# ssteinberg/wave_tracer

Hardware: AMD Instinct MI355X
Metric: Msamples/sec (whole node), cornell-box 1440^2 wave-mode (higher is better)
Workload: dtype f32

## Files before the change

### include/wtgpu.h

```cpp
#ifndef WTGPU_H
#define WTGPU_H

#include <stddef.h>
#include <stdint.h>

#include "wtgpu_scene.h"

#ifdef __cplusplus
extern "C" {
#endif

typedef struct wtgpu_scene wtgpu_scene;
typedef struct wtgpu_comm wtgpu_comm;

enum { WTGPU_OK = 0, WTGPU_ERR_INVALID = 1, WTGPU_ERR_NO_DEVICE = 2, WTGPU_ERR_HIP = 3, WTGPU_ERR_OOM = 4, WTGPU_ERR_OVERFLOW = 5, WTGPU_CANCELLED = 6,
       WTGPU_ERR_COMM = 7 };

typedef struct wtgpu_scene_params {
    uint32_t res;
    int32_t max_depth;
    int32_t fsd;
    int32_t mis;
    int32_t rr;
    int32_t force_ray_tracing;
// ... 34 lines not shown

int wtgpu_scene_upload(wtgpu_scene* scene, int device, uint64_t max_batch_samples);

int wtgpu_render(wtgpu_scene* scene, void* stream, double* d_value, double* d_weight, double* d_light, uint64_t sample_begin, uint64_t sample_end,
                 uint64_t seed);

int wtgpu_render_async(wtgpu_scene* scene, void* stream, double* d_value, double* d_weight, double* d_light, uint64_t sample_begin,
                       uint64_t sample_end, uint64_t seed);
int wtgpu_join(wtgpu_scene* scene, void* stream);

typedef int (*wtgpu_progress_cb)(uint64_t samples_done, uint64_t samples_total, void* user);
int wtgpu_render_progressive(wtgpu_scene* scene, void* stream, double* d_value, double* d_weight, double* d_light, uint64_t sample_begin,
                             uint64_t sample_end, uint64_t seed, uint32_t chunk_spp, wtgpu_progress_cb progress, void* user, uint64_t* spe_done);
int wtgpu_cancel(wtgpu_scene* scene);
int wtgpu_pause(wtgpu_scene* scene);
int wtgpu_resume(wtgpu_scene* scene);
typedef void (*wtgpu_capture_cb)(uint64_t samples_per_element_done, void* user);
int wtgpu_capture_intermediate(wtgpu_scene* scene, wtgpu_capture_cb capture, void* user);

#define WTGPU_COMM_ID_BYTES 128
int wtgpu_comm_unique_id(void* id_out);
int wtgpu_comm_create(int world_size, int rank, int device, const void* id, wtgpu_comm** out);
int wtgpu_film_reduce(wtgpu_comm* comm, void* stream, double* d_value, double* d_weight, double* d_light, uint64_t n_value, uint64_t n_weight,
                      int root);
void wtgpu_comm_destroy(wtgpu_comm* comm);

int wtgpu_trace_rays(wtgpu_scene* scene, void* stream, const float* d_rays, uint32_t n, float* d_dist, uint32_t* d_tuid, float* d_bary,
                     uint32_t* d_front);
int wtgpu_traverse_cones(wtgpu_scene* scene, void* stream, const float* d_cones, uint32_t n, uint32_t cap, float* d_dist, uint32_t* d_flags,
                         uint32_t* d_ntris, uint32_t* d_tris);

int wtgpu_query_regions(wtgpu_scene* scene, void* stream, const float* d_cones, uint32_t n, uint32_t edge_cap, float* d_dist, uint32_t* d_flags,
                        uint32_t* d_primary, uint32_t* d_ntris, uint32_t* d_nedges, uint32_t* d_edges, float* d_flux);

int wtgpu_scene_shape_id(const wtgpu_scene* scene, uint32_t shape, const char** id);
typedef struct wtgpu_sensor_mask_spec {
    int32_t present;
    uint32_t samples;
    const char* regex;
    const uint8_t* shape_flags;
    uint32_t n_shapes;
} wtgpu_sensor_mask_spec;
int wtgpu_scene_sensor_mask_spec(const wtgpu_scene* scene, wtgpu_sensor_mask_spec* out);
int wtgpu_sensor_mask(wtgpu_scene* scene, void* stream, const uint8_t* shape_flags, uint32_t samples, uint64_t seed, float* d_out);
int wtgpu_sensor_mask_host(const wtgpu_scene* scene, const uint8_t* shape_flags, uint32_t samples, uint64_t seed, uint32_t n_threads, float* out);

int wtgpu_calibrate_copy(uint64_t n_dwords, int repeats);

int wtgpu_get_counters(wtgpu_scene* scene, wtgpu_counters* out);
int wtgpu_reset_counters(wtgpu_scene* scene);

int wtgpu_last_render_timings(wtgpu_scene* scene, float out[12]);

int wtgpu_develop(const wtgpu_scene* scene, const double* value, const double* weight, const double* light, uint64_t spe, float* out);

int wtgpu_develop_device(wtgpu_scene* scene, void* stream, const double* d_value, const double* d_weight, const double* d_light, uint64_t spe, float* d_out);

typedef struct wtgpu_tonemap_spec {
    int32_t present, op, mode;
    float gamma, db_min, db_max;
    const char* colourmap;
    const char* function;
} wtgpu_tonemap_spec;
int wtgpu_scene_tonemap_spec(const wtgpu_scene* scene, wtgpu_tonemap_spec* out);
typedef struct wtgpu_tonemap {
    int32_t op, mode;
    float gamma, db_min, db_max;
    const float* table;
    uint32_t table_n;
} wtgpu_tonemap;
int wtgpu_tonemap_device(wtgpu_scene* scene, void* stream, const double* d_value, const double* d_weight, const double* d_light, uint64_t spe,
                         const wtgpu_tonemap* tm, uint32_t stokes_component, const float* d_mask, uint32_t format, void* d_out);
int wtgpu_tonemap_host(const wtgpu_scene* scene, const double* value, const double* weight, const double* light, uint64_t spe,
                       const wtgpu_tonemap* tm, uint32_t stokes_component, const float* mask, uint32_t format, uint32_t n_threads, void* out);

typedef struct wtgpu_film_stats_spec {
    uint32_t stokes_component, scale , bins , flags ;
    float lo, hi;
} wtgpu_film_stats_spec;
typedef struct wtgpu_film_stats {
    uint64_t n, n_nan, n_negative, n_zero, n_below, n_above;
    float min, max, min_positive, pad;
    double sum;
} wtgpu_film_stats;
int wtgpu_film_stats_edges(const wtgpu_film_stats_spec* spec, float* edges);
int wtgpu_film_stats_device(wtgpu_scene* scene, void* stream, const double* d_value, const double* d_weight, const double* d_light, uint64_t spe,
                            const wtgpu_film_stats_spec* spec, const float* d_mask, wtgpu_film_stats* out, uint64_t* hist);
int wtgpu_film_stats_host(const wtgpu_scene* scene, const double* value, const double* weight, const double* light, uint64_t spe,
                          const wtgpu_film_stats_spec* spec, const float* mask, uint32_t n_threads, wtgpu_film_stats* out, uint64_t* hist);

typedef struct wtgpu_film_compare_spec {
    uint32_t stokes_component, flags ;
    double eps;
} wtgpu_film_compare_spec;
typedef struct wtgpu_film_compare {
    uint64_t n, n_nonfinite, n_nonfinite_mismatch, n_differ, argmax;
    double max_abs, sum_abs, sum_sq, sum_a_sq, sum_b_sq, sum_rel;
} wtgpu_film_compare;
int wtgpu_film_compare_device(wtgpu_scene* scene, void* stream, const double* a_value, const double* a_weight, const double* a_light, uint64_t spe_a,
                              const double* b_value, const double* b_weight, const double* b_light, uint64_t spe_b, const wtgpu_film_compare_spec* spec,
                              const float* d_mask, wtgpu_film_compare* out, float* d_diff);
int wtgpu_film_compare_host(const wtgpu_scene* scene, const double* a_value, const double* a_weight, const double* a_light, uint64_t spe_a,
                            const double* b_value, const double* b_weight, const double* b_light, uint64_t spe_b, const wtgpu_film_compare_spec* spec,
                            const float* mask, uint32_t n_threads, wtgpu_film_compare* out, float* diff);

void wtgpu_scene_destroy(wtgpu_scene* scene);
// ... 8 lines not shown
```

### wave_tracer_amd/api.py

```python
import ctypes as C
import json
import math
import os

_HERE = os.path.dirname(os.path.abspath(__file__))

os.environ.setdefault("HSA_KERNARG_POOL_SIZE", str(16 << 20))


def lib_path():
    return os.environ.get("WTGPU_LIB") or os.path.join(_HERE, "libwtgpu.so")


class WtgpuError(RuntimeError):
    pass


class SceneParams(C.Structure):
    _fields_ = [("res", C.c_uint32), ("max_depth", C.c_int32), ("fsd", C.c_int32), ("mis", C.c_int32), ("rr", C.c_int32),
                ("force_ray_tracing", C.c_int32), ("mesh_detail", C.c_int32), ("lut_n_theta", C.c_uint32), ("lut_m", C.c_uint32),
                ("polarimetric", C.c_int32)]


class TestHooks(C.Structure):
# ... 22 lines not shown
class FilmStats(C.Structure):
    _fields_ = [("n", C.c_uint64), ("n_nan", C.c_uint64), ("n_negative", C.c_uint64), ("n_zero", C.c_uint64), ("n_below", C.c_uint64), ("n_above", C.c_uint64),
                ("min", C.c_float), ("max", C.c_float), ("min_positive", C.c_float), ("pad", C.c_float), ("sum", C.c_double)]


class FilmCompareSpec(C.Structure):
    _fields_ = [("stokes_component", C.c_uint32), ("flags", C.c_uint32), ("eps", C.c_double)]


FILM_COMPARE_FIELDS = [("n", C.c_uint64), ("n_nonfinite", C.c_uint64), ("n_nonfinite_mismatch", C.c_uint64), ("n_differ", C.c_uint64), ("argmax", C.c_uint64),
                       ("max_abs", C.c_double), ("sum_abs", C.c_double), ("sum_sq", C.c_double), ("sum_a_sq", C.c_double), ("sum_b_sq", C.c_double),
                       ("sum_rel", C.c_double)]


class FilmCompare(C.Structure):
    _fields_ = FILM_COMPARE_FIELDS


FILM_STATS_SCALES = ["linear", "dB"]
FILM_STATS_ABS, FILM_STATS_LUMINANCE = 1, 2
FILM_STATS_MAX_BINS = 4096
TONEMAP_OPS = ["linear", "gamma", "sRGB", "dB", "function"]
TONEMAP_MODES = ["select", "normal", "colourmap"]
TONEMAP_FORMATS = {"f32": 0, "u8": 1, "u16": 2}


class SceneInfo(C.Structure):
    _fields_ = [("width", C.c_uint32), ("height", C.c_uint32), ("channels", C.c_uint32), ("n_tris", C.c_uint32), ("n_edges", C.c_uint32),
                ("n_nodes", C.c_uint32), ("n_leaves", C.c_uint32), ("n_shapes", C.c_uint32), ("n_emitters", C.c_uint32),
                ("n_materials", C.c_uint32), ("max_depth", C.c_int32), ("sensor_type", C.c_uint32), ("fsd_lut_power", C.c_double * 2),
                ("bytes_per_sample_state", C.c_uint64), ("stokes", C.c_uint32), ("integrator", C.c_uint32)]


COUNTER_FIELDS = ["samples", "segments", "ray_queries", "cone_queries", "vertices", "connections", "shadow_rays", "cone_tri_overflow",
                  "edge_overflow", "fsd_edge_overflow", "fsd_pool_overflow", "fsd_interactions", "null_interactions",
                  "surface_interactions", "light_splats", "walk_iteration_cap_hits", "traversal_stack_dropped"]


class Counters(C.Structure):
    _fields_ = [(n, C.c_uint64) for n in COUNTER_FIELDS]

    def as_dict(self):
        return {n: int(getattr(self, n)) for n in COUNTER_FIELDS}


SYMBOLS = ["wtgpu_scene_create_named", "wtgpu_scene_create_from_desc", "wtgpu_scene_get_info", "wtgpu_scene_host_desc",
           "wtgpu_scene_upload", "wtgpu_render", "wtgpu_trace_rays", "wtgpu_traverse_cones", "wtgpu_get_counters",
           "wtgpu_reset_counters", "wtgpu_last_render_timings", "wtgpu_develop", "wtgpu_scene_destroy", "wtgpu_last_error",
           "wtgpu_scene_stats_json", "wtgpu_calibrate_copy", "wtgpu_render_async", "wtgpu_join", "wtgpu_query_regions", "wtgpu_render_progressive",
           "wtgpu_cancel", "wtgpu_pause", "wtgpu_resume", "wtgpu_capture_intermediate", "wtgpu_comm_unique_id", "wtgpu_comm_create", "wtgpu_film_reduce", "wtgpu_comm_destroy", "wtgpu_scene_create_from_xml",
           "wtgpu_scene_shape_id", "wtgpu_scene_sensor_mask_spec", "wtgpu_sensor_mask", "wtgpu_sensor_mask_host",
           "wtgpu_scene_tonemap_spec", "wtgpu_develop_device", "wtgpu_tonemap_device", "wtgpu_tonemap_host",
           "wtgpu_film_stats_edges", "wtgpu_film_stats_device", "wtgpu_film_stats_host",
           "wtgpu_film_compare_device", "wtgpu_film_compare_host"]
PROGRESS_CB = C.CFUNCTYPE(C.c_int, C.c_uint64, C.c_uint64, C.c_void_p)
CAPTURE_CB = C.CFUNCTYPE(None, C.c_uint64, C.c_void_p)

_lib = None


def connect_class_order():
    import numpy as np
    lib = load_library()
    lib.wtgpu_test_connect_class_order.argtypes = [C.c_void_p, C.c_uint32, C.c_void_p, C.c_void_p]
    n, dim = C.c_uint32(0), C.c_uint32(0)
    _check(lib.wtgpu_test_connect_class_order(None, 0, C.byref(n), C.byref(dim)))
    keys = np.zeros(n.value, np.uint32)
    _check(lib.wtgpu_test_connect_class_order(keys.ctypes.data, keys.size, C.byref(n), C.byref(dim)))
    return keys, int(dim.value)


def load_library():
    global _lib
    if _lib is not None:
        return _lib
    p = lib_path()
    if not os.path.exists(p):
        raise WtgpuError(f"{p} is missing: build it with `python -c 'import __graft_entry__ as g; g.build()'` "
                         f"(hipcc --offload-arch=gfx950); wave_tracer_amd has no CPU fallback")
    os.environ.setdefault("HSA_KERNARG_POOL_SIZE", str(16 << 20))
    try:
        import torch
    except ImportError:
        pass
    lib = C.CDLL(p)
    vp, u64, u32, i32 = C.c_void_p, C.c_uint64, C.c_uint32, C.c_int
    lib.wtgpu_scene_create_named.argtypes = [C.c_char_p, C.POINTER(SceneParams), C.POINTER(vp)]
    lib.wtgpu_scene_create_named_hooks.argtypes = [C.c_char_p, C.POINTER(SceneParams), C.POINTER(TestHooks), C.POINTER(vp)]
    lib.wtgpu_scene_create_from_desc.argtypes = [vp, C.POINTER(vp)]
    lib.wtgpu_scene_create_from_xml.argtypes = [C.c_char_p, C.POINTER(C.c_char_p), u32, C.POINTER(SceneParams), C.POINTER(vp)]
    lib.wtgpu_scene_compare.argtypes = [vp, vp, C.c_char_p, C.c_size_t]
    lib.wtgpu_scene_compare_part.argtypes = [vp, vp, C.c_char_p, C.c_char_p, C.c_size_t]
    lib.wtgpu_trace_ab_stats.argtypes = [vp, C.POINTER(C.c_double), C.POINTER(C.c_double), C.POINTER(u64), C.POINTER(u64), C.POINTER(u64)]
    lib.wtgpu_render_progressive.argtypes = [vp, vp, vp, vp, vp, u64, u64, u64, u32, PROGRESS_CB, vp, C.POINTER(u64)]
    lib.wtgpu_cancel.argtypes = [vp]
    lib.wtgpu_pause.argtypes = [vp]
    lib.wtgpu_resume.argtypes = [vp]
    lib.wtgpu_capture_intermediate.argtypes = [vp, CAPTURE_CB, vp]
    lib.wtgpu_comm_unique_id.argtypes = [vp]
    lib.wtgpu_comm_create.argtypes = [i32, i32, i32, vp, C.POINTER(vp)]
    lib.wtgpu_film_reduce.argtypes = [vp, vp, vp, vp, vp, u64, u64, i32]
    lib.wtgpu_comm_destroy.argtypes = [vp]
    lib.wtgpu_comm_destroy.restype = None
    lib.wtgpu_scene_get_info.argtypes = [vp, C.POINTER(SceneInfo)]
    lib.wtgpu_scene_host_desc.argtypes = [vp]
    lib.wtgpu_scene_host_desc.restype = vp
    lib.wtgpu_scene_upload.argtypes = [vp, i32, u64]
    lib.wtgpu_render.argtypes = [vp, vp, vp, vp, vp, u64, u64, u64]
    lib.wtgpu_render_async.argtypes = [vp, vp, vp, vp, vp, u64, u64, u64]
    lib.wtgpu_join.argtypes = [vp, vp]
    lib.wtgpu_trace_rays.argtypes = [vp, vp, vp, u32, vp, vp, vp, vp]
    lib.wtgpu_traverse_cones.argtypes = [vp, vp, vp, u32, u32, vp, vp, vp, vp]
    lib.wtgpu_query_regions.argtypes = [vp, vp, vp, u32, u32, vp, vp, vp, vp, vp, vp, vp]
    lib.wtgpu_test_fsd_apertures.argtypes = [vp, vp, vp, vp, vp, vp, u32, u32, u32, u32, vp, vp]
    lib.wtgpu_test_utd_sums.argtypes = [vp, vp, vp, vp, vp, u32, u32, u32, vp, vp, vp]
    lib.wtgpu_test_profile_counters.argtypes = [vp, vp, u32]
    lib.wtgpu_test_bsdf_queries.argtypes = [vp, vp, vp, u32, i32, vp]
    lib.wtgpu_test_source_queries.argtypes = [vp, vp, vp, u32, vp]
    lib.wtgpu_scene_shape_id.argtypes = [vp, u32, C.POINTER(C.c_char_p)]
    lib.wtgpu_scene_sensor_mask_spec.argtypes = [vp, C.POINTER(SensorMaskSpec)]
    lib.wtgpu_sensor_mask.argtypes = [vp, vp, vp, u32, u64, vp]
    lib.wtgpu_sensor_mask_host.argtypes = [vp, vp, u32, u64, u32, vp]
    lib.wtgpu_scene_tonemap_spec.argtypes = [vp, C.POINTER(TonemapSpec)]
    lib.wtgpu_develop_device.argtypes = [vp, vp, vp, vp, vp, u64, vp]
    lib.wtgpu_tonemap_device.argtypes = [vp, vp, vp, vp, vp, u64, C.POINTER(Tonemap), u32, vp, u32, vp]
    lib.wtgpu_tonemap_host.argtypes = [vp, vp, vp, vp, u64, C.POINTER(Tonemap), u32, vp, u32, u32, vp]
    lib.wtgpu_film_stats_edges.argtypes = [C.POINTER(FilmStatsSpec), vp]
    lib.wtgpu_film_stats_device.argtypes = [vp, vp, vp, vp, vp, u64, C.POINTER(FilmStatsSpec), vp, vp, vp]
    lib.wtgpu_film_stats_host.argtypes = [vp, vp, vp, vp, u64, C.POINTER(FilmStatsSpec), vp, u32, vp, vp]
    lib.wtgpu_film_compare_device.argtypes = [vp, vp, vp, vp, vp, u64, vp, vp, vp, u64, C.POINTER(FilmCompareSpec), vp, vp, vp]
    lib.wtgpu_film_compare_host.argtypes = [vp, vp, vp, vp, u64, vp, vp, vp, u64, C.POINTER(FilmCompareSpec), vp, u32, vp, vp]
    lib.wtgpu_calibrate_copy.argtypes = [u64, i32]
    lib.wtgpu_get_counters.argtypes = [vp, C.POINTER(Counters)]
    lib.wtgpu_reset_counters.argtypes = [vp]
    lib.wtgpu_last_render_timings.argtypes = [vp, C.POINTER(C.c_float * 12)]
    lib.wtgpu_develop.argtypes = [vp, vp, vp, vp, u64, vp]
    lib.wtgpu_scene_destroy.argtypes = [vp]
    lib.wtgpu_scene_destroy.restype = None
    lib.wtgpu_last_error.restype = C.c_char_p
    lib.wtgpu_scene_stats_json.argtypes = [vp]
    lib.wtgpu_scene_stats_json.restype = C.c_char_p
    _lib = lib
    return lib


def _check(rc):
    if rc != 0:
        raise WtgpuError(f"wtgpu error {rc}: {load_library().wtgpu_last_error().decode(errors='replace')}")


class Scene:

    def __init__(self, name, res=256, max_depth=-1, fsd=-1, mis=-1, rr=-1, force_ray_tracing=0, mesh_detail=1, lut=(0, 0), only_s=None, only_t=None, crop_of=0,
                 polarimetric=0):
        lib = load_library()
        p = SceneParams(res, max_depth, fsd, mis, rr, force_ray_tracing, mesh_detail, lut[0], lut[1], polarimetric)
        h = C.c_void_p()
        if only_s is None and only_t is None and not crop_of:
            _check(lib.wtgpu_scene_create_named(name.encode(), C.byref(p), C.byref(h)))
        else:
            hooks = TestHooks(0 if only_s is None else only_s + 1, 0 if only_t is None else only_t + 1, crop_of)
            _check(lib.wtgpu_scene_create_named_hooks(name.encode(), C.byref(p), C.byref(hooks), C.byref(h)))
        self._h = h
        self.name = name
        info = SceneInfo()
        _check(lib.wtgpu_scene_get_info(h, C.byref(info)))
        self.info = info
        self.spectral_channels, self.stokes = info.channels, info.stokes
        self.width, self.height, self.channels = info.width, info.height, info.channels * info.stokes
        self.device = None

    @classmethod
    def from_desc(cls, desc_ptr, keepalive=None, name="<desc>"):
        lib = load_library()
        self = cls.__new__(cls)
        h = C.c_void_p()
        _check(lib.wtgpu_scene_create_from_desc(C.c_void_p(desc_ptr), C.byref(h)))
        self._h = h
        self._keepalive = keepalive
        self.name = name
        info = SceneInfo()
        _check(lib.wtgpu_scene_get_info(h, C.byref(info)))
        self.info = info
        self.spectral_channels, self.stokes = info.channels, info.stokes
        self.width, self.height, self.channels = info.width, info.height, info.channels * info.stokes
        self.device = None
        return self

# ... 430 lines not shown
        import numpy as np
        sets = [self._host_films("film_compare_host", *films)[:3] for films in (films_a, films_b)]
        m = None if mask is None else np.ascontiguousarray(mask, dtype=np.float32)
        if m is not None and m.size != self.width * self.height:
            raise ValueError("film_compare_host: a mask of the scene's size expected")
        d = {}

        def call(spec, rec, planes):
            if diff:
                d["diff"] = np.zeros((self.height, self.width, planes), dtype=np.float32)
            _check(load_library().wtgpu_film_compare_host(self._h, *(t.ctypes.data for t in sets[0]), int(spe_a), *(t.ctypes.data for t in sets[1]), int(spe_b),
                                                          C.byref(spec), None if m is None else m.ctypes.data, int(threads), C.cast(rec, C.c_void_p),
                                                          d["diff"].ctypes.data if diff else None))
        out = self._film_compare(call, stokes_component, abs, luminance, eps)
        out.update(d)
        return out

    def profile_counters(self, n=8):
        out = (C.c_uint64 * n)()
        _check(load_library().wtgpu_test_profile_counters(self._h, out, n))
        return [int(v) for v in out]

    def connect_class_items(self, slice=0, max_items=1 << 22):
        import numpy as np
        lib = load_library()
        lib.wtgpu_test_connect_class_items.argtypes = [C.c_void_p, C.c_uint32, C.c_void_p, C.c_void_p, C.c_uint32, C.c_void_p]
        n_keys = connect_class_order()[0].size
        table = np.zeros(3 * n_keys + 1, np.uint32)
        items = np.zeros(max_items, np.uint32)
        n = C.c_uint32(0)
        _check(lib.wtgpu_test_connect_class_items(self._h, slice, table.ctypes.data, items.ctypes.data, items.size, C.byref(n)))
        return table[:n_keys + 1].copy(), table[n_keys + 1:2 * n_keys + 1].copy(), table[2 * n_keys + 1:].copy(), items[:n.value].copy()

    def counters(self):
        c = Counters()
        _check(load_library().wtgpu_get_counters(self._h, C.byref(c)))
        return c.as_dict()

    def reset_counters(self):
        _check(load_library().wtgpu_reset_counters(self._h))

    def trace_ab_stats(self):
        a, b, d, w, r = C.c_double(0), C.c_double(0), C.c_uint64(0), C.c_uint64(0), C.c_uint64(0)
        _check(load_library().wtgpu_trace_ab_stats(self._h, C.byref(a), C.byref(b), C.byref(d), C.byref(w), C.byref(r)))
        return {"ms_refill": a.value, "ms_sm": b.value, "differing_words": int(d.value), "walks": int(w.value), "rounds": int(r.value)}

    def timings(self):
        t = (C.c_float * 12)()
        _check(load_library().wtgpu_last_render_timings(self._h, C.byref(t)))
        return {"generate_ms": t[0], "trace_ms": t[1], "interact_ms": t[2], "connect_ms": t[3], "rounds": int(t[4]),
                "trace_launches": int(t[5]), "batches": int(t[6]), "trace_heavy_ms": t[7], "interact_b_ms": t[8], "flux_ms": t[9],
                "interact_c_ms": t[10], "rounds_per_batch": float(t[11])}

    def close(self):
        if self._h:
            load_library().wtgpu_scene_destroy(self._h)
            self._h = None

    def __del__(self):
        try:
            self.close()
        except Exception:
            pass


class Comm:

    def __init__(self, world, rank, device, unique_id):
        h = C.c_void_p()
        self._id = C.create_string_buffer(bytes(unique_id), 128)
        _check(load_library().wtgpu_comm_create(int(world), int(rank), int(device), self._id, C.byref(h)))
        self._h = h

    @staticmethod
    def unique_id():
        buf = C.create_string_buffer(128)
        _check(load_library().wtgpu_comm_unique_id(buf))
        return buf.raw

    def film_reduce(self, value, weight, light, root=0, stream=None):
        sp = C.c_void_p(stream) if stream else None
        _check(load_library().wtgpu_film_reduce(self._h, sp, value.data_ptr(), weight.data_ptr(), light.data_ptr(), value.numel(), weight.numel(), int(root)))

    def close(self):
        if self._h:
            load_library().wtgpu_comm_destroy(self._h)
            self._h = None

    def __del__(self):
        try:
            self.close()
        except Exception:
            pass
```

### wave_tracer_amd/csrc/kernels_fsd.hip

```cpp
#include "wtgpu_kernels.h"

namespace wtk {

__global__ void __launch_bounds__(64, 3) k_flux_split(launch_args_t a) {
    __shared__ coop_gather_shared_t sh;
    coop_set_dropped_counter(sh, a.st.counters + kDroppedSlot);
    uint32_t* ctl = a.st.ctl;
    const uint32_t n = ctl[CTL_INTC_COUNT];
    const int lane = threadIdx.x & 63;
    for (;;) {
        const uint32_t base = wave_grab(ctl + CTL_FSPLIT_HEAD);
        if (base >= n) break;
        uint32_t w_mine = 0;
        bool need = false;
        if (base + (uint32_t)lane < n) {
            w_mine = a.st.intc_queue[base + lane];
            need = is_region_marker(a.st.trav[(size_t)w_mine * kTravWords + WT_TRAV_WORD(tuid)]);
        }
        unsigned long long m = __ballot(need);
        while (m) {
            const int src = __ffsll((long long)m) - 1;
            m &= m - 1;
            const uint32_t w = (uint32_t)__shfl((int)w_mine, src, 64);
            const walk_trace_in_t wk = walk_load_trace_in(a.st.walks, a.st.walk_words, w);
            const cone_t tcone = walk_trace_envelope(a.sc, wk);
            const float beam_dist = __uint_as_float(a.st.trav[(size_t)w * kTravWords + WT_TRAV_WORD(dist)]);
            const float region_depth = __uint_as_float(a.st.trav[(size_t)w * kTravWords + WT_TRAV_WORD(region_depth)]);
            if (threadIdx.x == 0) a.st.facc[w] = 0.0;
            coop_split(a.sc, tcone, range_t{beam_dist, beam_dist + region_depth}, sh, a.flux_task_tris, [&](int32_t ptr) {
                const uint32_t idx = atomicAdd(ctl + CTL_FTASK_COUNT, 1u);
                if (idx < a.st.ftask_cap)
                    a.st.ftasks[idx] = make_uint2(w, (uint32_t)ptr);
                else
                    atomicAdd(a.st.counters + offsetof(bdpt_counters_t, fsd_pool_overflow) / sizeof(unsigned long long), 1ull);
            });
            __syncthreads();
        }
    }
}
__global__ void __launch_bounds__(64, WTGPU_LB_FLUX) k_flux_tasks(launch_args_t a) {
    __shared__ coop_gather_shared_t sh;
    coop_set_dropped_counter(sh, a.st.counters + kDroppedSlot);
    uint32_t* ctl = a.st.ctl;
    const uint32_t n = min(ctl[CTL_FTASK_COUNT], a.st.ftask_cap);
    const size_t W2 = 2 * (size_t)a.st.cap;
    for (;;) {
        const uint32_t item = wave_grab_item(ctl + CTL_FTASK_HEAD);
        if (item >= n) break;
        const uint2 task = a.st.ftasks[item];
        const uint32_t w = task.x;
        walk_t wk;
        soa_load(a.st.walks, a.st.walk_words, w, wk);
        const float beam_dist = __uint_as_float(a.st.trav[(size_t)w * kTravWords + WT_TRAV_WORD(dist)]);
        const float region_depth = __uint_as_float(a.st.trav[(size_t)w * kTravWords + WT_TRAV_WORD(region_depth)]);
        const bool want_front = a.st.trav[(size_t)w * kTravWords + WT_TRAV_WORD(front_face)] != 0;
        const range_t izr{beam_dist, beam_dist + region_depth};
        const vec3 sd3 = beam_footprint(wk.beam, beam_dist) / kBeamEnvelope;
        const cone_t tcone = walk_trace_envelope(a.sc, wk);
        unsigned long long gst[2] = {0, 0};
        const double flux = coop_gather(a.sc, tcone, izr, wk.beam.env, cone_frame(wk.beam.env), izr, vec2{sd3.x, sd3.y}, want_front, sh, true, false,
                                        a.profile ? gst : nullptr, (int32_t)task.y).flux;
        if (threadIdx.x == 0) {
            if (flux != 0.0) unsafeAtomicAdd(&a.st.facc[w], flux);
            if (a.profile) {
                atomicAdd(a.st.counters + kNumCounters + 0, 1ull);
                atomicAdd(a.st.counters + kNumCounters + 1, gst[0]);
                atomicAdd(a.st.counters + kNumCounters + 2, gst[1]);
                atomicMax(a.st.counters + kNumCounters + 4, gst[0]);
            }
        }
        __syncthreads();
    }
}

constexpr uint32_t kEasyTries = 512;
constexpr uint32_t kStageSegs = 256;
template <int BLOCK>
WT_D void interact_c_body(const launch_args_t& a, int in) {
    constexpr bool HARD = BLOCK > 64;
    __shared__ uint32_t s_item;
    __shared__ uint32_t s_tmin;
    __shared__ float s_res[3];
    __shared__ stack_entry_t lds[8];
    __shared__ fsd_edge_t s_seg[kStageSegs];
    uint32_t* ctl = a.st.ctl;
    const uint32_t n = ctl[HARD ? CTL_INTD_COUNT : CTL_INTC_COUNT];
    const uint32_t* queue_in = HARD ? a.st.intd_queue : a.st.intc_queue;
    const int tid = threadIdx.x, lane = threadIdx.x & 63;
    bdpt_counters_t ctr;
    memset(&ctr, 0, sizeof(ctr));
    const size_t W2 = 2 * (size_t)a.st.cap;
    const fsd_pool_t pool{a.st.fsd_hdr, a.st.fsd_edges, ctl + CTL_FSD_COUNTER, a.st.fsd_cap, ctl + CTL_FSD_ECOUNTER, a.st.fsd_ecap};
    for (;;) {
        const long long pl0 = a.profile == 3 ? clock64() : 0;
        uint32_t item = 0;
        if (HARD) {
            __syncthreads();
            if (tid == 0) s_item = atomicAdd(ctl + CTL_INTD_HEAD, 1u);
            __syncthreads();
            item = s_item;
        } else
            item = wave_grab_item(ctl + CTL_INTC_HEAD);
        if (item >= n) break;
        const uint32_t w = queue_in[item];
        uint32_t i, stream;
        walk_ident(a, w, i, stream);
        const uint64_t j = a.j0 + i;
        const uint32_t pix = (uint32_t)(j % a.npix);
        const uint64_t sample_id = ((uint64_t)pix << 32) | ((a.sample_begin + j / a.npix) & 0xFFFFFFFFull);
        const uint32_t rng_draws = a.st.walks[(size_t)w * a.st.walk_words + WT_WALK_WORD(rng_draws)];
        const uint32_t slot = a.st.trav[(size_t)w * kTravWords + WT_TRAV_WORD(by)];
        fsd_aperture_t ap = pool.hdr[slot];
        const fsd_edges_ref_t ed = fsd_pool_edges(pool, slot);
        const long long pc0 = a.profile == 3 ? clock64() : 0;
        if (!HARD) {
            const walk_trace_in_t wk = walk_load_trace_in(a.st.walks, a.st.walk_words, w);
            cone_t benv = wk.env;
            const float tr_dist = __uint_as_float(a.st.trav[(size_t)w * kTravWords + WT_TRAV_WORD(dist)]);
            const float tr_depth = __uint_as_float(a.st.trav[(size_t)w * kTravWords + WT_TRAV_WORD(region_depth)]);
            const uint32_t tr_tuid = a.st.trav[(size_t)w * kTravWords + WT_TRAV_WORD(tuid)], tr_ntris = a.st.trav[(size_t)w * kTravWords + WT_TRAV_WORD(ntris)];
            const bool tr_front = a.st.trav[(size_t)w * kTravWords + WT_TRAV_WORD(front_face)] != 0;
            const range_t izr{tr_dist, tr_dist + tr_depth};
            const vec2 axes = cone_axes(benv, tr_dist);
            const vec2 sigma{axes.x / kBeamEnvelope, axes.y / kBeamEnvelope};
            double flux;
            if (is_region_marker(tr_tuid)) {
                flux = a.st.facc[w];
            } else {
                const uint32_t* tl = a.st.tris + (size_t)w * kTriListWords;
                flux = (uint32_t)lane < tr_ntris ? (double)region_triangle_flux(a.sc, cone_frame(benv), benv, izr, sigma, tl[lane], tr_front) : 0.0;
#pragma unroll
                for (int off = 32; off > 0; off >>= 1) flux += __shfl_xor(flux, off, 64);
            }
            const float I = (float)(1.0 - flux);
            ap.recp_I = I > 0.f ? 1.f / I : 0.f;
            if (lane == 0) pool.hdr[slot] = ap;
        }
        const sampler_t ss = make_sampler(a.seed, sample_id, stream, 0);
        const uint32_t base = fsd_tries_base(make_sampler(a.seed, sample_id, stream, rng_draws));
        const uint32_t max_tries = fsd_max_tries(ap);
        const uint32_t t_begin = HARD ? kEasyTries : 0u, t_end = HARD ? max_tries : (max_tries < kEasyTries ? max_tries : kEasyTries);
        bool acc = false;
        uint32_t t_acc = 0;
        float rx = 0.f, ry = 0.f, rf = 0.f;
        auto run_tries = [&](const fsd_edges_ref_t& edr) {
            for (uint32_t t0 = t_begin; t0 < t_end && !acc; t0 += BLOCK) {
                const uint32_t t = t0 + (uint32_t)tid;
                fsd_try_t r{{0.f, 0.f}, 0.f, 0u};
                if (t < t_end) r = fsd_try(a.sc, ap, edr, sampler_at(ss, base + t * kFsdDrawsPerTry));
                if (!HARD) {
                    const unsigned long long am = __ballot(r.accept != 0);
                    if (am) {
                        const int wl = __ffsll((long long)am) - 1;
                        rx = __shfl(r.x.x, wl, 64);
                        ry = __shfl(r.x.y, wl, 64);
                        rf = __shfl(r.f, wl, 64);
                        t_acc = t0 + (uint32_t)wl;
                        acc = true;
                    }
                } else {
                    if (tid == 0) s_tmin = 0xFFFFFFFFu;
                    __syncthreads();
                    if (r.accept) atomicMin(&s_tmin, t);
                    __syncthreads();
                    const uint32_t tm = s_tmin;
                    if (tm != 0xFFFFFFFFu) {
                        if (t == tm) {
                            s_res[0] = r.x.x;
                            s_res[1] = r.x.y;
                            s_res[2] = r.f;
                        }
                        __syncthreads();
                        rx = s_res[0];
                        ry = s_res[1];
                        rf = s_res[2];
                        t_acc = tm;
                        acc = true;
                    }
                    __syncthreads();
                }
            }
        };
        if (ap.n_edges <= kStageSegs) {
            __syncthreads();
            for (uint32_t k = (uint32_t)tid; k < ap.n_edges; k += BLOCK) s_seg[k] = ed.p[k];
            __syncthreads();
            run_tries(fsd_edges_ref_t{s_seg, 1});
        } else
            run_tries(ed);
        if (a.profile == 3 && tid == 0) {
            const int bin = 31 - __clz((int)max(ap.n_edges, 1u));
            atomicAdd(a.st.counters + kNumCounters + 8 + bin, 1ull);
            atomicAdd(a.st.counters + kNumCounters + 24 + bin, (unsigned long long)(acc ? t_acc + 1u - t_begin : t_end - t_begin));
            atomicAdd(a.st.counters + kNumCounters + 40 + bin, (unsigned long long)(clock64() - pc0));
            atomicAdd(a.st.counters + kNumCounters + 112 + bin, (unsigned long long)(pc0 - pl0));
        }
        const long long pm0 = a.profile == 3 ? clock64() : 0;
        if (!HARD && !acc && t_end < max_tries) {
            if (lane == 0) a.st.intd_queue[atomicAdd(ctl + CTL_INTD_COUNT, 1u)] = w;
            continue;
        }
        bool cont = false;
        if (tid == 0) {
            walk_t wk;
            soa_load(a.st.walks, a.st.walk_words, w, wk);
            trav_result_t tr;
            soa_load(a.st.trav, kTravWords, w, tr);
            fsd_defer_t defer;
            defer.defer_sampling = defer.to_sampling_pass = 0;
            defer.have_aperture = 1;
            defer.split_no_primary = 0;
            defer.known_no_primary = 1;
            defer.no_primary = 0;
            defer.has_gather = defer.gather_n_edges = defer.gather_edge_overflow = 0;
            defer.gather_flux = 0.f;
            defer.gather_edges = nullptr;
            defer.pending = 0;
            defer.resolved = 1;
            defer.slot = slot;
            defer.base = base;
            defer.next_try = 0;
            defer.fs = fsd_finalize(ap, acc, vec2{rx, ry}, rf);
            defer.end_draws = fsd_draws_after(base, acc ? t_acc : max_tries - 1u);
            const uint_list_t tris{a.st.tris + (size_t)w * kTriListWords, 1u, kMaxConeTris};
            const vertex_store_t vs{a.st.verts, a.st.vert_words, w};
            stack_ref_t stack = make_stack_ref(lds, 1, 8, 8, nullptr);
            cont = bdpt_walk_step<2>(a.sc, wk, tr, tris, vs, pool, a.seed, sample_id, stream, &ctr, &stack, &defer);
            wk.active = cont ? 1u : 0u;
            soa_store(a.st.walks, a.st.walk_words, w, wk);
            if (a.profile == 3) atomicAdd(a.st.counters + kNumCounters + 96 + (31 - __clz((int)max(ap.n_edges, 1u))), (unsigned long long)(clock64() - pm0));
        }
        if (tid < 64) queue_append(a, ctl, 1 - in, cont, w);
    }
    if (a.count_stats && tid < 64) flush_counters(a.st.counters, ctr);
}
__global__ void __launch_bounds__(64, WTGPU_LB_INTERACT_C) k_interact_c(launch_args_t a, int in) { interact_c_body<64>(a, in); }
__global__ void __launch_bounds__(WTGPU_HARD_BLOCK) k_interact_c_hard(launch_args_t a, int in) { interact_c_body<WTGPU_HARD_BLOCK>(a, in); }

}
```

### wave_tracer_amd/csrc/kernels_trace.hip

```cpp
#include "wtgpu_kernels.h"

namespace wtk {

}
#include "kernels_trace_refill.h"
namespace wtk {

__global__ void __launch_bounds__(kBlock, WTGPU_LB_TRACE) k_trace_refill(launch_args_t a, int in, int first_round, uint32_t round) { trace_refill_body(a, in, first_round, round); }

#ifndef WTGPU_SM_EXACT_MIN
#define WTGPU_SM_EXACT_MIN 24
#endif
#ifndef WTGPU_SM_SPLIT_NODE
#define WTGPU_SM_SPLIT_NODE 0
#endif
#ifndef WTGPU_SM_BOTH
#define WTGPU_SM_BOTH 0
#endif
enum : int { PH_IDLE = 0, PH_NODE = 1, PH_TRI = 2, PH_EXACT = 3, PH_SERVE = 4, PH_POLICY = 5, PH_RAYDONE = 6 };
#ifdef WTGPU_SM_PROF
#define SP_DECL() unsigned long long sp_t[8] = {0, 0, 0, 0, 0, 0, 0, 0}, sp_l[8] = {0, 0, 0, 0, 0, 0, 0, 0}, sp_n[8] = {0, 0, 0, 0, 0, 0, 0, 0}; long long sp_c = 0
#define SP_BEGIN() sp_c = clock64()
#define SP_END(i, mask) do { const long long d_ = clock64() - sp_c; sp_t[i] += (unsigned long long)d_; sp_l[i] += (unsigned long long)d_ * (unsigned long long)__popcll(mask); sp_n[i] += 1; } while (0)
#else
#define SP_DECL()
#define SP_BEGIN()
#define SP_END(i, mask)
#endif
__global__ void __launch_bounds__(kBlock, WTGPU_LB_TRACE) k_trace_sm(launch_args_t a, int in, int first_round, uint32_t round) {
    __shared__ stack_entry_t lds[kLdsStack * kBlock];
    __shared__ float lds_tri[12 * kBlock];
    uint32_t* ctl = a.st.ctl;
    const uint32_t n = queue_count(ctl, in);
    if (blockIdx.x == 0 && threadIdx.x == 0) trace_round_begin(ctl, in, round, n);
    bdpt_counters_t ctr;
    memset(&ctr, 0, sizeof(ctr));
    stack_entry_t spill[kSpillStack];
    stack_ref_t stack;
    lds_stack(lds, spill, stack);
    const lane_nodes_t ns = lane_nodes(a.sc);
    const bool rt = a.sc.sensor.ray_trace_only || a.sc.opts.force_ray_tracing;
    const int lane = threadIdx.x & 63;
    const unsigned long long below = (1ull << lane) - 1ull;
    float* my_tri = lds_tri + threadIdx.x;
    int ph = PH_IDLE;
    uint32_t w = 0;
    uint32_t t_next = 0, t_left = 0;
    bool ray = false;
    bool pol = false, pol_hit = false;
    cone_t env;
    axis_walk_t aw;
    cone_query_t q;
    memset(&env, 0, sizeof(env));
    memset(&aw, 0, sizeof(aw));
    memset(&q, 0, sizeof(q));
    bool exhausted = false;
    SP_DECL();
    for (;;) {
// ... 544 lines not shown
        tr_finish(a, ctl, ctr, fin, w, r);
    }
    if (a.count_stats) flush_counters(a.st.counters, ctr);
}
__global__ void __launch_bounds__(kBlock, WTGPU_LB_TRACE) k_tr_tail(launch_args_t a, uint32_t it) {
    __shared__ stack_entry_t lds[kLdsStack * kBlock];
    uint32_t* ctl = a.st.ctl;
    const uint32_t n = ctl[CTL_TPOL_COUNT0 + (it & 1u)];
    if (blockIdx.x == 0 && threadIdx.x == 0) ctl[CTL_TCONE_COUNT0] = ctl[CTL_TCONE_COUNT1] = 0;
    bdpt_counters_t ctr;
    memset(&ctr, 0, sizeof(ctr));
    stack_entry_t spill[kSpillStack];
    stack_ref_t stack;
    lds_stack(lds, spill, stack);
    const lane_nodes_t ns = lane_nodes(a.sc);
    const bool rt = a.sc.sensor.ray_trace_only || a.sc.opts.force_ray_tracing;
    const int lane = threadIdx.x & 63;
    uint32_t* stage = trace_stage_words(a);
    const uint32_t* polq = trace_pol_queue(a);
    for (;;) {
        const uint32_t base = wave_grab(ctl + CTL_TPOL_HEAD);
        if (base >= n) break;
        const uint32_t qi = base + (uint32_t)lane;
        const bool have = qi < n;
        uint32_t w = 0;
        trav_result_t r;
        if (have) {
            w = polq[qi];
            trace_stage_t ts;
            soa_load(stage, kStageWords, w, ts);
            uint32_t* slot = a.st.tris + (size_t)w * kTriListWords;
            const uint_list_t tris{slot, 1u, (a.collect_list & 1u) ? kMaxConeTris : 0u, reinterpret_cast<float*>(slot + kMaxConeTris)};
            cone_query_t q;
            for (;;) {
                const int need = aw_next(a.sc, ts.env, rt, stack, ts.aw, q, r);
                if (need == AW_FINAL) break;
                if (need == AW_TEST) {
                    aw_test_done(ts.aw, cone_attempt_too_short_by(a.sc, ts.env, ts.aw.cand, ts.aw.sr, ts.aw.min_df_prog));
                    continue;
                }
                while (cq_running(q)) {
                    while (q.s > 0 && q.leaf == 0) cq_node_step(ns, ts.env, stack, q);
                    if (q.leaf != 0) cq_leaf_step(a.sc, ts.env, stack, tris, q);
                }
                cq_end(ts.env, tris, q);
                if (aw_query_done(a.sc, ts.env, ts.aw, q.rec, r)) break;
            }
        }
        tr_finish(a, ctl, ctr, have, w, r);
    }
    if (a.count_stats) flush_counters(a.st.counters, ctr);
}

template <bool PROF>
WT_D void trace_heavy_body(const launch_args_t& a, coop_shared_t& sh) {
    coop_set_dropped_counter(sh, a.st.counters + kDroppedSlot);
    uint32_t* ctl = a.st.ctl;
    const uint32_t n = ctl[CTL_HEAVY_COUNT];
    const uint32_t* hq = a.st.heavy_queue;
    uint32_t* head = ctl + CTL_HEAVY_HEAD;
    unsigned long long n_segments = 0, n_ray_queries = 0, n_cone_queries = 0, n_overflow = 0;
    const bool rt = a.sc.sensor.ray_trace_only || a.sc.opts.force_ray_tracing;
    for (;;) {
        const uint32_t item = wave_grab_item(head);
        if (item >= n) break;
        const uint32_t w = uniform(hq[item]);
        const walk_trace_in_t wk = walk_load_trace_in(a.st.walks, a.st.walk_words, w);
        const uint_list_t tris{a.st.tris + (size_t)w * kTriListWords, 1u, (a.collect_list & 1u) ? kMaxConeTris : 0u};
        const cone_t env = uniform(walk_trace_envelope(a.sc, wk));
        unsigned long long prof[12] = {0, 0, 0, 0, 0, 0, 0, 0, 0, 0, 0, 0};
        const long long tt0 = PROF ? clock64() : 0;
        const uint32_t* tv = a.st.trav + (size_t)w * kTravWords;
        const float dist0 = uniform(__uint_as_float(tv[WT_TRAV_WORD(dist)]));
        const uint32_t seg0 = uniform(tv[WT_TRAV_WORD(ntris)]);
        const uint32_t nray0 = uniform(tv[WT_TRAV_WORD(n_ray_queries)]), ncone0 = uniform(tv[WT_TRAV_WORD(n_cone_queries)]);
        ray_hit_t axis;
        axis.tuid = uniform(tv[WT_TRAV_WORD(tuid)]);
        axis.bx = uniform(__uint_as_float(tv[WT_TRAV_WORD(bx)]));
        axis.by = uniform(__uint_as_float(tv[WT_TRAV_WORD(by)]));
        axis.dist = uniform(__uint_as_float(tv[WT_TRAV_WORD(pdist)]));
        axis.front_face = uniform(tv[WT_TRAV_WORD(front_face)]);
        const uint32_t short0 = uniform(tv[WT_TRAV_WORD(overflow)]);
        const uint32_t origin0 = uniform(wk.prev_offset_tuid);
        const trav_result_t tr2 = coop_traverse(a.sc, env, uniform(wavenum_to_wavelen_m(wk.k)), WT_INF, rt, sh, tris, PROF ? prof : nullptr, true, seg0, dist0, nray0, ncone0,
                                                &axis, !(a.collect_list & 1u) || (a.collect_list & 2u), a.heavy_probe != 0, a.heavy_cache ? short0 : kInvalid, a.heavy_cache ? origin0 : kInvalid, a.heavy_cache != 0);
        if (PROF && threadIdx.x == 0) {
            prof[3] = (unsigned long long)(clock64() - tt0);
            for (int q = 0; q < 4; ++q) atomicAdd(a.st.counters + kNumCounters + q, prof[q]);
            atomicAdd(a.st.counters + kNumCounters + 5, prof[5]);
            atomicAdd(a.st.counters + kNumCounters + 6, prof[6]);
            atomicAdd(a.st.counters + kNumCounters + 7, prof[7]);
            for (int q = 8; q < 12; ++q) atomicAdd(a.st.counters + kNumCounters + q, prof[q]);
            atomicAdd(a.st.counters + kNumCounters + 4, 1ull);
        }
        n_segments += 1;
        n_ray_queries += tr2.n_ray_queries;
        n_cone_queries += tr2.n_cone_queries;
        if (a.collect_list & 1u) n_overflow += tr2.overflow;
        if (threadIdx.x == 0) soa_store(a.st.trav, kTravWords, w, tr2);
    }
    if (a.count_stats && threadIdx.x == 0) {
        unsigned long long* g = a.st.counters;
        if (n_segments) atomicAdd(g + offsetof(bdpt_counters_t, segments) / 8, n_segments);
        if (n_ray_queries) atomicAdd(g + offsetof(bdpt_counters_t, ray_queries) / 8, n_ray_queries);
        if (n_cone_queries) atomicAdd(g + offsetof(bdpt_counters_t, cone_queries) / 8, n_cone_queries);
        if (n_overflow) atomicAdd(g + offsetof(bdpt_counters_t, cone_tri_overflow) / 8, n_overflow);
    }
}
__global__ void __launch_bounds__(64, WTGPU_LB_HEAVY) k_trace_heavy(launch_args_t a) {
    __shared__ coop_shared_t sh;
    trace_heavy_body<false>(a, sh);
}
__global__ void __launch_bounds__(64, 2) k_trace_heavy_prof(launch_args_t a) {
    __shared__ coop_shared_t sh;
    trace_heavy_body<true>(a, sh);
}

__global__ void __launch_bounds__(256) k_calib_copy(const uint32_t* in, uint32_t* out, size_t n) {
    for (size_t i = blockIdx.x * (size_t)blockDim.x + threadIdx.x; i < n; i += (size_t)gridDim.x * blockDim.x) out[i] = in[i] + 1u;
}

__global__ void __launch_bounds__(kBlock) k_trace_rays(scene_t sc, const float* rays, uint32_t n, float* dist, uint32_t* tuid, float* bary, uint32_t* front) {
    __shared__ stack_entry_t lds[kLdsStack * kBlock];
    const uint32_t i = blockIdx.x * kBlock + threadIdx.x;
    if (i >= n) return;
    stack_entry_t spill[kSpillStack];
    stack_ref_t stack;
    lds_stack(lds, spill, stack);
    const float* r = rays + 8 * (size_t)i;
    ray_hit_t h;
    ads_intersect_ray(sc, vec3{r[0], r[1], r[2]}, vec3{r[3], r[4], r[5]}, range_t{r[6], r[7]}, stack, h);
    dist[i] = h.dist;
    tuid[i] = h.tuid;
    bary[2 * i] = h.bx;
    bary[2 * i + 1] = h.by;
    front[i] = h.front_face;
}
__global__ void __launch_bounds__(kBlock) k_traverse_cones(scene_t sc, const float* cones, uint32_t n, uint32_t cap, float* dist, uint32_t* flags,
                                                           uint32_t* ntris, uint32_t* out_tris, uint32_t* scratch_tris) {
    __shared__ stack_entry_t lds[kLdsStack * kBlock];
    const uint32_t i = blockIdx.x * kBlock + threadIdx.x;
    if (i >= n) return;
    stack_entry_t spill[128 - kLdsStack];
    stack_ref_t stack;
    lds_stack(lds, spill, stack);
    stack.cap = 128;
    const float* c = cones + 10 * (size_t)i;
    const vec3 d = normalize(vec3{c[3], c[4], c[5]});
    const cone_t env = make_cone(vec3{c[0], c[1], c[2]}, d, build_orthogonal_frame(d).t, c[6], c[8], c[7]);
    const uint_list_t tris{scratch_tris + i, n, kMaxConeTris, reinterpret_cast<float*>(scratch_tris + (size_t)n * kMaxConeTris) + i};
    const trav_result_t tr = traverse(sc, env, c[9], WT_INF, false, stack, tris);
    dist[i] = tr.dist;
    flags[i] = (tr.empty ? 1u : 0u) | (tr.ballistic ? 2u : 0u) | (tr.front_face ? 4u : 0u);
    ntris[i] = tr.ballistic ? (tr.empty ? 0 : 1) : tr.ntris;
    for (uint32_t j = 0; j < cap; ++j) out_tris[(size_t)i * cap + j] = kInvalid;
    if (tr.ballistic) {
        if (!tr.empty) out_tris[(size_t)i * cap] = tr.tuid;
    } else {
        uint32_t m = 0;
        for (uint32_t j = 0; j < tr.ntris; ++j) {
            const uint32_t v = tris[j];
// ... 55 lines not shown
```

### wave_tracer_amd/csrc/kernels_trace_refill.h

```cpp
#pragma once
#include "wtgpu_kernels.h"

namespace wtk {

#ifndef WTGPU_LEAF_NUM
#define WTGPU_LEAF_NUM 1
#define WTGPU_LEAF_DEN 2
#endif
#ifndef WTGPU_REFILL_MIN
#define WTGPU_REFILL_MIN 16
#endif
WT_D bool policy_next_query(const scene_t& sc, const cone_t& env, bool rt, const stack_ref_t& stack, axis_walk_t& aw, cone_query_t& q, trav_result_t& r) {
    for (;;) {
        const int need = aw_next(sc, env, rt, stack, aw, q, r);
        if (need != AW_TEST) return need == AW_QUERY;
        aw_test_done(aw, cone_attempt_too_short_by(sc, env, aw.cand, aw.sr, aw.min_df_prog));
    }
}
WT_D void trace_round_begin(uint32_t* ctl, int in, uint32_t round, uint32_t n) {
    ctl[CTL_COUNT0 + (1 - in)] = 0;
    ctl[CTL_BACK0 + (1 - in)] = 0;
    ctl[CTL_HEAD_INTERACT] = 0;
    ctl[CTL_INTB_COUNT] = 0;
    ctl[CTL_INTB_HEAD] = 0;
    ctl[CTL_GATHER_COUNT] = 0;
    ctl[CTL_GATHER_HEAD] = 0;
    ctl[CTL_INTC_COUNT] = 0;
    ctl[CTL_INTC_HEAD] = 0;
    ctl[CTL_FTASK_COUNT] = 0;
    ctl[CTL_FTASK_HEAD] = 0;
    ctl[CTL_FSPLIT_HEAD] = 0;
    ctl[CTL_EPOOL_COUNT] = 0;
    ctl[CTL_INTD_COUNT] = 0;
    ctl[CTL_INTD_HEAD] = 0;
#pragma unroll
    for (uint32_t c = 0; c < kNumWalkClasses; ++c) ctl[CTL_CLS_COUNT0 + c] = ctl[CTL_CLS_HEAD0 + c] = 0;
    ctl[CTL_UTD_COUNT0 + (round & 1u)] = 0;
    ctl[CTL_FSDQ_COUNT0 + ((round + 1u) & 1u)] = 0;
    ctl[CTL_FSDQ_HEAD] = 0;
    ctl[CTL_NEEQ_COUNT] = 0;
    ctl[CTL_NEEQ_HEAD] = 0;
    if (n > 0) ctl[CTL_ROUNDS] = round + 1;
}
WT_D void trace_refill_body(const launch_args_t& a, int in, int first_round, uint32_t round) {
    __shared__ stack_entry_t lds[kLdsStack * kBlock];
    uint32_t* ctl = a.st.ctl;
    const uint32_t n = queue_count(ctl, in);
    if (blockIdx.x == 0 && threadIdx.x == 0) trace_round_begin(ctl, in, round, n);
    bdpt_counters_t ctr;
    memset(&ctr, 0, sizeof(ctr));
    stack_entry_t spill[kSpillStack];
    stack_ref_t stack;
    lds_stack(lds, spill, stack);
    const size_t W2 = 2 * (size_t)a.st.cap;
    const bool rt = a.sc.sensor.ray_trace_only || a.sc.opts.force_ray_tracing;
    const int lane = threadIdx.x & 63;
    const unsigned long long below = (1ull << lane) - 1ull;
    int st = 0;
    uint32_t w = 0;
    cone_t env;
    axis_walk_t aw;
    cone_query_t q;
    uint_list_t tris{nullptr, 1u, 0u, nullptr};
    memset(&env, 0, sizeof(env));
    memset(&aw, 0, sizeof(aw));
    memset(&q, 0, sizeof(q));
    bool exhausted = false;
#ifdef WTGPU_REFILL_PROF
    unsigned long long pc[6] = {0, 0, 0, 0, 0, 0}, pl[6] = {0, 0, 0, 0, 0, 0};
    long long pt;
#define RP_BEGIN() pt = clock64()
#define RP_END(i, mask) do { const long long d_ = clock64() - pt; pc[i] += (unsigned long long)d_; pl[i] += (unsigned long long)d_ * (unsigned long long)__popcll(mask); } while (0)
#else
#define RP_BEGIN()
#define RP_END(i, mask)
#endif
    for (;;) {
        bool fin = false;
        trav_result_t r;
        RP_BEGIN();
        const unsigned long long m_srv = __ballot(st == 2);
        if (st == 2) {
            cq_end(env, tris, q);
            fin = aw_query_done(a.sc, env, aw, q.rec, r);
            if (!fin) fin = !policy_next_query(a.sc, env, rt, stack, aw, q, r);
            st = fin ? 0 : 1;
        }
        RP_END(0, m_srv);
        uint32_t w_fin = w;
        const int n_idle = __popcll(__ballot(st == 0 && !fin)), n_run = __popcll(__ballot(st == 1));
        bool fetched = false;
        const bool any_fin = __ballot(fin) != 0;
        if (!exhausted && !any_fin && (n_idle >= WTGPU_REFILL_MIN || n_run == 0)) {
            const unsigned long long im = __ballot(st == 0);
            const bool take = st == 0;
// ... 91 lines not shown
```

### wave_tracer_amd/csrc/kernels_walk.hip

```cpp
#include "wtgpu_kernels.h"
#include "kernels_trace_refill.h"

namespace wtk {

__global__ void __launch_bounds__(kBlock) k_generate(launch_args_t a) {
    const uint32_t i = blockIdx.x * kBlock + threadIdx.x;
    if (i == 0) {
        uint32_t* ctl = a.st.ctl;
        ctl[CTL_COUNT0] = 2 * a.nb;
        ctl[CTL_COUNT1] = 0;
        ctl[CTL_BACK0] = ctl[CTL_BACK1] = 0;
        ctl[CTL_HEAD_TRACE] = ctl[CTL_HEAD_INTERACT] = ctl[CTL_HEAVY_COUNT] = ctl[CTL_HEAVY_HEAD] = ctl[CTL_FSD_COUNTER] = ctl[CTL_ROUNDS] = 0;
        ctl[CTL_TPOL_COUNT0] = ctl[CTL_TPOL_COUNT1] = ctl[CTL_TPOL_HEAD] = ctl[CTL_TCONE_COUNT0] = ctl[CTL_TCONE_COUNT1] = ctl[CTL_TCONE_HEAD] = 0;
        ctl[CTL_INTB_COUNT] = ctl[CTL_INTB_HEAD] = ctl[CTL_GATHER_COUNT] = ctl[CTL_GATHER_HEAD] = ctl[CTL_INTC_COUNT] = ctl[CTL_INTC_HEAD] = 0;
        ctl[CTL_FTASK_COUNT] = ctl[CTL_FTASK_HEAD] = ctl[CTL_FSPLIT_HEAD] = ctl[CTL_EPOOL_COUNT] = ctl[CTL_FSD_ECOUNTER] = 0;
        ctl[CTL_INTD_COUNT] = ctl[CTL_INTD_HEAD] = 0;
    }
    if (i >= a.nb) return;
    const uint64_t j = a.j0 + i;
    const uint32_t pix = (uint32_t)(j % a.npix);
    const uint64_t s = a.sample_begin + j / a.npix;
    const uint64_t sample_id = ((uint64_t)pix << 32) | (s & 0xFFFFFFFFull);
    const size_t W2 = 2 * (size_t)a.st.cap;
    sample_ctx_t ctx;
    walk_t sw, ew;
    const vertex_store_t svs{a.st.verts, a.st.vert_words, i}, evs{a.st.verts, a.st.vert_words, (size_t)a.st.cap + i};
    bdpt_generate(a.sc, a.seed, sample_id, pix % a.sc.sensor.width, pix / a.sc.sensor.width, ctx, sw, ew, svs, evs);
    soa_store(a.st.ctx, kCtxWords, i, ctx);
    soa_store(a.st.walks, a.st.walk_words, i, sw);
    soa_store(a.st.walks, a.st.walk_words, (size_t)a.st.cap + i, ew);
}

template <int PASS, bool COOP = false>
WT_D void interact_body(const launch_args_t& a, int in, int first_round) {
    constexpr bool PASS_B = PASS == 1;
    __shared__ uint32_t s_io[COOP ? (kBlock / 64) * kIoRows * io_pitch<(int)kVertexWords>() : 1];
    uint32_t* io = s_io + (COOP ? (threadIdx.x >> 6) * kIoRows * io_pitch<(int)kVertexWords>() : 0);
    uint32_t* ctl = a.st.ctl;
    const uint32_t n = PASS_B ? ctl[CTL_INTB_COUNT] : queue_count(ctl, in);
    if (!PASS_B && blockIdx.x == 0 && threadIdx.x == 0) {
        ctl[CTL_HEAVY_COUNT] = 0;
        ctl[CTL_HEAVY_HEAD] = 0;
        ctl[CTL_HEAD_TRACE] = 0;
    }
    bdpt_counters_t ctr;
    memset(&ctr, 0, sizeof(ctr));
    const size_t W2 = 2 * (size_t)a.st.cap;
    const fsd_pool_t pool{a.st.fsd_hdr, a.st.fsd_edges, ctl + CTL_FSD_COUNTER, a.st.fsd_cap, ctl + CTL_FSD_ECOUNTER, a.st.fsd_ecap};
    for (;;) {
        const uint32_t qi = wave_grab(ctl + (PASS_B ? CTL_INTB_HEAD : CTL_HEAD_INTERACT)) + (threadIdx.x & 63);
        if (qi - (threadIdx.x & 63) >= n) break;
        bool cont = false;
        uint32_t w = 0;
        fsd_defer_t defer;
        defer.pending = defer.resolved = 0;
        defer.slot = defer.base = defer.next_try = defer.end_draws = 0;
        defer.defer_sampling = PASS_B ? 1u : 0u;
        defer.to_sampling_pass = 0;
        defer.have_aperture = 0;
        defer.split_no_primary = PASS_B ? 0u : 1u;
        defer.known_no_primary = PASS_B ? 1u : 0u;
        defer.no_primary = 0;
        defer.has_gather = defer.gather_n_edges = defer.gather_edge_overflow = 0;
        defer.gather_flux = 0.f;
        defer.gather_edges = nullptr;
        bool need_gather = false;
        const bool valid = qi < n;
        if (valid) w = PASS_B ? a.st.intb_queue[qi] : queue_walk(a, ctl, in, qi, first_round);
        walk_t wk;
// ... 117 lines not shown
            const uint64_t j = a.j0 + i;
            const uint32_t pix = (uint32_t)(j % a.npix);
            const uint64_t s = a.sample_begin + j / a.npix;
            const uint64_t sample_id = ((uint64_t)pix << 32) | (s & 0xFFFFFFFFull);
            const uint32_t* tv = a.st.trav + (size_t)w * kTravWords;
            const vec3 origin{__uint_as_float(tv[WT_TRAV_WORD(origin.x)]), __uint_as_float(tv[WT_TRAV_WORD(origin.y)]), __uint_as_float(tv[WT_TRAV_WORD(origin.z)])};
            const float beam_dist = __uint_as_float(tv[WT_TRAV_WORD(dist)]);
            const primary_hit_t ph{tv[WT_TRAV_WORD(tuid)], __uint_as_float(tv[WT_TRAV_WORD(pdist)]), __uint_as_float(tv[WT_TRAV_WORD(bx)]), __uint_as_float(tv[WT_TRAV_WORD(by)])};
            const walk_rec_t wr{a.st.walks + (size_t)w * a.st.walk_words};
            const vertex_store_t vs{a.st.verts, a.st.vert_words, w};
            cont = bdpt_surface_step<CLS>(a.sc, wr, origin, beam_dist, ph, vs, a.seed, sample_id, stream, &ctr);
        }
        queue_append(a, ctl, 1 - in, cont, w);
    }
    if (a.count_stats) {
        unsigned long long vsi = ctr.surface_interactions, vv = ctr.vertices;
        for (int off = 32; off > 0; off >>= 1) {
            vsi += __shfl_down(vsi, off, 64);
            vv += __shfl_down(vv, off, 64);
        }
        if ((threadIdx.x & 63) == 0) {
            if (vsi) atomicAdd(a.st.counters + offsetof(bdpt_counters_t, surface_interactions) / sizeof(unsigned long long), vsi);
            if (vv) atomicAdd(a.st.counters + offsetof(bdpt_counters_t, vertices) / sizeof(unsigned long long), vv);
        }
    }
}
#ifndef WTGPU_LB_CLS
#define WTGPU_LB_CLS 3
#endif
#ifndef WTGPU_LB_CLS_SPM
#define WTGPU_LB_CLS_SPM 3
#endif
#ifndef WTGPU_LB_SORTED
#define WTGPU_LB_SORTED 2
#endif
__global__ void __launch_bounds__(kBlock, WTGPU_LB_SORTED) k_interact_sorted(launch_args_t a, int in) {
    static constexpr unsigned char start_of[8] = {0, 0, 2, 0, 1, 0, 2, 3};
    const uint32_t first = start_of[blockIdx.x & 7u];
#pragma unroll 1
    for (uint32_t k = 0; k < kNumWalkClasses; ++k) {
        switch ((first + k) & 3u) {
        case WCLS_DIFFUSE: interact_cls_body<MAT_DIFFUSE>(a, in); break;
        case WCLS_DIELECTRIC: interact_cls_body<MAT_DIELECTRIC>(a, in); break;
        case WCLS_SPM: interact_cls_body<MAT_SURFACE_SPM>(a, in); break;
        default: interact_cls_body<-1>(a, in); break;
        }
    }
}
__global__ void __launch_bounds__(kBlock, WTGPU_LB_CLS) k_interact_diffuse(launch_args_t a, int in) { interact_cls_body<MAT_DIFFUSE>(a, in); }
__global__ void __launch_bounds__(kBlock, WTGPU_LB_CLS) k_interact_dielectric(launch_args_t a, int in) { interact_cls_body<MAT_DIELECTRIC>(a, in); }
__global__ void __launch_bounds__(kBlock, WTGPU_LB_CLS_SPM) k_interact_spm(launch_args_t a, int in) { interact_cls_body<MAT_SURFACE_SPM>(a, in); }
__global__ void __launch_bounds__(kBlock, WTGPU_LB_CLS_SPM) k_interact_any(launch_args_t a, int in) { interact_cls_body<-1>(a, in); }

__global__ void __launch_bounds__(64, 3) k_edges(launch_args_t a) {
    __shared__ coop_gather_shared_t sh;
    __shared__ coop_edges_t eg;
    coop_set_dropped_counter(sh, a.st.counters + kDroppedSlot);
    uint32_t* ctl = a.st.ctl;
    const uint32_t n = ctl[CTL_GATHER_COUNT];
    const size_t W2 = 2 * (size_t)a.st.cap;
    const fsd_pool_t pool{a.st.fsd_hdr, a.st.fsd_edges, ctl + CTL_FSD_COUNTER, a.st.fsd_cap, ctl + CTL_FSD_ECOUNTER, a.st.fsd_ecap};
    for (;;) {
        const uint32_t item = wave_grab_item(ctl + CTL_GATHER_HEAD);
        if (item >= n) break;
        const uint32_t w = a.st.gather_queue[item];
        walk_t wk;
        soa_load(a.st.walks, a.st.walk_words, w, wk);
        const float beam_dist = __uint_as_float(a.st.trav[(size_t)w * kTravWords + WT_TRAV_WORD(dist)]);
        const float region_depth = __uint_as_float(a.st.trav[(size_t)w * kTravWords + WT_TRAV_WORD(region_depth)]);
        const range_t izr{beam_dist, beam_dist + region_depth};
        const cone_t tcone = walk_trace_envelope(a.sc, wk);
        const gather_out_t g = coop_gather(a.sc, tcone, izr, wk.beam.env, cone_frame(wk.beam.env), izr, vec2{1.f, 1.f}, false, sh, false, true, nullptr, 1, &eg);
        __syncthreads();
        const bool bitmap = a.sc.n_edges <= kCoopEdgeBits;
        uint32_t n_edges = bitmap ? coop_edge_count(a.sc, eg) : g.n_edges, dropped = bitmap ? 0u : g.edge_overflow, off = 0;
        off = wave_grab0(ctl + CTL_EPOOL_COUNT, n_edges);
        if (off + n_edges > a.st.epool_cap) {
            dropped += n_edges;
            n_edges = 0;
        } else if (bitmap)
            coop_edge_write(a.sc, eg, a.st.epool + off, n_edges);
        else
            for (uint32_t j = threadIdx.x; j < n_edges; j += 64) a.st.epool[off + j] = eg.edge_ids[j];
        uint32_t marker = kGatherMarker, slot = 0;
        if (n_edges >= a.coop_aperture_min) {
            const uint32_t* eids = a.st.epool + off;
            __syncthreads();
            if (threadIdx.x == 0) slot = fsd_pool_alloc(pool);
            slot = wave_bcast0(slot);
            if (slot < pool.cap) {
                fsd_aperture_t ap;
                const vec3 sd3 = beam_footprint(wk.beam, beam_dist) / kBeamEnvelope;
                const bool ok = coop_build_aperture(a.sc, cone_frame(wk.beam.env), wk.beam.k, wk.beam.env, eids, n_edges, vec2{sd3.x, sd3.y}, pool, slot, ap);
                marker = ap.n_edges > 0 ? kApertureMarker : kNullApertureMarker;
                if (threadIdx.x == 0) {
                    pool.hdr[slot] = ap;
                    if (marker == kApertureMarker) a.st.intc_queue[atomicAdd(ctl + CTL_INTC_COUNT, 1u)] = w;
                    if (a.count_stats) {
                        if (dropped) atomicAdd(a.st.counters + offsetof(bdpt_counters_t, edge_overflow) / sizeof(unsigned long long), (unsigned long long)dropped);
                        if (ap.overflow) atomicAdd(a.st.counters + offsetof(bdpt_counters_t, fsd_edge_overflow) / sizeof(unsigned long long), (unsigned long long)ap.overflow);
                        if (!ok) atomicAdd(a.st.counters + offsetof(bdpt_counters_t, fsd_pool_overflow) / sizeof(unsigned long long), 1ull);
                    }
                }
            }
        }
        if (threadIdx.x == 0) {
            a.st.trav[(size_t)w * kTravWords + WT_TRAV_WORD(tuid)] = marker;
            a.st.trav[(size_t)w * kTravWords + WT_TRAV_WORD(by)] = slot;
            a.st.trav[(size_t)w * kTravWords + WT_TRAV_WORD(bx)] = off;
            a.st.trav[(size_t)w * kTravWords + WT_TRAV_WORD(n_ray_queries)] = n_edges;
            a.st.trav[(size_t)w * kTravWords + WT_TRAV_WORD(n_cone_queries)] = dropped;
            if (a.profile) {
                atomicAdd(a.st.counters + kNumCounters + 5, 1ull);
                atomicAdd(a.st.counters + kNumCounters + 6, (unsigned long long)n_edges);
                if (marker == kApertureMarker) atomicAdd(a.st.counters + kNumCounters + 3, 1ull);
            }
        }
        __syncthreads();
    }
}

__global__ void __launch_bounds__(kBlock, WTGPU_LB_INTERACT) k_interact(launch_args_t a, int in, int first_round) { interact_body<0>(a, in, first_round); }
#ifndef WTGPU_LB_INTERACT_COOP
#define WTGPU_LB_INTERACT_COOP 3
#endif
__global__ void __launch_bounds__(kBlock, WTGPU_LB_INTERACT_COOP) k_interact_coop(launch_args_t a, int in, int first_round) { interact_body<0, true>(a, in, first_round); }
__global__ void __launch_bounds__(kBlock, WTGPU_LB_INTERACT_B) k_interact_b(launch_args_t a, int in) { interact_body<1>(a, in, 0); }

#ifndef WTGPU_LIGHT_MAX_WALKS
#define WTGPU_LIGHT_MAX_WALKS 2048
#endif
constexpr uint32_t kLightMaxWalks = WTGPU_LIGHT_MAX_WALKS;
#ifndef WTGPU_LIGHT_FENCE
#define WTGPU_LIGHT_FENCE 0
#endif
WT_D void light_stage_barrier() {
#if WTGPU_LIGHT_FENCE
    __threadfence();
    __syncthreads();
#else
    __syncthreads();
    __builtin_amdgcn_fence(__ATOMIC_ACQUIRE, "agent");
#endif
}
__global__ void __launch_bounds__(kBlock, 2) k_light_rounds(launch_args_t a, int in, uint32_t round, uint32_t max_rounds) {
    uint32_t* ctl = a.st.ctl;
    uint32_t done = 0, stop = 0;
    if (queue_count(ctl, in) > kLightMaxWalks) {
        if (threadIdx.x == 0) {
            ctl[CTL_LIGHT_DONE] = 0;
            ctl[CTL_LIGHT_STOP] = 4;
        }
        return;
    }
    if (queue_count(ctl, in) == 0) max_rounds = 0;
    for (; done < max_rounds; ++done) {
        trace_refill_body(a, in, 0, round + done);
        light_stage_barrier();
        if (ctl[CTL_HEAVY_COUNT] != 0) {
            stop = 1;
            break;
        }
        interact_body<0>(a, in, 0);
        light_stage_barrier();
        if (ctl[CTL_GATHER_COUNT] != 0) {
            stop = 2;
            break;
        }
        interact_body<1>(a, in, 0);
        light_stage_barrier();
        if (ctl[CTL_INTC_COUNT] != 0) {
            stop = 3;
            break;
        }
        in = 1 - in;
        if (queue_count(ctl, in) == 0) {
            ++done;
            break;
        }
    }
    if (threadIdx.x == 0) {
        ctl[CTL_LIGHT_DONE] = done;
        ctl[CTL_LIGHT_STOP] = stop;
    }
}

}
```

### wave_tracer_amd/csrc/wtgpu.hip

```cpp
#include "wtgpu_host.h"

thread_local std::string g_err;

static void note_rounds(wtgpu_scene* s, uint32_t n) { s->rounds_hist[s->rounds_hist_n++ % 8u] = n; }
static int drain_rec(wtgpu_scene* s, chunk_rec_t& r) {
    if (!r.busy) return WTGPU_OK;
    HIP_CHECK(hipEventSynchronize(r.ev[r.ev_final]));
    const uint32_t rounds = r.h_ctl[CTL_ROUNDS];
    s->cap_hits += r.h_ctl[CTL_COUNT0 + (r.rounds_launched & 1u)] + r.h_ctl[CTL_BACK0 + (r.rounds_launched & 1u)];
    s->acc[4] += rounds;
    s->acc[5] += rounds;
    s->acc[6] += 1;
    s->rounds_launched_total += r.rounds_launched;
    if (s->knobs.timing) {
        auto elapsed = [](hipEvent_t a, hipEvent_t b) {
            float ms = 0.f;
            return hipEventElapsedTime(&ms, a, b) == hipSuccess ? ms : 0.f;
        };
        s->acc[0] += elapsed(r.ev[0], r.ev[1]);
        size_t e = 1;
        for (uint32_t k = 0; k < r.rounds_timed; ++k, e += 6) {
            static const int slot[6] = {1, 7, 2, 8, 9, 10};
            for (int q = 0; q < 6; ++q) s->acc[slot[q]] += elapsed(r.ev[e + q], r.ev[e + q + 1]);
        }
        s->acc[3] += elapsed(r.ev[e], r.ev[r.ev_final]);
    }
    r.busy = false;
    return WTGPU_OK;
}

struct batch_launcher_t {
    wtgpu_scene* s;
    const wtgpu_scene::knobs_t& K;
    uint32_t grid_round = 0, grid_heavy = 0;
    bool path_mode = false;
    bool ev_fail = false;
    static constexpr int kHpSlots = 64;
    bool hp_on = false, trace_on = false;
    double hp_t[kHpSlots] = {0};
    unsigned long hp_n[kHpSlots] = {0};
    static const char** hp_labels() {
        static const char* labels[kHpSlots] = {nullptr};
        return labels;
    }
    static int hp_slot(const char* label) {
        static std::mutex m;
        std::lock_guard<std::mutex> l(m);
        const char** labels = hp_labels();
        int i = 0;
        while (i < kHpSlots - 1 && labels[i] && std::strcmp(labels[i], label) != 0) ++i;
        if (!labels[i]) labels[i] = label;
        return i;
    }
    explicit batch_launcher_t(wtgpu_scene* s_) : s(s_), K(s_->knobs) {
        grid_round = s->n_cus * K.round_blocks_per_cu;
        grid_heavy = s->n_cus * K.heavy_waves_per_cu;
        path_mode = s->host.opts.integrator != INTEGRATOR_BDPT;
// ... 54 lines not shown
                const uint32_t shrink = round < K.shrink_r1 ? 1u : (round < K.shrink_r2 ? K.shrink_f1 : K.shrink_f2);
                g0 = std::max<uint32_t>(1u, gf / shrink);
                gh = std::max<uint32_t>(1u, std::min<uint32_t>(grid_heavy, walks_per_sample * nb) / (round < K.shrink_r1 ? 1u : (round < K.shrink_r2 ? K.shrink_h1 : 32u)));
            }
            const int sf = round == r_begin ? stage_from : 0;
            if (sf <= 0 && dbg_stage >= 2 + 3 * (int)round) {
                if (round < K.trace_ab) {
                    const int rc = trace_ab_round(s, a, st_, in, first, round, g0);
                    if (rc) return rc;
                } else if (K.trace_sm || (K.trace_staged && round < K.trace_staged_rounds))
                    launch_trace_alt(s, a, st_, in, first, round, g0);
                else
                    HP_LAUNCH(k_trace_refill, dim3(g0), dim3(kBlock), 0, st_, a, in, first, round);
            }
            rec(r, st_);
            if (sf <= 1 && dbg_stage >= 3 + 3 * (int)round) {
                if (a.profile == 2)
                    HP_LAUNCH(k_trace_heavy_prof, dim3(gh), dim3(64), 0, st_, a);
                else
                    HP_LAUNCH(k_trace_heavy, dim3(gh), dim3(64), 0, st_, a);
            }
            rec(r, st_);
            if (path_mode) {
                if (round > 0) HP_LAUNCH(k_path_fsd, dim3(gh), dim3(64), 0, st_, a, ps, round);
                if (dbg_stage >= 4 + 3 * (int)round) HP_LAUNCH(k_path_interact, dim3(g0), dim3(kBlock), 0, st_, a, ps, in, first, round);
                HP_LAUNCH(k_path_edges, dim3(gh), dim3(64), 0, st_, a, ps);
                HP_LAUNCH(k_path_interact_b, dim3(std::max<uint32_t>(1u, g0 / 2u)), dim3(kBlock), 0, st_, a, ps, in, round);
                HP_LAUNCH(k_path_nee, dim3(gh), dim3(64), 0, st_, a, ps, round);
                rec(r, st_);
                rec(r, st_);
                rec(r, st_);
                rec(r, st_);
                continue;
            }
            if (sf > 2) {
            } else if (K.sorted_interact) {
                HP_LAUNCH(k_classify, dim3(g0), dim3(kBlock), 0, st_, a, in, first);
                if (K.sorted_interact >= 2)
                    HP_LAUNCH(k_interact_sorted, dim3(g0), dim3(kBlock), 0, st_, a, in);
                else {
                HP_LAUNCH(k_interact_diffuse, dim3(std::max<uint32_t>(1u, g0 / K.grid_div_cls[0])), dim3(kBlock), 0, st_, a, in);
                HP_LAUNCH(k_interact_dielectric, dim3(std::max<uint32_t>(1u, g0 / K.grid_div_cls[1])), dim3(kBlock), 0, st_, a, in);
                HP_LAUNCH(k_interact_spm, dim3(std::max<uint32_t>(1u, g0 / K.grid_div_cls[2])), dim3(kBlock), 0, st_, a, in);
                HP_LAUNCH(k_interact_any, dim3(std::max<uint32_t>(1u, g0 / K.grid_div_cls[3])), dim3(kBlock), 0, st_, a, in);
                }
            } else if (K.coop_io)
                HP_LAUNCH(k_interact_coop, dim3(g0), dim3(kBlock), 0, st_, a, in, first);
            else
                HP_LAUNCH(k_interact, dim3(g0), dim3(kBlock), 0, st_, a, in, first);
            rec(r, st_);
            if (sf <= 3) HP_LAUNCH(k_edges, dim3(gh), dim3(64), 0, st_, a);
            if (sf <= 4) HP_LAUNCH(k_interact_b, dim3(std::max<uint32_t>(1u, g0 / grid_div_b)), dim3(kBlock), 0, st_, a, in);
            rec(r, st_);
            HP_LAUNCH(k_flux_split, dim3(std::max<uint32_t>(1u, gh / 4u)), dim3(64), 0, st_, a);
            HP_LAUNCH(k_flux_tasks, dim3(std::max<uint32_t>(1u, gh * grid_mul_flux)), dim3(64), 0, st_, a);
            rec(r, st_);
            HP_LAUNCH(k_interact_c, dim3(std::max<uint32_t>(1u, gh / grid_div_c)), dim3(64), 0, st_, a, in);
            HP_LAUNCH(k_interact_c_hard, dim3(std::max<uint32_t>(1u, gh / K.grid_div_hard)), dim3(WTGPU_HARD_BLOCK), 0, st_, a, in);
            rec(r, st_);
        }
        r.rounds_launched = r_end;
        return WTGPU_OK;
    }
    void light(const launch_args_t& a, hipStream_t st_, uint32_t launched) {
        if (path_mode || !K.light_rounds || launched >= K.max_rounds) return;
        HP_LAUNCH(k_light_rounds, dim3(1), dim3(kBlock), 0, st_, a, (int)(launched & 1u), launched, K.max_rounds - launched);
    }
    int tail(const launch_args_t& a, chunk_rec_t& r, hipStream_t st_) {
        const uint32_t nb = a.nb, gf = g_full(nb);
        if (path_mode) {
            HP_LAUNCH(k_path_flush, dim3(kFlushGrid), dim3(kBlock), 0, st_, a, (int)(r.rounds_launched & 1u));
        } else {
            const bool open = (uint32_t)s->host.opts.max_depth + 2 >= kKeyDim - 1;
            const bool staged = K.staged_connect && !open;
            const uint32_t by_class = !staged && K.connect_class ? 1u : 0u;
            HP_LAUNCH(k_connect_enum, dim3((nb + kEnumBlock - 1) / kEnumBlock), dim3(kEnumBlock), 0, st_, a, by_class);
            HP_LAUNCH(k_connect_scan, dim3(1), dim3(64), 0, st_, a, by_class);
            if (staged) {
                for (uint32_t c = 0; c < s->n_chunks; ++c) {
                    const uint32_t g = c == 0 ? gf : std::max<uint32_t>(1u, gf / 8u);
                    HP_LAUNCH(k_connect_eval, dim3(g), dim3(kBlock), 0, st_, a, c);
                    HP_LAUNCH(k_connect_shadow, dim3(g), dim3(kBlock), 0, st_, a, c);
                    HP_LAUNCH(k_connect_mis, dim3(g), dim3(kBlock), 0, st_, a, c);
                }
            } else if (by_class) {
                HP_LAUNCH(k_connect_class, dim3(gf), dim3(kBlock), 0, st_, a);
                if (open) HP_LAUNCH(k_connect_class_open, dim3(std::max<uint32_t>(1u, gf / 8u)), dim3(kBlock), 0, st_, a);
            } else {
                HP_LAUNCH(k_connect_strat, dim3(gf), dim3(kBlock), 0, st_, a);
                if (open) HP_LAUNCH(k_connect_strat_open, dim3(std::max<uint32_t>(1u, gf / 8u)), dim3(kBlock), 0, st_, a);
            }
            const uint32_t fw = a.film.width, fh = a.film.height, planes = film_planes(s->host.sensor);
            if (K.tiled_splat && s->host.sensor.rf_radius <= 1 && planes <= 16 && (uint64_t)nb * 2u >= (uint64_t)a.npix)
                HP_LAUNCH(k_connect_splat_tiled, dim3(fh * ((fw + kBlock - 1) / kBlock)), dim3(kBlock), 3 * kSplatCols * (planes + 1) * sizeof(double), st_, a);
            else
                HP_LAUNCH(k_connect_splat, dim3((nb + kBlock - 1) / kBlock), dim3(kBlock), 0, st_, a);
        }
        HIP_CHECK(hipGetLastError());
        HIP_CHECK(hipMemcpyAsync(r.h_ctl, a.st.ctl, CTL_WORDS * sizeof(uint32_t), hipMemcpyDeviceToHost, st_));
        r.ev_final = s->knobs.timing ? r.ev_used : 0;
        HIP_CHECK(hipEventRecord(r.ev[r.ev_final], st_));
        if (ev_fail) return fail(WTGPU_ERR_HIP, "hipEventRecord failed");
        r.busy = true;
        return WTGPU_OK;
    }
#undef HP_LAUNCH
    void report() const {
        if (!hp_on) return;
        const char* const* labels = hp_labels();
        for (int i = 0; i < kHpSlots; ++i)
            if (hp_n[i]) fprintf(stderr, "[host prof] %-22s %6lu calls %9.1f us total %7.2f us each\n", labels[i], hp_n[i], hp_t[i], hp_t[i] / hp_n[i]);
    }
};
static_assert(sizeof(launch_args_t) <= sizeof(wtgpu_scene::pending_t::args), "pending_t::args holds a launch block");

static uint32_t expected_rounds(const wtgpu_scene* s) {
    if (s->knobs.first_rounds) return s->knobs.first_rounds;
    if (s->rounds_hist_n == 0) return std::min<uint32_t>(kMaxWalkIters, 32u);
    const uint32_t n = std::min<uint32_t>(s->rounds_hist_n, 8u);
    uint32_t sum = 0;
    for (uint32_t i = 0; i < n; ++i) sum += s->rounds_hist[i];
    const uint32_t mean = (sum + n - 1) / n;
    return std::min<uint32_t>(kMaxWalkIters, mean + s->knobs.rounds_margin);
}
static int finish_look(wtgpu_scene* s, size_t k, batch_launcher_t& L) {
    wtgpu_scene::pending_t& p = s->pending[k];
    chunk_rec_t& r = *p.rec;
    launch_args_t a;
    std::memcpy(&a, p.args, sizeof(a));
    hipStream_t st_ = s->streams[k];
    uint32_t& launched = p.launched;
    const bool light = !L.path_mode && s->knobs.light_rounds != 0;
    uint32_t stop = 0;
    if (light && launched < s->knobs.max_rounds) {
        launched += r.h_mid[CTL_LIGHT_DONE];
        stop = r.h_mid[CTL_LIGHT_STOP];
        s->light_rounds_run += r.h_mid[CTL_LIGHT_DONE];
    }
    bool done = false;
    if (s->knobs.tail_diag) {
        static unsigned long long looks = 0, by_stop[8] = {0}, light_done = 0, left_sum = 0;
        static bool reg = false;
        if (!reg) { reg = true; atexit([] { fprintf(stderr, "[tail diag] looks %llu (stop 0/1/2/3/4: %llu %llu %llu %llu %llu), light rounds %llu, walks left at looks (sum) %llu\n", looks, by_stop[0], by_stop[1], by_stop[2], by_stop[3], by_stop[4], light_done, left_sum); }); }
        looks++; by_stop[stop < 8 ? stop : 7]++; light_done += light ? r.h_mid[CTL_LIGHT_DONE] : 0;
        left_sum += r.h_mid[CTL_COUNT0 + (launched & 1u)] + r.h_mid[CTL_BACK0 + (launched & 1u)];
    }
    if (stop >= 1 && stop <= 3) {
        static const int from[4] = {0, 1, 3, 5};
        const int rc = L.rounds(a, s->d_path_slices[k], r, st_, launched, launched + 1, from[stop]);
        if (rc) return rc;
        launched += 1;
    } else {
        const uint32_t q = launched & 1u;
        const uint32_t left = r.h_mid[CTL_COUNT0 + q] + r.h_mid[CTL_BACK0 + q];
        if (left == 0) {
            note_rounds(s, std::min<uint32_t>(r.h_mid[CTL_ROUNDS], kMaxWalkIters));
            done = true;
        } else if (launched >= s->knobs.max_rounds)
            done = true;
        else {
            s->round_fallbacks++;
            const uint32_t next = std::min<uint32_t>(s->knobs.max_rounds, launched + p.rounds_step);
            const int rc = L.rounds(a, s->d_path_slices[k], r, st_, launched, next);
            if (rc) return rc;
            launched = next;
            p.rounds_step = std::min<uint32_t>(64u, p.rounds_step * 2u);
        }
    }
    if (done) {
        p.active = false;
        r.rounds_launched = launched;
        return L.tail(a, r, st_);
    }
    L.light(a, st_, launched);
    HIP_CHECK(hipMemcpyAsync(r.h_mid, a.st.ctl, CTL_WORDS * sizeof(uint32_t), hipMemcpyDeviceToHost, st_));
    HIP_CHECK(hipEventRecord(r.ev_mid, st_));
    return WTGPU_OK;
}
static int serve_pending(wtgpu_scene* s, size_t k, batch_launcher_t& L) {
    const size_t n = s->pending.size();
    for (;;) {
        bool any = false, progressed = false;
        for (size_t j = 0; j < n; ++j) {
            wtgpu_scene::pending_t& p = s->pending[j];
            if (!p.active) continue;
            if (k != (size_t)-1 && !s->pending[k].active) break;
            any = true;
            const hipError_t q = hipEventQuery(p.rec->ev_mid);
            if (q == hipSuccess) {
                const int rc = finish_look(s, j, L);
                if (rc) return rc;
                progressed = true;
            } else if (q != hipErrorNotReady)
                HIP_CHECK(q);
            else
                (void)hipGetLastError();
        }
        if (k != (size_t)-1 ? !s->pending[k].active : !any) return WTGPU_OK;
        if (!progressed) {
            std::this_thread::sleep_for(std::chrono::microseconds(20));
        }
    }
}
static int finish_all_pending(wtgpu_scene* s) {
    bool any = false;
    for (const auto& p : s->pending) any = any || p.active;
    if (!any) return WTGPU_OK;
    batch_launcher_t L(s);
    return serve_pending(s, (size_t)-1, L);
// ... 122 lines not shown
```

### wave_tracer_amd/csrc/wtgpu_counters.hip

```cpp
#include "wtgpu_host.h"

extern "C" {

int wtgpu_get_counters(wtgpu_scene* s, wtgpu_counters* out) {
    if (!s || !out || !s->uploaded) return fail(WTGPU_ERR_INVALID, "scene not uploaded");
    bdpt_counters_t c;
    {
        const int rc = drain_all(s);
        if (rc) return rc;
    }
    HIP_CHECK(hipDeviceSynchronize());
    HIP_CHECK(hipMemcpy(&c, s->slices[0].counters, sizeof(c), hipMemcpyDeviceToHost));
    out->samples = s->samples_rendered;
    out->segments = c.segments;
    out->ray_queries = c.ray_queries;
    out->cone_queries = c.cone_queries;
    out->vertices = c.vertices;
    out->connections = c.connections;
    out->shadow_rays = c.shadow_rays;
    out->cone_tri_overflow = c.cone_tri_overflow;
    out->edge_overflow = c.edge_overflow;
    out->fsd_edge_overflow = c.fsd_edge_overflow;
    out->fsd_pool_overflow = c.fsd_pool_overflow;
    out->fsd_interactions = c.fsd_interactions;
// ... 26 lines not shown
    if (s->knobs.profile == 1) {
        unsigned long long p[8];
        HIP_CHECK(hipMemcpy(p, s->slices[0].counters + kNumCounters, sizeof(p), hipMemcpyDeviceToHost));
        fprintf(stderr, "[wtgpu profile] flux tasks: %llu, candidates %llu (max %llu per task), exact-tested %llu; k_edges: %llu walks, %llu edges, %llu apertures built\n", p[0], p[1], p[4], p[2], p[5], p[6], p[3]);
    }
    if (s->knobs.profile == 3) {
        unsigned long long p[kProfSlots];
        HIP_CHECK(hipMemcpy(p, s->slices[0].counters + kNumCounters, sizeof(p), hipMemcpyDeviceToHost));
        fprintf(stderr, "[wtgpu profile] pass C by aperture size (slice 0): bin=log2(segments) items tries/item kticks/item total-Mticks\n");
        for (int b = 0; b < 16; ++b)
            if (p[8 + b]) fprintf(stderr, "[wtgpu profile]   C %2d %8llu %10.1f %10.1f %10.1f   fetch+load %.1f commit %.1f kticks/item\n", b, p[8 + b], double(p[24 + b]) / p[8 + b], double(p[40 + b]) / p[8 + b] * 1e-3, double(p[40 + b]) * 1e-6, double(p[112 + b]) / p[8 + b] * 1e-3, double(p[96 + b]) / p[8 + b] * 1e-3);
        fprintf(stderr, "[wtgpu profile] pass B by gathered scene edges: bin items kticks/item total-Mticks\n");
        for (int b = 0; b < 16; ++b)
            if (p[56 + b]) fprintf(stderr, "[wtgpu profile]   B %2d %8llu %10.1f %10.1f\n", b, p[56 + b], double(p[72 + b]) / p[56 + b] * 1e-3, double(p[72 + b]) * 1e-6);
    }
#ifdef WTGPU_REFILL_PROF
    {
        unsigned long long p[16];
        HIP_CHECK(hipMemcpy(p, s->slices[0].counters + kNumCounters, sizeof(p), hipMemcpyDeviceToHost));
        const char* nm[6] = {"serve", "fetch", "store", "nodes", "leaf", "(ray in fetch)"};
        for (int i = 0; i < 6; ++i) fprintf(stderr, "[refill prof] %-16s %10.1f Mticks  lanes %.1f\n", nm[i], p[i] * 1e-6, p[i] ? double(p[8 + i]) / p[i] : 0.);
    }
#endif
#ifdef WTGPU_SM_PROF
    {
        unsigned long long p[64];
        HIP_CHECK(hipMemcpy(p, s->slices[0].counters + kNumCounters, sizeof(p), hipMemcpyDeviceToHost));
        const char* nm[7] = {"serve", "fetch", "aw_next", "store", "NODE", "TRI", "EXACT"};
        for (int i = 0; i < 7; ++i)
            fprintf(stderr, "[sm prof] %-8s %10.1f Mticks  %10.2f Msteps  %7.0f ticks/step  lanes %.1f\n", nm[i], p[32 + i] * 1e-6, p[48 + i] * 1e-6, p[48 + i] ? double(p[32 + i]) / p[48 + i] : 0.,
                    p[32 + i] ? double(p[40 + i]) / p[32 + i] : 0.);
    }
#endif
    if (s->knobs.profile == 2) {
        unsigned long long p[8];
        HIP_CHECK(hipMemcpy(p, s->slices[0].counters + kNumCounters, sizeof(p), hipMemcpyDeviceToHost));
        fprintf(stderr, "[wtgpu profile] heavy items %llu: clock ticks ray %llu probe %llu cone %llu total %llu (per item: ray %.0f probe %.0f cone %.0f total %.0f; cone+probe phase A %.0f phase B %.0f; phase-A steps %.1f entries %.1f)\n", p[4], p[0],
                p[1], p[2], p[3], p[4] ? double(p[0]) / p[4] : 0., p[4] ? double(p[1]) / p[4] : 0., p[4] ? double(p[2]) / p[4] : 0., p[4] ? double(p[3]) / p[4] : 0., p[4] ? double(p[5]) / p[4] : 0., p[4] ? double(p[6]) / p[4] : 0., p[4] ? double(p[7] & 0xffffffffull) / p[4] : 0., p[4] ? double(p[7] >> 32) / p[4] : 0.);
    }
    return WTGPU_OK;
}
int wtgpu_reset_counters(wtgpu_scene* s) {
    if (!s || !s->uploaded) return fail(WTGPU_ERR_INVALID, "scene not uploaded");
    {
        const int rc = drain_all(s);
        if (rc) return rc;
    }
    HIP_CHECK(hipDeviceSynchronize());
    HIP_CHECK(hipMemset(s->slices[0].counters, 0, (kNumCounters + kProfSlots + 1) * sizeof(unsigned long long)));
    s->samples_rendered = 0;
    s->cap_hits = 0;
    for (double& v : s->acc) v = 0;
    s->rounds_launched_total = 0;
    return WTGPU_OK;
}

int wtgpu_test_profile_counters(wtgpu_scene* s, unsigned long long* out, uint32_t n) {
    if (!s || !out || !s->uploaded || n > kProfSlots) return fail(WTGPU_ERR_INVALID, "wtgpu_test_profile_counters: uploaded scene, n <= kProfSlots");
    {
        const int rc = drain_all(s);
        if (rc) return rc;
    }
    HIP_CHECK(hipDeviceSynchronize());
    HIP_CHECK(hipMemcpy(out, s->slices[0].counters + kNumCounters, n * sizeof(unsigned long long), hipMemcpyDeviceToHost));
    return WTGPU_OK;
}

}
```

### wave_tracer_amd/csrc/wtgpu_host.h

```cpp
#pragma once
#include <hip/hip_runtime.h>
#include <chrono>

#include <atomic>
#include <cmath>
#include <cstdio>
#include <cstdlib>
#include <algorithm>
#include <cstring>
#include <memory>
#include <mutex>
#include <thread>
#include <string>
#include <vector>

#include "wtgpu_kernels.h"
#include "wtgpu_test_hooks.h"
#include "wtgpu_knobs.h"
#include "host/scene_builder.h"

static_assert(kKnobConeBudget == kConeBudget && kKnobFluxTaskTris == kFluxTaskTris, "wtgpu_knobs.h repeats two defaults of wtgpu_kernels.h");

#pragma GCC visibility push(hidden)
extern thread_local std::string g_err;
// ... 28 lines not shown

struct wtgpu_scene {
    std::unique_ptr<wth::scene_builder_t> builder;
    scene_t host{};
    scene_t dev{};
    std::vector<void*> dev_allocs;
    int device = -1;
    uint32_t n_cus = 0;
    bool uploaded = false;
    std::vector<device_state_t> slices;
    std::vector<const path_state_t*> d_path_slices;
    const unsigned char* d_tri_class = nullptr;
    uint32_t pend_cap = 0, n_chunks = 0;
    std::vector<hipStream_t> streams;
    std::vector<hipEvent_t> ev_done;
    hipEvent_t ev_begin = nullptr;
    hipEvent_t ev_stagger_last = nullptr;
    std::vector<chunk_rec_t> recs;
    size_t rec_next = 0;
    size_t slice_next = 0;
    struct pending_t {
        bool active = false;
        unsigned char args[1024];
        chunk_rec_t* rec = nullptr;
        uint32_t launched = 0, rounds_step = 8;
    };
    std::vector<pending_t> pending;
    uint32_t rounds_hist[8] = {0};
    uint32_t rounds_hist_n = 0;
    uint64_t round_fallbacks = 0;
    uint64_t rounds_launched_total = 0;
    std::string stats;
    double lut_power[2] = {0, 0};
    double acc[12] = {0};
    uint64_t samples_rendered = 0;
    uint64_t cap_hits = 0;
    std::atomic<int> cancel{0};
    std::atomic<int> paused{0};
    std::mutex capture_mutex;
    wtgpu_capture_cb capture_cb = nullptr;
    void* capture_user = nullptr;
    uint32_t* query_scratch = nullptr;
    size_t query_scratch_bytes = 0;
    wth::scene_file_extras_t file;
    uint8_t* d_mask_flags = nullptr;
    uint8_t* h_mask_flags = nullptr;
    hipEvent_t ev_mask = nullptr;
    float* d_tm_table = nullptr;
    float* h_tm_table = nullptr;
    hipEvent_t ev_tm = nullptr;
    film_scratch_t fs, fc;
    double ab_ms[2] = {0, 0};
    uint64_t ab_mismatch = 0, ab_walks = 0, ab_rounds = 0;
    uint64_t light_rounds_run = 0;
    using knobs_t = ::knobs_t;
    knobs_t knobs{};
};

struct device_guard_t {
    int prev = -1;
    explicit device_guard_t(int dev) {
        if (hipGetDevice(&prev) != hipSuccess) prev = -1;
        if (prev != dev) (void)hipSetDevice(dev);
        else prev = -1;
    }
    ~device_guard_t() {
        if (prev >= 0) (void)hipSetDevice(prev);
    }
};

template <class T>
int upload(wtgpu_scene* s, const T* src, size_t n, const T** dst) {
    *dst = nullptr;
    if (n == 0 || !src) return WTGPU_OK;
    void* p = nullptr;
    HIP_CHECK(hipMalloc(&p, n * sizeof(T)));
    s->dev_allocs.push_back(p);
    HIP_CHECK(hipMemcpy(p, src, n * sizeof(T), hipMemcpyHostToDevice));
    *dst = static_cast<const T*>(p);
    return WTGPU_OK;
}
template <class T>
int dmalloc(wtgpu_scene* s, T** p, size_t n) {
    void* q = nullptr;
    hipError_t e = hipMalloc(&q, n * sizeof(T));
    if (e != hipSuccess) return fail(WTGPU_ERR_OOM, std::string("hipMalloc of ") + std::to_string(n * sizeof(T)) + " bytes: " + hipGetErrorString(e));
    s->dev_allocs.push_back(q);
    *p = static_cast<T*>(q);
    return WTGPU_OK;
}


struct scene_extents_t {
    size_t spec_words = 0;
    size_t tex_words = 0;
    size_t shape_tris = 0;
    size_t kd_words = 0;
    size_t cmp_kdists = 0, cmp_kd_words = 0;
};
scene_extents_t scene_extents(const scene_t& sc);
void release_device(wtgpu_scene* s);
void film_scratch_free(film_scratch_t& f);
int drain_all(wtgpu_scene* s);
void launch_trace_alt(const wtgpu_scene* s, const launch_args_t& a, hipStream_t st_, int in, int first, uint32_t round, uint32_t g0);
int trace_ab_round(wtgpu_scene* s, const launch_args_t& a, hipStream_t st_, int in, int first, uint32_t round, uint32_t g0);
#pragma GCC visibility pop
```

### wave_tracer_amd/csrc/wtgpu_kernels.h

```cpp
#pragma once
#include <hip/hip_runtime.h>

#include <cstddef>
#include <cstdint>
#include <cstring>

#include "../../include/wtgpu.h"
#include "wt/bdpt.h"
#include "wt/coop.h"
#include "wt/coop_fsd.h"
#include "wt/coop_utd.h"
#include "wt/path.h"

using namespace wt;
namespace wt {
struct tonemap_args_t;
}

namespace wtk {


#ifndef WTGPU_LB_TRACE
#define WTGPU_LB_TRACE 3
#endif
#ifndef WTGPU_LB_HEAVY
#define WTGPU_LB_HEAVY 3
#endif
#ifndef WTGPU_LB_INTERACT
#define WTGPU_LB_INTERACT 3
#endif
#ifndef WTGPU_LB_INTERACT_B
#define WTGPU_LB_INTERACT_B 3
#endif
#ifndef WTGPU_LB_INTERACT_C
#define WTGPU_LB_INTERACT_C 3
#endif
#ifndef WTGPU_LB_FLUX
#define WTGPU_LB_FLUX 3
#endif
#ifndef WTGPU_LB_CONNECT
#define WTGPU_LB_CONNECT 2
#endif
constexpr uint32_t kFluxTaskTris = 2048;
constexpr int kBlock = 128;
#ifndef WTGPU_LDS_STACK
#define WTGPU_LDS_STACK 20
#endif
constexpr int kLdsStack = WTGPU_LDS_STACK;
constexpr uint32_t kConeBudget = 96;
constexpr int kSpillStack = 64 - kLdsStack;

enum : uint32_t { CTL_STRAT_HEAD_OPEN = 25, CTL_UTD_COUNT0 = 26, CTL_UTD_COUNT1 = 27, CTL_FSDQ_COUNT0 = 28, CTL_FSDQ_COUNT1 = 29, CTL_FSDQ_HEAD = 30, CTL_NEEQ_COUNT = 31, CTL_NEEQ_HEAD = 32, CTL_COUNT0 = 0, CTL_COUNT1 = 1, CTL_HEAD_TRACE = 2, CTL_HEAD_INTERACT = 3, CTL_HEAVY_COUNT = 4, CTL_HEAVY_HEAD = 5, CTL_FSD_COUNTER = 6,
                  CTL_ROUNDS = 7, CTL_STRAT_HEAD = 8, CTL_INTB_COUNT = 9, CTL_INTB_HEAD = 10, CTL_GATHER_COUNT = 11, CTL_GATHER_HEAD = 12, CTL_INTC_COUNT = 13, CTL_INTC_HEAD = 14, CTL_FTASK_COUNT = 15, CTL_FTASK_HEAD = 16, CTL_FSPLIT_HEAD = 17, CTL_EPOOL_COUNT = 18, CTL_FSD_ECOUNTER = 19, CTL_INTD_COUNT = 20, CTL_INTD_HEAD = 21, CTL_BACK0 = 22, CTL_BACK1 = 23,
                  CTL_TPOL_COUNT0 = 41, CTL_TPOL_COUNT1 = 42, CTL_TPOL_HEAD = 43, CTL_TCONE_COUNT0 = 44, CTL_TCONE_COUNT1 = 45, CTL_TCONE_HEAD = 46,
                  CTL_CLS_COUNT0 = 33, CTL_CLS_HEAD0 = 37,
                  CTL_LIGHT_DONE = 47, CTL_LIGHT_STOP = 48,
                  CTL_WORDS = 56 };
constexpr uint32_t kTriListWords = 128;
constexpr uint32_t kGatherMarker = 0xFFFFFFFEu;
constexpr uint32_t kApertureMarker = 0xFFFFFFFDu, kNullApertureMarker = 0xFFFFFFFCu;
__host__ __device__ inline bool is_region_marker(uint32_t t) { return t == kGatherMarker || t == kApertureMarker; }
constexpr uint32_t kKeyDim = kMaxVerts + 2, kNumKeys = kKeyDim * kKeyDim;
__host__ __device__ constexpr uint32_t class_key_work(uint32_t key) { return (key / kKeyDim) * (key % kKeyDim); }
__host__ __device__ constexpr uint32_t class_key_rank(uint32_t key) {
    uint32_t r = 0;
    for (uint32_t k = 0; k < kNumKeys; ++k)
        if (class_key_work(k) > class_key_work(key) || (class_key_work(k) == class_key_work(key) && k < key)) ++r;
    return r;
}
__host__ __device__ constexpr bool class_key_open(uint32_t key) { return key / kKeyDim == kKeyDim - 1 || key % kKeyDim == kKeyDim - 1; }
constexpr uint32_t kClassCount = kNumKeys + 1, kClassKey = kClassCount + kNumKeys, kClassTableWords = kClassKey + kNumKeys;

struct device_state_t {
    uint64_t cap = 0;
    uint32_t max_verts = 0;
    uint32_t walk_words = 0;
    size_t vert_words = 0;
    uint32_t* walks = nullptr;
    uint32_t* verts = nullptr;
    uint32_t* ctx = nullptr;
    uint32_t* trav = nullptr;
    uint32_t* tris = nullptr;
    uint32_t* queue[2] = {nullptr, nullptr};
    uint32_t* heavy_queue = nullptr;
    uint32_t* intb_queue = nullptr;
    uint32_t* gather_queue = nullptr;
    uint32_t* intc_queue = nullptr;
    uint32_t* intd_queue = nullptr;
    uint2* ftasks = nullptr;
    uint32_t ftask_cap = 0;
    double* facc = nullptr;
    uint32_t* epool = nullptr;
    uint32_t epool_cap = 0;
    uint32_t* ctl = nullptr;
    fsd_aperture_t* fsd_hdr = nullptr;
    fsd_edge_t* fsd_edges = nullptr;
    uint32_t fsd_cap = 0;
    uint32_t fsd_ecap = 0;
    uint32_t* strat_items = nullptr;
    uint32_t* strat_count = nullptr;
    uint32_t* strat_prefix = nullptr;
    double* lacc = nullptr;
    unsigned long long* counters = nullptr;
    const struct bdpt_ext_t* ext = nullptr;
};
struct bdpt_ext_t {
    const unsigned char* tri_class = nullptr;
    uint32_t* cls_queue = nullptr;
    struct conn_pending_t* pend = nullptr;
    uint32_t* surv = nullptr;
// ... 152 lines not shown
template <int W, class T>
WT_D void wave_store_records(uint32_t* base, size_t stride, uint32_t idx, uint32_t off, bool valid, uint32_t* lds, const T& in) {
    static_assert(sizeof(T) == 4 * W, "record size");
    constexpr int P = io_pitch<W>();
    const int lane = threadIdx.x & 63;
    const uint32_t* o = reinterpret_cast<const uint32_t*>(&in);
    const unsigned long long all = __ballot(valid);
    if (!all) return;
#pragma unroll 1
    for (int h = 0; h < 2; ++h) {
        if (valid && (lane >> 5) == h) {
#pragma unroll
            for (int i = 0; i < W; ++i) lds[(lane & 31) * P + i] = o[i];
        }
        __builtin_amdgcn_wave_barrier();
        unsigned long long m = all & (h ? 0xFFFFFFFF00000000ull : 0x00000000FFFFFFFFull);
        while (m) {
            const int r = __ffsll((long long)m) - 1;
            m &= m - 1;
            uint32_t* dst = base + (size_t)__builtin_amdgcn_readlane(idx, r) * stride + __builtin_amdgcn_readlane(off, r);
#pragma unroll
            for (int w0 = 0; w0 < W; w0 += 64)
                if (w0 + lane < W) dst[w0 + lane] = lds[(r & 31) * P + w0 + lane];
        }
        __builtin_amdgcn_wave_barrier();
    }
}

constexpr uint32_t kFlushGrid = 64;
constexpr int kEnumBlock = 1024;
constexpr uint32_t kSplatCols = kBlock + 2;
#ifndef WTGPU_HARD_BLOCK
#define WTGPU_HARD_BLOCK 256
#endif
__global__ void k_generate(launch_args_t a);
__global__ void k_trace_refill(launch_args_t a, int in, int first_round, uint32_t round);
__global__ void k_trace_sm(launch_args_t a, int in, int first_round, uint32_t round);
__global__ void k_tr_axis(launch_args_t a, int in, int first_round, uint32_t round);
__global__ void k_tr_cone(launch_args_t a, uint32_t it);
__global__ void k_tr_policy(launch_args_t a, uint32_t it);
__global__ void k_tr_tail(launch_args_t a, uint32_t it);
__global__ void k_trace_heavy(launch_args_t a);
__global__ void k_trace_heavy_prof(launch_args_t a);
__global__ void k_interact(launch_args_t a, int in, int first_round);
__global__ void k_classify(launch_args_t a, int in, int first_round);
__global__ void k_interact_diffuse(launch_args_t a, int in);
__global__ void k_interact_dielectric(launch_args_t a, int in);
__global__ void k_interact_spm(launch_args_t a, int in);
__global__ void k_interact_any(launch_args_t a, int in);
__global__ void k_interact_sorted(launch_args_t a, int in);
__global__ void k_interact_coop(launch_args_t a, int in, int first_round);
__global__ void k_edges(launch_args_t a);
__global__ void k_interact_b(launch_args_t a, int in);
__global__ void k_light_rounds(launch_args_t a, int in, uint32_t round, uint32_t max_rounds);
__global__ void k_flux_split(launch_args_t a);
__global__ void k_flux_tasks(launch_args_t a);
__global__ void k_interact_c(launch_args_t a, int in);
__global__ void k_interact_c_hard(launch_args_t a, int in);
__global__ void k_path_generate(launch_args_t a);
__global__ void k_path_fsd(launch_args_t a, const path_state_t* __restrict__ ps, uint32_t round);
__global__ void k_path_edges(launch_args_t a, const path_state_t* __restrict__ ps);
__global__ void k_path_interact(launch_args_t a, const path_state_t* __restrict__ ps, int in, int first_round, uint32_t round);
__global__ void k_path_interact_b(launch_args_t a, const path_state_t* __restrict__ ps, int in, uint32_t round);
__global__ void k_path_nee(launch_args_t a, const path_state_t* __restrict__ ps, uint32_t round);
__global__ void k_path_flush(launch_args_t a, int in);
__global__ void k_connect_enum(launch_args_t a, uint32_t by_class);
__global__ void k_connect_scan(launch_args_t a, uint32_t by_class);
__global__ void k_connect_strat(launch_args_t a);
__global__ void k_connect_strat_open(launch_args_t a);
__global__ void k_connect_class(launch_args_t a);
__global__ void k_connect_class_open(launch_args_t a);
__global__ void k_connect_eval(launch_args_t a, uint32_t chunk);
__global__ void k_connect_shadow(launch_args_t a, uint32_t chunk);
__global__ void k_connect_mis(launch_args_t a, uint32_t chunk);
__global__ void k_connect_splat(launch_args_t a);
__global__ void k_connect_splat_tiled(launch_args_t a);
__global__ void k_calib_copy(const uint32_t* in, uint32_t* out, size_t n);
__global__ void k_trace_rays(scene_t sc, const float* rays, uint32_t n, float* dist, uint32_t* tuid, float* bary, uint32_t* front);
__global__ void k_traverse_cones(scene_t sc, const float* cones, uint32_t n, uint32_t cap, float* dist, uint32_t* flags, uint32_t* ntris, uint32_t* out_tris,
                                 uint32_t* scratch_tris);
__global__ void k_query_regions(scene_t sc, const float* cones, uint32_t n, uint32_t edge_cap, float* dist, uint32_t* flags, uint32_t* primary, uint32_t* ntris,
                                uint32_t* nedges, uint32_t* edges, float* flux, unsigned long long* dropped);
int test_fsd_apertures(const scene_t& sc, hipStream_t stream, const float* d_cones, const float* d_sk, const uint32_t* d_ids, const uint32_t* d_n_ids,
                       uint32_t n, uint32_t id_cap, uint32_t pool_cap, uint32_t mode, uint32_t* d_hdr, float* d_segs);
int test_utd_sums(const scene_t& sc, hipStream_t stream, const float* d_queries, const uint32_t* d_ids, const uint32_t* d_n_ids, uint32_t n, uint32_t id_cap,
                  uint32_t utd_cap, uint32_t* d_recs, uint32_t* d_hdr, uint32_t* d_edges);
int test_bsdf_queries(const scene_t& sc, hipStream_t stream, const uint32_t* d_queries, uint32_t n, int form, uint32_t* d_out);
int test_source_queries(const scene_t& sc, hipStream_t stream, const uint32_t* d_queries, uint32_t n, uint32_t* d_out);
int sensor_mask_launch(const scene_t& sc, hipStream_t stream, const uint8_t* d_shape_matches, uint32_t samples, uint64_t seed, float* d_out);
void sensor_mask_host(const scene_t& sc, const uint8_t* shape_matches, uint32_t samples, uint64_t seed, uint32_t n_threads, float* out);
constexpr uint32_t kMaxTonemapTable = 1024;
int develop_launch(const sensor_t& sn, hipStream_t stream, const double* d_value, const double* d_weight, const double* d_light, uint64_t spe,
                   uint32_t per_pixel, float* d_out);
int develop_tonemap_launch(const sensor_t& sn, hipStream_t stream, const double* d_value, const double* d_weight, const double* d_light, uint64_t spe,
                           const tonemap_args_t& t, uint32_t s, const float* d_mask, uint32_t format, uint32_t lds_table, void* d_out);
void develop_tonemap_host(const sensor_t& sn, const double* value, const double* weight, const double* light, uint64_t spe, const tonemap_args_t& t, uint32_t s,
                          const float* mask, uint32_t format, uint32_t n_threads, void* out);
int film_stats_launch(const sensor_t& sn, hipStream_t stream, uint32_t n_cus, const double* d_value, const double* d_weight, const double* d_light, uint64_t spe, uint32_t s,
                      uint32_t flags, const float* d_mask, const float* d_edges, uint32_t bins, void* d_rec, unsigned long long* d_hist, double* d_sums);
void film_stats_host(const sensor_t& sn, const double* value, const double* weight, const double* light, uint64_t spe, uint32_t s, uint32_t flags, const float* mask,
                     const float* edges, uint32_t bins, uint32_t n_threads, void* out_rec, unsigned long long* out_hist);
size_t film_compare_wave_bytes(uint64_t npix, uint32_t n_cus);
int film_compare_launch(const sensor_t& sn, hipStream_t stream, uint32_t n_cus, const double* a_value, const double* a_weight, const double* a_light, uint64_t spe_a,
                        const double* b_value, const double* b_weight, const double* b_light, uint64_t spe_b, uint32_t s, uint32_t flags, double eps, const float* d_mask,
                        void* d_rec, double* d_sums, void* d_wave, float* d_diff);
void film_compare_host(const sensor_t& sn, const double* a_value, const double* a_weight, const double* a_light, uint64_t spe_a, const double* b_value,
                       const double* b_weight, const double* b_light, uint64_t spe_b, uint32_t s, uint32_t flags, double eps, const float* mask, uint32_t n_threads,
// ... 5 lines not shown
```

### wave_tracer_amd/csrc/wtgpu_knobs.h

```cpp
#pragma once
#include <cstddef>
#include <cstdint>

struct knobs_t {
    uint32_t cone_budget, count_stats, split_queues, lane_cache, heavy_cache, heavy_probe, coop_aperture_min, flux_task_tris, profile, no_lists, primary_axis;
    uint32_t streams, state_gb, timing, conn_pool;
    uint32_t first_rounds, rounds_margin, light_rounds, max_rounds, stagger_round;
    uint32_t shrink_r1, shrink_f1, shrink_r2, shrink_f2, shrink_h1, decay_q, decay_c;
    uint32_t heavy_waves_per_cu, round_blocks_per_cu, grid_div_b, grid_div_c, grid_div_hard, grid_mul_flux;
    uint32_t sorted_interact, coop_io, staged_connect, connect_class, tiled_splat;
    uint32_t trace_staged, trace_stages, trace_staged_rounds, trace_sm, trace_ab;
    uint32_t develop_per_pixel, tonemap_lds_table;
    uint32_t dbg_stage;
    uint32_t host_prof, trace_launch, tail_diag, trace_ab_verbose;
    uint32_t grid_div_cls[4];
};

enum knob_kind_t {
    KNOB_U32,
    KNOB_INT,
    KNOB_NONZERO,
    KNOB_PRESENT
};
struct knob_t {
    const char* name;
    uint32_t knobs_t::*field;
    knob_kind_t kind;
    long long dflt, lo, hi;
    const char* help;
};
#pragma GCC visibility push(hidden)
extern const knob_t kKnobs[];
extern const size_t kNumKnobs;
constexpr uint32_t kKnobConeBudget = 96, kKnobFluxTaskTris = 2048;

void read_knobs(knobs_t& k);
#pragma GCC visibility pop
```

### wave_tracer_amd/csrc/wtgpu_knobs.hip

```cpp
#include "wtgpu_knobs.h"

#include <algorithm>
#include <climits>
#include <cstdio>
#include <cstdlib>

#include "wt/bdpt.h"

using wt::kMaxWalkIters;
using wt::kWalkIterLimit;

#define K(field) &knobs_t::field
static constexpr long long kU32 = 0xFFFFFFFFll;
const knob_t kKnobs[] = {
    {"WTGPU_CONE_BUDGET", K(cone_budget), KNOB_U32, kKnobConeBudget, 0, kU32, "work units one lane may spend on a cone query before it is handed to a wavefront (wtgpu_kernels.h: kConeBudget)"},
    {"WTGPU_COUNT_STATS", K(count_stats), KNOB_U32, 1, 0, kU32, "0: the kernels keep no statistics (wtgpu_kernels.h: launch_args_t::count_stats)"},
    {"WTGPU_SPLIT_QUEUES", K(split_queues), KNOB_U32, 1, 0, kU32, "round queues keep sensor and emitter walks apart; 0: one mixed queue (A/B)"},
    {"WTGPU_LANE_CACHE", K(lane_cache), KNOB_U32, 1, 0, kU32, "0 (diagnostic): the per-lane traversal without its remembered rejecting triangles"},
    {"WTGPU_HEAVY_CACHE", K(heavy_cache), KNOB_U32, 1, 0, kU32, "0 (diagnostic): the wave-cooperative traversal without its remembered rejecting triangles"},
    {"WTGPU_HEAVY_PROBE", K(heavy_probe), KNOB_U32, 1, 0, kU32, "k_trace_heavy: any-hit probe of the near slab before the handed-over cone query too; 0: off"},
    {"WTGPU_COOP_APERTURE_MIN", K(coop_aperture_min), KNOB_U32, 8, 0, kU32, "segments from which an aperture is built by a wavefront; 0xFFFFFFFF: every aperture by a single lane of pass B"},
    {"WTGPU_FLUX_TASK_TRIS", K(flux_task_tris), KNOB_U32, kKnobFluxTaskTris, 64, kU32, "triangles per region-sum task (k_flux_split / k_flux_tasks; wtgpu_kernels.h: kFluxTaskTris)"},
    {"WTGPU_PROFILE", K(profile), KNOB_U32, 0, 0, kU32, "1 / 2 / 3: in-kernel clock breakdowns, printed by wtgpu_get_counters (wtgpu_counters.hip)"},
    {"WTGPU_NO_LISTS", K(no_lists), KNOB_PRESENT, 0, 0, 1, "set (any value; plt_bdpt, diagnostic): no bounded triangle lists, every interaction region is gathered"},
    {"WTGPU_PRIMARY_AXIS", K(primary_axis), KNOB_U32, 0, 0, kU32, "1 (plt_bdpt): the triangle under the beam axis of every diffusive hit comes from the trace kernels' axis query"},
    {"WTGPU_STREAMS", K(streams), KNOB_INT, 3, 1, INT_MAX, "state slices = internal streams; ms per pass at 1 / 2 / 3 / 4 / 6 / 8: 158 / 142 / 130 / 142 / 157 / 206 (headline)"},
    {"WTGPU_STATE_GB", K(state_gb), KNOB_INT, 224, 1, INT_MAX, "budget of the per-batch state of all slices, GB (of the MI355X's 288; never more than 85 % of what is free): deep scenes get smaller batches"},
    {"WTGPU_TIMING", K(timing), KNOB_NONZERO, 1, 0, 1, "0: no per-kernel HIP events (wtgpu_last_render_timings reads zeros)"},
    {"WTGPU_CONN_POOL", K(conn_pool), KNOB_U32, 16, 1, kU32, "staged connections: pending connections per sample of a chunk"},
    {"WTGPU_FIRST_ROUNDS", K(first_rounds), KNOB_U32, 0, 0, kMaxWalkIters, "rounds launched up front; 0: adaptive (the recent batches' mean + WTGPU_ROUNDS_MARGIN); tests use 2, 96 = as before round 4"},
    {"WTGPU_ROUNDS_MARGIN", K(rounds_margin), KNOB_U32, 2, 0, kU32, "rounds added to the recent batches' mean"},
    {"WTGPU_LIGHT_ROUNDS", K(light_rounds), KNOB_U32, 1, 0, kU32, "0: the rounds beyond the expected ones as ordinary rounds only (k_light_rounds off)"},
    {"WTGPU_MAX_ROUNDS", K(max_rounds), KNOB_U32, kWalkIterLimit, 8, kWalkIterLimit, "rounds a batch may get before its surviving walks are dropped and counted (CHANGES RESULTS below the default, wt/bdpt.h kWalkIterLimit: nothing is dropped in any workload seen; 96 = rounds 1-5)"},
    {"WTGPU_STAGGER_ROUND", K(stagger_round), KNOB_U32, 0, 0, kMaxWalkIters - 1, "r > 0 (diagnostic): a batch starts when the previous one has finished its round r; 0: all streams start at once.  4 streams, r = 0 / 3 / 6 / 10 / 16: 151 / 150 / 161 / 200 / 263 ms per pass"},
    {"WTGPU_SHRINK_R1", K(shrink_r1), KNOB_U32, 8, 0, kU32, "from this round on the round kernels' grids are divided by WTGPU_SHRINK_F1 (heavy: WTGPU_SHRINK_H1)"},
    {"WTGPU_SHRINK_F1", K(shrink_f1), KNOB_U32, 4, 1, kU32, "see WTGPU_SHRINK_R1"},
    {"WTGPU_SHRINK_R2", K(shrink_r2), KNOB_U32, 16, 0, kU32, "from this round on the grids are divided by WTGPU_SHRINK_F2 (heavy: 32)"},
    {"WTGPU_SHRINK_F2", K(shrink_f2), KNOB_U32, 32, 1, kU32, "see WTGPU_SHRINK_R2"},
    {"WTGPU_SHRINK_H1", K(shrink_h1), KNOB_U32, 4, 1, kU32, "see WTGPU_SHRINK_R1"},
    {"WTGPU_DECAY_Q", K(decay_q), KNOB_U32, 0, 0, kU32, "per cent; > 0: grids follow WTGPU_DECAY_C x q^round instead of the step schedule above"},
    {"WTGPU_DECAY_C", K(decay_c), KNOB_U32, 4, 1, kU32, "safety factor of the geometric schedule"},
    {"WTGPU_HEAVY_WAVES", K(heavy_waves_per_cu), KNOB_U32, 8, 1, kU32, "wavefronts per CU of the wave-per-item kernels; swept 6 / 8 / 10 / 12 / 16 / 24 / 32: 169.6 / 168.0 / 171.6 / 174.3 / 176 / 181 / 183 ms per pass"},
    {"WTGPU_ROUND_BLOCKS", K(round_blocks_per_cu), KNOB_U32, 8, 1, kU32, "blocks per CU of the round kernels' persistent grids"},
    {"WTGPU_GRID_B", K(grid_div_b), KNOB_U32, 4, 1, kU32, "pass B's grid relative to the round's (divisor)"},
    {"WTGPU_GRID_C", K(grid_div_c), KNOB_U32, 1, 1, kU32, "pass C's grid (divisor); 2 until round 4; 1: bidir_room 33.6 -> 33.9, cornell 25.15 -> 25.35 Msamples/s, pass C's bracket 69 -> 56 / 93 -> 65 ms"},
    {"WTGPU_GRID_HARD", K(grid_div_hard), KNOB_U32, 4, 1, kU32, "k_interact_c_hard's grid (divisor)"},
    {"WTGPU_GRID_FLUX", K(grid_mul_flux), KNOB_U32, 2, 1, kU32, "k_flux_tasks' grid (multiplier)"},
    {"WTGPU_SORTED_INTERACT", K(sorted_interact), KNOB_U32, 0, 0, kU32, "pass A: 0 k_interact (one kernel, every walk); 1 k_classify + one kernel per material class; 2 k_classify + k_interact_sorted"},
    {"WTGPU_COOP_IO", K(coop_io), KNOB_U32, 0, 0, kU32, "1: pass A with wave-cooperative record transfers (k_interact_coop)"},
    {"WTGPU_STAGED_CONNECT", K(staged_connect), KNOB_U32, 0, 0, kU32, "connections: 0 k_connect_strat (one kernel per strategy item); 1 k_connect_eval -> k_connect_shadow -> k_connect_mis, in chunks"},
    {"WTGPU_CONNECT_CLASS", K(connect_class), KNOB_U32, 1, 0, kU32, "connections (the one-kernel form): 0 k_connect_strat (an item is one strategy of a sample); 1 k_connect_class (an item is a sample, bucketed by the lengths of its subpaths, all of its strategies in a row; DESIGN.md §4)"},
    {"WTGPU_TILED_SPLAT", K(tiled_splat), KNOB_U32, 1, 0, kU32, "0: the plain per-sample splat kernel"},
    {"WTGPU_TRACE_STAGED", K(trace_staged), KNOB_U32, 1, 0, kU32, "1: the traversal in stages (k_tr_axis / k_tr_cone / k_tr_policy / k_tr_tail) ..."},
    {"WTGPU_TRACE_STAGES", K(trace_stages), KNOB_U32, 3, 1, 16, "... with this many cone stages before the tail ..."},
    {"WTGPU_TRACE_STAGED_ROUNDS", K(trace_staged_rounds), KNOB_U32, 4, 0, kU32, "... for the first so many rounds of a batch (the long ones: a stage is a launch, and a short round is bound by its launches)"},
    {"WTGPU_TRACE_SM", K(trace_sm), KNOB_U32, 0, 0, kU32, "1: the phase-machine trace kernel (k_trace_sm)"},
    {"WTGPU_TRACE_AB", K(trace_ab), KNOB_U32, 0, 0, kU32, "n: the first n rounds replay their trace queue through both trace kernels, timed, outputs compared (wtgpu_trace_ab.hip)"},
    {"WTGPU_DEVELOP_PER_PIXEL", K(develop_per_pixel), KNOB_U32, 0, 0, 1, "k_develop: 0 one lane per plane element; 1 one lane per pixel (A/B: tools/bench_develop.py)"},
    {"WTGPU_TONEMAP_LDS_TABLE", K(tonemap_lds_table), KNOB_U32, 0, 0, 1, "k_develop_tonemap: 1 every block stages the colour table in LDS; 0 the lanes read it through the caches (A/B: tools/bench_develop.py)"},
    {"WTGPU_DEBUG_STAGE", K(dbg_stage), KNOB_INT, 1 << 30, INT_MIN, INT_MAX, "bring-up aid: stops launching the round kernels after stage n (INVALID RESULTS)"},
    {"WTGPU_HOST_PROF", K(host_prof), KNOB_PRESENT, 0, 0, 1, "set: host time spent inside each kind of launch call, printed per render call"},
    {"WTGPU_TRACE_LAUNCH", K(trace_launch), KNOB_PRESENT, 0, 0, 1, "set (bring-up aid): every launch is named and waited for — the last line names a kernel that hangs"},
    {"WTGPU_TAIL_DIAG", K(tail_diag), KNOB_PRESENT, 0, 0, 1, "set: why the host was called back for a pending batch, printed at exit (DESIGN.md §9)"},
    {"WTGPU_TRACE_AB_VERBOSE", K(trace_ab_verbose), KNOB_PRESENT, 0, 0, 1, "set: one line per round replayed by WTGPU_TRACE_AB"},
};
#undef K
const size_t kNumKnobs = sizeof(kKnobs) / sizeof(kKnobs[0]);

void read_knobs(knobs_t& k) {
    for (size_t i = 0; i < kNumKnobs; ++i) {
        const knob_t& d = kKnobs[i];
        const char* e = getenv(d.name);
        long long v = d.dflt;
        if (d.kind == KNOB_PRESENT) v = e ? 1 : 0;
        else if (e && d.kind == KNOB_U32) v = std::min<long long>(std::max<long long>(0, strtoll(e, nullptr, 10)), kU32);
        else if (e && d.kind == KNOB_INT) v = atoi(e);
        else if (e) v = atoi(e) != 0;
        k.*d.field = (uint32_t)std::min(d.hi, std::max(d.lo, v));
    }
    unsigned v[4] = {1, 4, 2, 4};
    if (const char* e = getenv("WTGPU_GRID_CLS")) sscanf(e, "%u,%u,%u,%u", &v[0], &v[1], &v[2], &v[3]);
    for (int c = 0; c < 4; ++c) k.grid_div_cls[c] = std::max(1u, v[c]);
}
```

### wave_tracer_amd/csrc/wtgpu_upload.hip

```cpp
#include "wtgpu_host.h"

static int g_env_by_host = 0;
__attribute__((constructor)) static void wtgpu_runtime_settings() {
    if (getenv("HSA_KERNARG_POOL_SIZE")) g_env_by_host |= 1;
    setenv("HSA_KERNARG_POOL_SIZE", "16777216", 0);
}
static int runtime_settings_ok(std::string& why) {
    const char* k = getenv("HSA_KERNARG_POOL_SIZE");
    const long ring = k ? atol(k) : (1l << 20);
    if (getenv("WTGPU_ALLOW_SLOW_RUNTIME")) return 1;
    if (ring < (4l << 20)) {
        why = "HSA_KERNARG_POOL_SIZE=" + std::string(k ? k : "(unset)") + ": a batch enqueues ~900 launches of ~1 KB of kernel arguments; with a ring below 4 MiB the enqueueing "
              "thread blocks and the streams serialise; export HSA_KERNARG_POOL_SIZE=16777216 before the HIP runtime initialises, or WTGPU_ALLOW_SLOW_RUNTIME=1";
        return 0;
    }
    if (!(g_env_by_host & 1) && !getenv("WTGPU_QUIET")) {
        static bool told = false;
        if (!told) fprintf(stderr, "[wtgpu] note: HSA_KERNARG_POOL_SIZE=16777216 defaulted by libwtgpu.so; effective only if the HIP runtime had not initialised before the library was loaded "
                           "(a host that uses HIP earlier exports it itself, INTEGRATION.md)\n");
        told = true;
    }
    return 1;
}

// ... 102 lines not shown
            if ((rc = dmalloc(s, &P.fsdq[q], path_mode ? (size_t)st.cap : 1))) return rc;
        }
        if ((rc = dmalloc(s, &P.neeq, path_mode ? (size_t)st.cap : 1))) return rc;
        if ((rc = dmalloc(s, &P.fsd_f, path_mode ? (size_t)st.cap : 1))) return rc;
        if ((rc = dmalloc(s, &P.nee_recs, path_mode ? (size_t)st.cap : 1))) return rc;
        if ((rc = dmalloc(s, &P.gather_info, path_mode ? (size_t)st.cap : 1))) return rc;
        path_state_t* dP = nullptr;
        if ((rc = dmalloc(s, &dP, 1))) return rc;
        HIP_CHECK(hipMemcpy(dP, &P, sizeof(P), hipMemcpyHostToDevice));
        s->d_path_slices.push_back(dP);
    }
    if (!path_mode) {
        bdpt_ext_t X;
        X.tri_class = s->d_tri_class;
        if (s->knobs.sorted_interact && (rc = dmalloc(s, &X.cls_queue, (size_t)kNumWalkClasses * W2))) return rc;
        X.pend_cap = (uint32_t)std::min<uint64_t>((uint64_t)s->knobs.conn_pool * st.cap + 4096, 0xFFFFFF00ull);
        if (s->knobs.staged_connect) {
            uint64_t pairs = 0;
            const int md = h.opts.max_depth;
            for (int t = 0; t <= md + 2; ++t)
                for (int q = 0; q <= md + 2; ++q)
                    if (t + q - 2 >= 0 && t + q - 2 <= md && !(t == 1 && q == 1)) ++pairs;
            X.n_chunks = (uint32_t)((pairs * st.cap + X.pend_cap - 1) / X.pend_cap);
            if ((rc = dmalloc(s, &X.pend, (size_t)X.pend_cap))) return rc;
            if ((rc = dmalloc(s, &X.surv, (size_t)X.pend_cap))) return rc;
            if ((rc = dmalloc(s, &X.chunk_ctl, (size_t)X.n_chunks * kChunkCtlWords))) return rc;
        } else
            X.pend_cap = 0;
        s->pend_cap = X.pend_cap;
        s->n_chunks = X.n_chunks;
        bdpt_ext_t* dX = nullptr;
        if ((rc = dmalloc(s, &dX, 1))) return rc;
        HIP_CHECK(hipMemcpy(dX, &X, sizeof(X), hipMemcpyHostToDevice));
        st.ext = dX;
    }
    if ((rc = dmalloc(s, &st.verts, path_mode ? 1 : (size_t)st.max_verts * kVertexWords * W2))) return rc;
    if ((rc = dmalloc(s, &st.ctx, kCtxWords * (size_t)st.cap))) return rc;
    if ((rc = dmalloc(s, &st.trav, (kTravWords + kStageWords) * W2))) return rc;
    if ((rc = dmalloc(s, &st.tris, (size_t)kTriListWords * W2))) return rc;
    if ((rc = dmalloc(s, &st.queue[0], W2))) return rc;
    if ((rc = dmalloc(s, &st.queue[1], W2))) return rc;
    if ((rc = dmalloc(s, &st.heavy_queue, 3 * W2))) return rc;
    if ((rc = dmalloc(s, &st.intb_queue, W2))) return rc;
    if ((rc = dmalloc(s, &st.gather_queue, W2))) return rc;
    if ((rc = dmalloc(s, &st.intc_queue, W2))) return rc;
    if ((rc = dmalloc(s, &st.intd_queue, W2))) return rc;
    st.ftask_cap = path_mode ? 1u : (1u << 22);
    if ((rc = dmalloc(s, &st.ftasks, (size_t)st.ftask_cap))) return rc;
    if ((rc = dmalloc(s, &st.facc, path_mode ? 1 : W2))) return rc;
    st.epool_cap = 1u << 23;
    if ((rc = dmalloc(s, &st.epool, (size_t)st.epool_cap))) return rc;
    if ((rc = dmalloc(s, &st.ctl, (size_t)CTL_WORDS))) return rc;
    HIP_CHECK(hipMemset(st.ctl, 0, CTL_WORDS * sizeof(uint32_t)));
    st.fsd_cap = (h.opts.FSD && !h.opts.force_ray_tracing && !path_mode) ? (uint32_t)std::min<uint64_t>(W2, 1u << 22) : 1u;
    if ((rc = dmalloc(s, &st.fsd_hdr, st.fsd_cap))) return rc;
    st.fsd_ecap = st.fsd_cap > 1 ? (uint32_t)std::min<uint64_t>(64ull * st.cap + kFsdMaxEdges, 1ull << 28) : 1u;
    if ((rc = dmalloc(s, &st.fsd_edges, (size_t)st.fsd_ecap))) return rc;
    if ((rc = dmalloc(s, &st.strat_items, path_mode ? 1 : (size_t)kNumKeys * st.cap))) return rc;
    if ((rc = dmalloc(s, &st.strat_count, (size_t)kNumKeys))) return rc;
    if ((rc = dmalloc(s, &st.strat_prefix, (size_t)kClassTableWords))) return rc;
    if ((rc = dmalloc(s, &st.lacc, 4 * (size_t)st.cap))) return rc;
    HIP_CHECK(hipMemset(st.strat_count, 0, kNumKeys * sizeof(uint32_t)));
    HIP_CHECK(hipStreamCreateWithFlags(&s->streams[k], hipStreamNonBlocking));
    HIP_CHECK(hipEventCreateWithFlags(&s->ev_done[k], hipEventDisableTiming));
    return WTGPU_OK;
}

static uint64_t size_batches(const wtgpu_scene* s, uint64_t max_batch, uint32_t& n_slices) {
    const scene_t& h = s->host;
    const uint64_t npix = (uint64_t)h.sensor.width * h.sensor.height;
    n_slices = s->knobs.streams;
    uint64_t batch_cap = max_batch ? std::min<uint64_t>(max_batch, 1u << 24) : std::min<uint64_t>(npix, 1u << 22);
    n_slices = (uint32_t)std::min<uint64_t>(n_slices, std::max<uint64_t>(1, batch_cap / 64));
    {
        const bool pm = h.opts.integrator != INTEGRATOR_BDPT;
        const uint64_t mv = (uint64_t)h.opts.max_depth + 2;
        uint64_t per_sample = 4ull * (2 * ((pm ? kPathWalkWords : kWalkWords) + (pm ? 0 : mv * kVertexWords) + kTravWords + kStageWords + 2 + kTriListWords) + kCtxWords) + 64ull * 28ull + 2048ull;
        if (pm) per_sample += 2ull * 48ull * sizeof(utd_edge_rec_t) + sizeof(path_nee_rec_t) + 3ull * 4ull + 4ull + sizeof(uint2);
        else per_sample += (s->knobs.staged_connect ? (uint64_t)s->knobs.conn_pool * (sizeof(conn_pending_t) + 4ull) : 0ull) + (s->knobs.sorted_interact ? 4ull * 2ull * kNumWalkClasses : 0ull);
        uint64_t budget = (uint64_t)s->knobs.state_gb << 30;
        size_t free_b = 0, total_b = 0;
        if (hipMemGetInfo(&free_b, &total_b) == hipSuccess && free_b > 0) budget = std::min<uint64_t>(budget, (uint64_t)((double)free_b * 0.85));
        const uint64_t fixed = (uint64_t)n_slices * ((1ull << 23) * 4ull + (1ull << 22) * 8ull + (64ull << 20));
        budget = budget > 2 * fixed ? budget - fixed : budget / 2;
        const uint64_t fit = std::max<uint64_t>(4096, budget / per_sample / n_slices);
        if (batch_cap > fit) batch_cap = fit;
    }
    return batch_cap;
}

static int upload_impl(wtgpu_scene* s, uint64_t max_batch) {
    read_knobs(s->knobs);
    int n_cu = 256;
    (void)hipDeviceGetAttribute(&n_cu, hipDeviceAttributeMultiprocessorCount, s->device);
    s->n_cus = (uint32_t)std::max(1, n_cu);
    int rc;
    if ((rc = upload_scene_arrays(s)) != WTGPU_OK) return rc;
    uint32_t n_slices = 0;
    const uint64_t batch_cap = size_batches(s, max_batch, n_slices);
    unsigned long long* counters = nullptr;
    if ((rc = dmalloc(s, &counters, kNumCounters + kProfSlots + 1))) return rc;
    HIP_CHECK(hipMemset(counters, 0, (kNumCounters + kProfSlots + 1) * sizeof(unsigned long long)));
    s->slices.resize(n_slices);
    s->streams.resize(n_slices);
    s->ev_done.resize(n_slices);
    for (uint32_t k = 0; k < n_slices; ++k)
// ... 84 lines not shown
```

Measured before the change: 32.70.

## Run thin-queue tail rounds fully in the resident light-rounds kernel with hand-over tracking

Moves the per-stage bodies of the FSD kernels (flux split, flux tasks, interaction C) into a shared header so the resident k_light_rounds kernel can run every stage of a round in a single one-wavefront launch. It adds a configurable walk limit (WTGPU_LIGHT_MAX_WALKS) below which the resident kernel takes over, and records the round at which the queue becomes thin. The host then ends the up-front rounds where the queue is expected to be thin. The aim is to cut launch overhead and per-round host round-trips in the long tail of nearly empty rounds, at the cost of running those rounds on one wavefront and adding tail statistics bookkeeping.

Measured after the change: 32.44. Within noise of the previous version (-0.8%).

```diff
diff --git a/include/wtgpu.h b/include/wtgpu.h
--- a/include/wtgpu.h
+++ b/include/wtgpu.h
@@ -110,6 +110,8 @@
 
 int wtgpu_last_render_timings(wtgpu_scene* scene, float out[12]);
 
+int wtgpu_tail_stats(wtgpu_scene* scene, uint64_t out[16]);
+
 int wtgpu_develop(const wtgpu_scene* scene, const double* value, const double* weight, const double* light, uint64_t spe, float* out);
 
 int wtgpu_develop_device(wtgpu_scene* scene, void* stream, const double* d_value, const double* d_weight, const double* d_light, uint64_t spe, float* d_out);
diff --git a/wave_tracer_amd/api.py b/wave_tracer_amd/api.py
--- a/wave_tracer_amd/api.py
+++ b/wave_tracer_amd/api.py
@@ -98,7 +98,8 @@
            "wtgpu_scene_shape_id", "wtgpu_scene_sensor_mask_spec", "wtgpu_sensor_mask", "wtgpu_sensor_mask_host",
            "wtgpu_scene_tonemap_spec", "wtgpu_develop_device", "wtgpu_tonemap_device", "wtgpu_tonemap_host",
            "wtgpu_film_stats_edges", "wtgpu_film_stats_device", "wtgpu_film_stats_host",
-           "wtgpu_film_compare_device", "wtgpu_film_compare_host"]
+           "wtgpu_film_compare_device", "wtgpu_film_compare_host", "wtgpu_tail_stats"]
+TAIL_STAGES = ("trace", "heavy", "pass_a", "edge_walk", "pass_b", "flux_tasks", "pass_c")
 PROGRESS_CB = C.CFUNCTYPE(C.c_int, C.c_uint64, C.c_uint64, C.c_void_p)
 CAPTURE_CB = C.CFUNCTYPE(None, C.c_uint64, C.c_void_p)
 
@@ -180,6 +181,7 @@
     lib.wtgpu_get_counters.argtypes = [vp, C.POINTER(Counters)]
     lib.wtgpu_reset_counters.argtypes = [vp]
     lib.wtgpu_last_render_timings.argtypes = [vp, C.POINTER(C.c_float * 12)]
+    lib.wtgpu_tail_stats.argtypes = [vp, C.POINTER(C.c_uint64 * 16)]
     lib.wtgpu_develop.argtypes = [vp, vp, vp, vp, u64, vp]
     lib.wtgpu_scene_destroy.argtypes = [vp]
     lib.wtgpu_scene_destroy.restype = None
@@ -716,6 +718,13 @@
                 "trace_launches": int(t[5]), "batches": int(t[6]), "trace_heavy_ms": t[7], "interact_b_ms": t[8], "flux_ms": t[9],
                 "interact_c_ms": t[10], "rounds_per_batch": float(t[11])}
 
+    def tail_stats(self):
+        t = (C.c_uint64 * 16)()
+        _check(load_library().wtgpu_tail_stats(self._h, C.byref(t)))
+        return {"launches": int(t[0]), "rounds": int(t[1]),
+                "items": dict(zip(TAIL_STAGES, (int(t[2 + i]) for i in range(len(TAIL_STAGES))))),
+                "looks_by_stop": {code: int(t[9 + code]) for code in range(6)}}
+
     def close(self):
         if self._h:
             load_library().wtgpu_scene_destroy(self._h)
diff --git a/wave_tracer_amd/csrc/kernels_fsd.hip b/wave_tracer_amd/csrc/kernels_fsd.hip
--- a/wave_tracer_amd/csrc/kernels_fsd.hip
+++ b/wave_tracer_amd/csrc/kernels_fsd.hip
@@ -1,238 +1,15 @@
 #include "wtgpu_kernels.h"
+#include "kernels_fsd_bodies.h"
 
 namespace wtk {
 
 __global__ void __launch_bounds__(64, 3) k_flux_split(launch_args_t a) {
     __shared__ coop_gather_shared_t sh;
-    coop_set_dropped_counter(sh, a.st.counters + kDroppedSlot);
-    uint32_t* ctl = a.st.ctl;
-    const uint32_t n = ctl[CTL_INTC_COUNT];
-    const int lane = threadIdx.x & 63;
-    for (;;) {
-        const uint32_t base = wave_grab(ctl + CTL_FSPLIT_HEAD);
-        if (base >= n) break;
-        uint32_t w_mine = 0;
-        bool need = false;
-        if (base + (uint32_t)lane < n) {
-            w_mine = a.st.intc_queue[base + lane];
-            need = is_region_marker(a.st.trav[(size_t)w_mine * kTravWords + WT_TRAV_WORD(tuid)]);
-        }
-        unsigned long long m = __ballot(need);
-        while (m) {
-            const int src = __ffsll((long long)m) - 1;
-            m &= m - 1;
-            const uint32_t w = (uint32_t)__shfl((int)w_mine, src, 64);
-            const walk_trace_in_t wk = walk_load_trace_in(a.st.walks, a.st.walk_words, w);
-            const cone_t tcone = walk_trace_envelope(a.sc, wk);
-            const float beam_dist = __uint_as_float(a.st.trav[(size_t)w * kTravWords + WT_TRAV_WORD(dist)]);
-            const float region_depth = __uint_as_float(a.st.trav[(size_t)w * kTravWords + WT_TRAV_WORD(region_depth)]);
-            if (threadIdx.x == 0) a.st.facc[w] = 0.0;
-            coop_split(a.sc, tcone, range_t{beam_dist, beam_dist + region_depth}, sh, a.flux_task_tris, [&](int32_t ptr) {
-                const uint32_t idx = atomicAdd(ctl + CTL_FTASK_COUNT, 1u);
-                if (idx < a.st.ftask_cap)
-                    a.st.ftasks[idx] = make_uint2(w, (uint32_t)ptr);
-                else
-                    atomicAdd(a.st.counters + offsetof(bdpt_counters_t, fsd_pool_overflow) / sizeof(unsigned long long), 1ull);
-            });
-            __syncthreads();
-        }
-    }
+    flux_split_body(a, sh);
 }
 __global__ void __launch_bounds__(64, WTGPU_LB_FLUX) k_flux_tasks(launch_args_t a) {
     __shared__ coop_gather_shared_t sh;
-    coop_set_dropped_counter(sh, a.st.counters + kDroppedSlot);
-    uint32_t* ctl = a.st.ctl;
-    const uint32_t n = min(ctl[CTL_FTASK_COUNT], a.st.ftask_cap);
-    const size_t W2 = 2 * (size_t)a.st.cap;
-    for (;;) {
-        const uint32_t item = wave_grab_item(ctl + CTL_FTASK_HEAD);
-        if (item >= n) break;
-        const uint2 task = a.st.ftasks[item];
-        const uint32_t w = task.x;
-        walk_t wk;
-        soa_load(a.st.walks, a.st.walk_words, w, wk);
-        const float beam_dist = __uint_as_float(a.st.trav[(size_t)w * kTravWords + WT_TRAV_WORD(dist)]);
-        const float region_depth = __uint_as_float(a.st.trav[(size_t)w * kTravWords + WT_TRAV_WORD(region_depth)]);
-        const bool want_front = a.st.trav[(size_t)w * kTravWords + WT_TRAV_WORD(front_face)] != 0;
-        const range_t izr{beam_dist, beam_dist + region_depth};
-        const vec3 sd3 = beam_footprint(wk.beam, beam_dist) / kBeamEnvelope;
-        const cone_t tcone = walk_trace_envelope(a.sc, wk);
-        unsigned long long gst[2] = {0, 0};
-        const double flux = coop_gather(a.sc, tcone, izr, wk.beam.env, cone_frame(wk.beam.env), izr, vec2{sd3.x, sd3.y}, want_front, sh, true, false,
-                                        a.profile ? gst : nullptr, (int32_t)task.y).flux;
-        if (threadIdx.x == 0) {
-            if (flux != 0.0) unsafeAtomicAdd(&a.st.facc[w], flux);
-            if (a.profile) {
-                atomicAdd(a.st.counters + kNumCounters + 0, 1ull);
-                atomicAdd(a.st.counters + kNumCounters + 1, gst[0]);
-                atomicAdd(a.st.counters + kNumCounters + 2, gst[1]);
-                atomicMax(a.st.counters + kNumCounters + 4, gst[0]);
-            }
-        }
-        __syncthreads();
-    }
-}
-
-constexpr uint32_t kEasyTries = 512;
-constexpr uint32_t kStageSegs = 256;
-template <int BLOCK>
-WT_D void interact_c_body(const launch_args_t& a, int in) {
-    constexpr bool HARD = BLOCK > 64;
-    __shared__ uint32_t s_item;
-    __shared__ uint32_t s_tmin;
-    __shared__ float s_res[3];
-    __shared__ stack_entry_t lds[8];
-    __shared__ fsd_edge_t s_seg[kStageSegs];
-    uint32_t* ctl = a.st.ctl;
-    const uint32_t n = ctl[HARD ? CTL_INTD_COUNT : CTL_INTC_COUNT];
-    const uint32_t* queue_in = HARD ? a.st.intd_queue : a.st.intc_queue;
-    const int tid = threadIdx.x, lane = threadIdx.x & 63;
-    bdpt_counters_t ctr;
-    memset(&ctr, 0, sizeof(ctr));
-    const size_t W2 = 2 * (size_t)a.st.cap;
-    const fsd_pool_t pool{a.st.fsd_hdr, a.st.fsd_edges, ctl + CTL_FSD_COUNTER, a.st.fsd_cap, ctl + CTL_FSD_ECOUNTER, a.st.fsd_ecap};
-    for (;;) {
-        const long long pl0 = a.profile == 3 ? clock64() : 0;
-        uint32_t item = 0;
-        if (HARD) {
-            __syncthreads();
-            if (tid == 0) s_item = atomicAdd(ctl + CTL_INTD_HEAD, 1u);
-            __syncthreads();
-            item = s_item;
-        } else
-            item = wave_grab_item(ctl + CTL_INTC_HEAD);
-        if (item >= n) break;
-        const uint32_t w = queue_in[item];
-        uint32_t i, stream;
-        walk_ident(a, w, i, stream);
-        const uint64_t j = a.j0 + i;
-        const uint32_t pix = (uint32_t)(j % a.npix);
-        const uint64_t sample_id = ((uint64_t)pix << 32) | ((a.sample_begin + j / a.npix) & 0xFFFFFFFFull);
-        const uint32_t rng_draws = a.st.walks[(size_t)w * a.st.walk_words + WT_WALK_WORD(rng_draws)];
-        const uint32_t slot = a.st.trav[(size_t)w * kTravWords + WT_TRAV_WORD(by)];
-        fsd_aperture_t ap = pool.hdr[slot];
-        const fsd_edges_ref_t ed = fsd_pool_edges(pool, slot);
-        const long long pc0 = a.profile == 3 ? clock64() : 0;
-        if (!HARD) {
-            const walk_trace_in_t wk = walk_load_trace_in(a.st.walks, a.st.walk_words, w);
-            cone_t benv = wk.env;
-            const float tr_dist = __uint_as_float(a.st.trav[(size_t)w * kTravWords + WT_TRAV_WORD(dist)]);
-            const float tr_depth = __uint_as_float(a.st.trav[(size_t)w * kTravWords + WT_TRAV_WORD(region_depth)]);
-            const uint32_t tr_tuid = a.st.trav[(size_t)w * kTravWords + WT_TRAV_WORD(tuid)], tr_ntris = a.st.trav[(size_t)w * kTravWords + WT_TRAV_WORD(ntris)];
-            const bool tr_front = a.st.trav[(size_t)w * kTravWords + WT_TRAV_WORD(front_face)] != 0;
-            const range_t izr{tr_dist, tr_dist + tr_depth};
-            const vec2 axes = cone_axes(benv, tr_dist);
-            const vec2 sigma{axes.x / kBeamEnvelope, axes.y / kBeamEnvelope};
-            double flux;
-            if (is_region_marker(tr_tuid)) {
-                flux = a.st.facc[w];
-            } else {
-                const uint32_t* tl = a.st.tris + (size_t)w * kTriListWords;
-                flux = (uint32_t)lane < tr_ntris ? (double)region_triangle_flux(a.sc, cone_frame(benv), benv, izr, sigma, tl[lane], tr_front) : 0.0;
-#pragma unroll
-                for (int off = 32; off > 0; off >>= 1) flux += __shfl_xor(flux, off, 64);
-            }
-            const float I = (float)(1.0 - flux);
-            ap.recp_I = I > 0.f ? 1.f / I : 0.f;
-            if (lane == 0) pool.hdr[slot] = ap;
-        }
-        const sampler_t ss = make_sampler(a.seed, sample_id, stream, 0);
-        const uint32_t base = fsd_tries_base(make_sampler(a.seed, sample_id, stream, rng_draws));
-        const uint32_t max_tries = fsd_max_tries(ap);
-        const uint32_t t_begin = HARD ? kEasyTries : 0u, t_end = HARD ? max_tries : (max_tries < kEasyTries ? max_tries : kEasyTries);
-        bool acc = false;
-        uint32_t t_acc = 0;
-        float rx = 0.f, ry = 0.f, rf = 0.f;
-        auto run_tries = [&](const fsd_edges_ref_t& edr) {
-            for (uint32_t t0 = t_begin; t0 < t_end && !acc; t0 += BLOCK) {
-                const uint32_t t = t0 + (uint32_t)tid;
-                fsd_try_t r{{0.f, 0.f}, 0.f, 0u};
-                if (t < t_end) r = fsd_try(a.sc, ap, edr, sampler_at(ss, base + t * kFsdDrawsPerTry));
-                if (!HARD) {
-                    const unsigned long long am = __ballot(r.accept != 0);
-                    if (am) {
-                        const int wl = __ffsll((long long)am) - 1;
-                        rx = __shfl(r.x.x, wl, 64);
-                        ry = __shfl(r.x.y, wl, 64);
-                        rf = __shfl(r.f, wl, 64);
-                        t_acc = t0 + (uint32_t)wl;
-                        acc = true;
-                    }
-                } else {
-                    if (tid == 0) s_tmin = 0xFFFFFFFFu;
-                    __syncthreads();
-                    if (r.accept) atomicMin(&s_tmin, t);
-                    __syncthreads();
-                    const uint32_t tm = s_tmin;
-                    if (tm != 0xFFFFFFFFu) {
-                        if (t == tm) {
-                            s_res[0] = r.x.x;
-                            s_res[1] = r.x.y;
-                            s_res[2] = r.f;
-                        }
-                        __syncthreads();
-                        rx = s_res[0];
-                        ry = s_res[1];
-                        rf = s_res[2];
-                        t_acc = tm;
-                        acc = true;
-                    }
-                    __syncthreads();
-                }
-            }
-        };
-        if (ap.n_edges <= kStageSegs) {
-            __syncthreads();
-            for (uint32_t k = (uint32_t)tid; k < ap.n_edges; k += BLOCK) s_seg[k] = ed.p[k];
-            __syncthreads();
-            run_tries(fsd_edges_ref_t{s_seg, 1});
-        } else
-            run_tries(ed);
-        if (a.profile == 3 && tid == 0) {
-            const int bin = 31 - __clz((int)max(ap.n_edges, 1u));
-            atomicAdd(a.st.counters + kNumCounters + 8 + bin, 1ull);
-            atomicAdd(a.st.counters + kNumCounters + 24 + bin, (unsigned long long)(acc ? t_acc + 1u - t_begin : t_end - t_begin));
-            atomicAdd(a.st.counters + kNumCounters + 40 + bin, (unsigned long long)(clock64() - pc0));
-            atomicAdd(a.st.counters + kNumCounters + 112 + bin, (unsigned long long)(pc0 - pl0));
-        }
-        const long long pm0 = a.profile == 3 ? clock64() : 0;
-        if (!HARD && !acc && t_end < max_tries) {
-            if (lane == 0) a.st.intd_queue[atomicAdd(ctl + CTL_INTD_COUNT, 1u)] = w;
-            continue;
-        }
-        bool cont = false;
-        if (tid == 0) {
-            walk_t wk;
-            soa_load(a.st.walks, a.st.walk_words, w, wk);
-            trav_result_t tr;
-            soa_load(a.st.trav, kTravWords, w, tr);
-            fsd_defer_t defer;
-            defer.defer_sampling = defer.to_sampling_pass = 0;
-            defer.have_aperture = 1;
-            defer.split_no_primary = 0;
-            defer.known_no_primary = 1;
-            defer.no_primary = 0;
-            defer.has_gather = defer.gather_n_edges = defer.gather_edge_overflow = 0;
-            defer.gather_flux = 0.f;
-            defer.gather_edges = nullptr;
-            defer.pending = 0;
-            defer.resolved = 1;
-            defer.slot = slot;
-            defer.base = base;
-            defer.next_try = 0;
-            defer.fs = fsd_finalize(ap, acc, vec2{rx, ry}, rf);
-            defer.end_draws = fsd_draws_after(base, acc ? t_acc : max_tries - 1u);
-            const uint_list_t tris{a.st.tris + (size_t)w * kTriListWords, 1u, kMaxConeTris};
-            const vertex_store_t vs{a.st.verts, a.st.vert_words, w};
-            stack_ref_t stack = make_stack_ref(lds, 1, 8, 8, nullptr);
-            cont = bdpt_walk_step<2>(a.sc, wk, tr, tris, vs, pool, a.seed, sample_id, stream, &ctr, &stack, &defer);
-            wk.active = cont ? 1u : 0u;
-            soa_store(a.st.walks, a.st.walk_words, w, wk);
-            if (a.profile == 3) atomicAdd(a.st.counters + kNumCounters + 96 + (31 - __clz((int)max(ap.n_edges, 1u))), (unsigned long long)(clock64() - pm0));
-        }
-        if (tid < 64) queue_append(a, ctl, 1 - in, cont, w);
-    }
-    if (a.count_stats && tid < 64) flush_counters(a.st.counters, ctr);
+    flux_tasks_body(a, sh);
 }
 __global__ void __launch_bounds__(64, WTGPU_LB_INTERACT_C) k_interact_c(launch_args_t a, int in) { interact_c_body<64>(a, in); }
 __global__ void __launch_bounds__(WTGPU_HARD_BLOCK) k_interact_c_hard(launch_args_t a, int in) { interact_c_body<WTGPU_HARD_BLOCK>(a, in); }
diff --git a/wave_tracer_amd/csrc/kernels_fsd_bodies.h b/wave_tracer_amd/csrc/kernels_fsd_bodies.h
--- /dev/null
+++ b/wave_tracer_amd/csrc/kernels_fsd_bodies.h
@@ -0,0 +1,237 @@
+#pragma once
+#include "wtgpu_kernels.h"
+
+namespace wtk {
+
+WT_D void flux_split_body(const launch_args_t& a, coop_gather_shared_t& sh) {
+    coop_set_dropped_counter(sh, a.st.counters + kDroppedSlot);
+    uint32_t* ctl = a.st.ctl;
+    const uint32_t n = ctl[CTL_INTC_COUNT];
+    const int lane = threadIdx.x & 63;
+    for (;;) {
+        const uint32_t base = wave_grab(ctl + CTL_FSPLIT_HEAD);
+        if (base >= n) break;
+        uint32_t w_mine = 0;
+        bool need = false;
+        if (base + (uint32_t)lane < n) {
+            w_mine = a.st.intc_queue[base + lane];
+            need = is_region_marker(a.st.trav[(size_t)w_mine * kTravWords + WT_TRAV_WORD(tuid)]);
+        }
+        unsigned long long m = __ballot(need);
+        while (m) {
+            const int src = __ffsll((long long)m) - 1;
+            m &= m - 1;
+            const uint32_t w = (uint32_t)__shfl((int)w_mine, src, 64);
+            const walk_trace_in_t wk = walk_load_trace_in(a.st.walks, a.st.walk_words, w);
+            const cone_t tcone = walk_trace_envelope(a.sc, wk);
+            const float beam_dist = __uint_as_float(a.st.trav[(size_t)w * kTravWords + WT_TRAV_WORD(dist)]);
+            const float region_depth = __uint_as_float(a.st.trav[(size_t)w * kTravWords + WT_TRAV_WORD(region_depth)]);
+            if (threadIdx.x == 0) a.st.facc[w] = 0.0;
+            coop_split(a.sc, tcone, range_t{beam_dist, beam_dist + region_depth}, sh, a.flux_task_tris, [&](int32_t ptr) {
+                const uint32_t idx = atomicAdd(ctl + CTL_FTASK_COUNT, 1u);
+                if (idx < a.st.ftask_cap)
+                    a.st.ftasks[idx] = make_uint2(w, (uint32_t)ptr);
+                else
+                    atomicAdd(a.st.counters + offsetof(bdpt_counters_t, fsd_pool_overflow) / sizeof(unsigned long long), 1ull);
+            });
+            __syncthreads();
+        }
+    }
+}
+WT_D void flux_tasks_body(const launch_args_t& a, coop_gather_shared_t& sh) {
+    coop_set_dropped_counter(sh, a.st.counters + kDroppedSlot);
+    uint32_t* ctl = a.st.ctl;
+    const uint32_t n = min(ctl[CTL_FTASK_COUNT], a.st.ftask_cap);
+    const size_t W2 = 2 * (size_t)a.st.cap;
+    for (;;) {
+        const uint32_t item = wave_grab_item(ctl + CTL_FTASK_HEAD);
+        if (item >= n) break;
+        const uint2 task = a.st.ftasks[item];
+        const uint32_t w = task.x;
+        walk_t wk;
+        soa_load(a.st.walks, a.st.walk_words, w, wk);
+        const float beam_dist = __uint_as_float(a.st.trav[(size_t)w * kTravWords + WT_TRAV_WORD(dist)]);
+        const float region_depth = __uint_as_float(a.st.trav[(size_t)w * kTravWords + WT_TRAV_WORD(region_depth)]);
+        const bool want_front = a.st.trav[(size_t)w * kTravWords + WT_TRAV_WORD(front_face)] != 0;
+        const range_t izr{beam_dist, beam_dist + region_depth};
+        const vec3 sd3 = beam_footprint(wk.beam, beam_dist) / kBeamEnvelope;
+        const cone_t tcone = walk_trace_envelope(a.sc, wk);
+        unsigned long long gst[2] = {0, 0};
+        const double flux = coop_gather(a.sc, tcone, izr, wk.beam.env, cone_frame(wk.beam.env), izr, vec2{sd3.x, sd3.y}, want_front, sh, true, false,
+                                        a.profile ? gst : nullptr, (int32_t)task.y).flux;
+        if (threadIdx.x == 0) {
+            if (flux != 0.0) unsafeAtomicAdd(&a.st.facc[w], flux);
+            if (a.profile) {
+                atomicAdd(a.st.counters + kNumCounters + 0, 1ull);
+                atomicAdd(a.st.counters + kNumCounters + 1, gst[0]);
+                atomicAdd(a.st.counters + kNumCounters + 2, gst[1]);
+                atomicMax(a.st.counters + kNumCounters + 4, gst[0]);
+            }
+        }
+        __syncthreads();
+    }
+}
+
+constexpr uint32_t kEasyTries = 512;
+constexpr uint32_t kStageSegs = 256;
+template <int BLOCK>
+WT_D void interact_c_body(const launch_args_t& a, int in) {
+    constexpr bool HARD = BLOCK > 64;
+    __shared__ uint32_t s_item;
+    __shared__ uint32_t s_tmin;
+    __shared__ float s_res[3];
+    __shared__ stack_entry_t lds[8];
+    __shared__ fsd_edge_t s_seg[kStageSegs];
+    uint32_t* ctl = a.st.ctl;
+    const uint32_t n = ctl[HARD ? CTL_INTD_COUNT : CTL_INTC_COUNT];
+    const uint32_t* queue_in = HARD ? a.st.intd_queue : a.st.intc_queue;
+    const int tid = threadIdx.x, lane = threadIdx.x & 63;
+    bdpt_counters_t ctr;
+    memset(&ctr, 0, sizeof(ctr));
+    const size_t W2 = 2 * (size_t)a.st.cap;
+    const fsd_pool_t pool{a.st.fsd_hdr, a.st.fsd_edges, ctl + CTL_FSD_COUNTER, a.st.fsd_cap, ctl + CTL_FSD_ECOUNTER, a.st.fsd_ecap};
+    for (;;) {
+        const long long pl0 = a.profile == 3 ? clock64() : 0;
+        uint32_t item = 0;
+        if (HARD) {
+            __syncthreads();
+            if (tid == 0) s_item = atomicAdd(ctl + CTL_INTD_HEAD, 1u);
+            __syncthreads();
+            item = s_item;
+        } else
+            item = wave_grab_item(ctl + CTL_INTC_HEAD);
+        if (item >= n) break;
+        const uint32_t w = queue_in[item];
+        uint32_t i, stream;
+        walk_ident(a, w, i, stream);
+        const uint64_t j = a.j0 + i;
+        const uint32_t pix = (uint32_t)(j % a.npix);
+        const uint64_t sample_id = ((uint64_t)pix << 32) | ((a.sample_begin + j / a.npix) & 0xFFFFFFFFull);
+        const uint32_t rng_draws = a.st.walks[(size_t)w * a.st.walk_words + WT_WALK_WORD(rng_draws)];
+        const uint32_t slot = a.st.trav[(size_t)w * kTravWords + WT_TRAV_WORD(by)];
+        fsd_aperture_t ap = pool.hdr[slot];
+        const fsd_edges_ref_t ed = fsd_pool_edges(pool, slot);
+        const long long pc0 = a.profile == 3 ? clock64() : 0;
+        if (!HARD) {
+            const walk_trace_in_t wk = walk_load_trace_in(a.st.walks, a.st.walk_words, w);
+            cone_t benv = wk.env;
+            const float tr_dist = __uint_as_float(a.st.trav[(size_t)w * kTravWords + WT_TRAV_WORD(dist)]);
+            const float tr_depth = __uint_as_float(a.st.trav[(size_t)w * kTravWords + WT_TRAV_WORD(region_depth)]);
+            const uint32_t tr_tuid = a.st.trav[(size_t)w * kTravWords + WT_TRAV_WORD(tuid)], tr_ntris = a.st.trav[(size_t)w * kTravWords + WT_TRAV_WORD(ntris)];
+            const bool tr_front = a.st.trav[(size_t)w * kTravWords + WT_TRAV_WORD(front_face)] != 0;
+            const range_t izr{tr_dist, tr_dist + tr_depth};
+            const vec2 axes = cone_axes(benv, tr_dist);
+            const vec2 sigma{axes.x / kBeamEnvelope, axes.y / kBeamEnvelope};
+            double flux;
+            if (is_region_marker(tr_tuid)) {
+                flux = a.st.facc[w];
+            } else {
+                const uint32_t* tl = a.st.tris + (size_t)w * kTriListWords;
+                flux = (uint32_t)lane < tr_ntris ? (double)region_triangle_flux(a.sc, cone_frame(benv), benv, izr, sigma, tl[lane], tr_front) : 0.0;
+#pragma unroll
+                for (int off = 32; off > 0; off >>= 1) flux += __shfl_xor(flux, off, 64);
+            }
+            const float I = (float)(1.0 - flux);
+            ap.recp_I = I > 0.f ? 1.f / I : 0.f;
+            if (lane == 0) pool.hdr[slot] = ap;
+        }
+        const sampler_t ss = make_sampler(a.seed, sample_id, stream, 0);
+        const uint32_t base = fsd_tries_base(make_sampler(a.seed, sample_id, stream, rng_draws));
+        const uint32_t max_tries = fsd_max_tries(ap);
+        const uint32_t t_begin = HARD ? kEasyTries : 0u, t_end = HARD ? max_tries : (max_tries < kEasyTries ? max_tries : kEasyTries);
+        bool acc = false;
+        uint32_t t_acc = 0;
+        float rx = 0.f, ry = 0.f, rf = 0.f;
+        auto run_tries = [&](const fsd_edges_ref_t& edr) {
+            for (uint32_t t0 = t_begin; t0 < t_end && !acc; t0 += BLOCK) {
+                const uint32_t t = t0 + (uint32_t)tid;
+                fsd_try_t r{{0.f, 0.f}, 0.f, 0u};
+                if (t < t_end) r = fsd_try(a.sc, ap, edr, sampler_at(ss, base + t * kFsdDrawsPerTry));
+                if (!HARD) {
+                    const unsigned long long am = __ballot(r.accept != 0);
+                    if (am) {
+                        const int wl = __ffsll((long long)am) - 1;
+                        rx = __shfl(r.x.x, wl, 64);
+                        ry = __shfl(r.x.y, wl, 64);
+                        rf = __shfl(r.f, wl, 64);
+                        t_acc = t0 + (uint32_t)wl;
+                        acc = true;
+                    }
+                } else {
+                    if (tid == 0) s_tmin = 0xFFFFFFFFu;
+                    __syncthreads();
+                    if (r.accept) atomicMin(&s_tmin, t);
+                    __syncthreads();
+                    const uint32_t tm = s_tmin;
+                    if (tm != 0xFFFFFFFFu) {
+                        if (t == tm) {
+                            s_res[0] = r.x.x;
+                            s_res[1] = r.x.y;
+                            s_res[2] = r.f;
+                        }
+                        __syncthreads();
+                        rx = s_res[0];
+                        ry = s_res[1];
+                        rf = s_res[2];
+                        t_acc = tm;
+                        acc = true;
+                    }
+                    __syncthreads();
+                }
+            }
+        };
+        if (ap.n_edges <= kStageSegs) {
+            __syncthreads();
+            for (uint32_t k = (uint32_t)tid; k < ap.n_edges; k += BLOCK) s_seg[k] = ed.p[k];
+            __syncthreads();
+            run_tries(fsd_edges_ref_t{s_seg, 1});
+        } else
+            run_tries(ed);
+        if (a.profile == 3 && tid == 0) {
+            const int bin = 31 - __clz((int)max(ap.n_edges, 1u));
+            atomicAdd(a.st.counters + kNumCounters + 8 + bin, 1ull);
+            atomicAdd(a.st.counters + kNumCounters + 24 + bin, (unsigned long long)(acc ? t_acc + 1u - t_begin : t_end - t_begin));
+            atomicAdd(a.st.counters + kNumCounters + 40 + bin, (unsigned long long)(clock64() - pc0));
+            atomicAdd(a.st.counters + kNumCounters + 112 + bin, (unsigned long long)(pc0 - pl0));
+        }
+        const long long pm0 = a.profile == 3 ? clock64() : 0;
+        if (!HARD && !acc && t_end < max_tries) {
+            if (lane == 0) a.st.intd_queue[atomicAdd(ctl + CTL_INTD_COUNT, 1u)] = w;
+            continue;
+        }
+        bool cont = false;
+        if (tid == 0) {
+            walk_t wk;
+            soa_load(a.st.walks, a.st.walk_words, w, wk);
+            trav_result_t tr;
+            soa_load(a.st.trav, kTravWords, w, tr);
+            fsd_defer_t defer;
+            defer.defer_sampling = defer.to_sampling_pass = 0;
+            defer.have_aperture = 1;
+            defer.split_no_primary = 0;
+            defer.known_no_primary = 1;
+            defer.no_primary = 0;
+            defer.has_gather = defer.gather_n_edges = defer.gather_edge_overflow = 0;
+            defer.gather_flux = 0.f;
+            defer.gather_edges = nullptr;
+            defer.pending = 0;
+            defer.resolved = 1;
+            defer.slot = slot;
+            defer.base = base;
+            defer.next_try = 0;
+            defer.fs = fsd_finalize(ap, acc, vec2{rx, ry}, rf);
+            defer.end_draws = fsd_draws_after(base, acc ? t_acc : max_tries - 1u);
+            const uint_list_t tris{a.st.tris + (size_t)w * kTriListWords, 1u, kMaxConeTris};
+            const vertex_store_t vs{a.st.verts, a.st.vert_words, w};
+            stack_ref_t stack = make_stack_ref(lds, 1, 8, 8, nullptr);
+            cont = bdpt_walk_step<2>(a.sc, wk, tr, tris, vs, pool, a.seed, sample_id, stream, &ctr, &stack, &defer);
+            wk.active = cont ? 1u : 0u;
+            soa_store(a.st.walks, a.st.walk_words, w, wk);
+            if (a.profile == 3) atomicAdd(a.st.counters + kNumCounters + 96 + (31 - __clz((int)max(ap.n_edges, 1u))), (unsigned long long)(clock64() - pm0));
+        }
+        if (tid < 64) queue_append(a, ctl, 1 - in, cont, w);
+    }
+    if (a.count_stats && tid < 64) flush_counters(a.st.counters, ctr);
+}
+
+}
diff --git a/wave_tracer_amd/csrc/kernels_trace.hip b/wave_tracer_amd/csrc/kernels_trace.hip
--- a/wave_tracer_amd/csrc/kernels_trace.hip
+++ b/wave_tracer_amd/csrc/kernels_trace.hip
@@ -4,6 +4,7 @@
 
 }
 #include "kernels_trace_refill.h"
+#include "kernels_trace_heavy.h"
 namespace wtk {
 
 __global__ void __launch_bounds__(kBlock, WTGPU_LB_TRACE) k_trace_refill(launch_args_t a, int in, int first_round, uint32_t round) { trace_refill_body(a, in, first_round, round); }
@@ -654,61 +655,6 @@
     if (a.count_stats) flush_counters(a.st.counters, ctr);
 }
 
-template <bool PROF>
-WT_D void trace_heavy_body(const launch_args_t& a, coop_shared_t& sh) {
-    coop_set_dropped_counter(sh, a.st.counters + kDroppedSlot);
-    uint32_t* ctl = a.st.ctl;
-    const uint32_t n = ctl[CTL_HEAVY_COUNT];
-    const uint32_t* hq = a.st.heavy_queue;
-    uint32_t* head = ctl + CTL_HEAVY_HEAD;
-    unsigned long long n_segments = 0, n_ray_queries = 0, n_cone_queries = 0, n_overflow = 0;
-    const bool rt = a.sc.sensor.ray_trace_only || a.sc.opts.force_ray_tracing;
-    for (;;) {
-        const uint32_t item = wave_grab_item(head);
-        if (item >= n) break;
-        const uint32_t w = uniform(hq[item]);
-        const walk_trace_in_t wk = walk_load_trace_in(a.st.walks, a.st.walk_words, w);
-        const uint_list_t tris{a.st.tris + (size_t)w * kTriListWords, 1u, (a.collect_list & 1u) ? kMaxConeTris : 0u};
-        const cone_t env = uniform(walk_trace_envelope(a.sc, wk));
-        unsigned long long prof[12] = {0, 0, 0, 0, 0, 0, 0, 0, 0, 0, 0, 0};
-        const long long tt0 = PROF ? clock64() : 0;
-        const uint32_t* tv = a.st.trav + (size_t)w * kTravWords;
-        const float dist0 = uniform(__uint_as_float(tv[WT_TRAV_WORD(dist)]));
-        const uint32_t seg0 = uniform(tv[WT_TRAV_WORD(ntris)]);
-        const uint32_t nray0 = uniform(tv[WT_TRAV_WORD(n_ray_queries)]), ncone0 = uniform(tv[WT_TRAV_WORD(n_cone_queries)]);
-        ray_hit_t axis;
-        axis.tuid = uniform(tv[WT_TRAV_WORD(tuid)]);
-        axis.bx = uniform(__uint_as_float(tv[WT_TRAV_WORD(bx)]));
-        axis.by = uniform(__uint_as_float(tv[WT_TRAV_WORD(by)]));
-        axis.dist = uniform(__uint_as_float(tv[WT_TRAV_WORD(pdist)]));
-        axis.front_face = uniform(tv[WT_TRAV_WORD(front_face)]);
-        const uint32_t short0 = uniform(tv[WT_TRAV_WORD(overflow)]);
-        const uint32_t origin0 = uniform(wk.prev_offset_tuid);
-        const trav_result_t tr2 = coop_traverse(a.sc, env, uniform(wavenum_to_wavelen_m(wk.k)), WT_INF, rt, sh, tris, PROF ? prof : nullptr, true, seg0, dist0, nray0, ncone0,
-                                                &axis, !(a.collect_list & 1u) || (a.collect_list & 2u), a.heavy_probe != 0, a.heavy_cache ? short0 : kInvalid, a.heavy_cache ? origin0 : kInvalid, a.heavy_cache != 0);
-        if (PROF && threadIdx.x == 0) {
-            prof[3] = (unsigned long long)(clock64() - tt0);
-            for (int q = 0; q < 4; ++q) atomicAdd(a.st.counters + kNumCounters + q, prof[q]);
-            atomicAdd(a.st.counters + kNumCounters + 5, prof[5]);
-            atomicAdd(a.st.counters + kNumCounters + 6, prof[6]);
-            atomicAdd(a.st.counters + kNumCounters + 7, prof[7]);
-            for (int q = 8; q < 12; ++q) atomicAdd(a.st.counters + kNumCounters + q, prof[q]);
-            atomicAdd(a.st.counters + kNumCounters + 4, 1ull);
-        }
-        n_segments += 1;
-        n_ray_queries += tr2.n_ray_queries;
-        n_cone_queries += tr2.n_cone_queries;
-        if (a.collect_list & 1u) n_overflow += tr2.overflow;
-        if (threadIdx.x == 0) soa_store(a.st.trav, kTravWords, w, tr2);
-    }
-    if (a.count_stats && threadIdx.x == 0) {
-        unsigned long long* g = a.st.counters;
-        if (n_segments) atomicAdd(g + offsetof(bdpt_counters_t, segments) / 8, n_segments);
-        if (n_ray_queries) atomicAdd(g + offsetof(bdpt_counters_t, ray_queries) / 8, n_ray_queries);
-        if (n_cone_queries) atomicAdd(g + offsetof(bdpt_counters_t, cone_queries) / 8, n_cone_queries);
-        if (n_overflow) atomicAdd(g + offsetof(bdpt_counters_t, cone_tri_overflow) / 8, n_overflow);
-    }
-}
 __global__ void __launch_bounds__(64, WTGPU_LB_HEAVY) k_trace_heavy(launch_args_t a) {
     __shared__ coop_shared_t sh;
     trace_heavy_body<false>(a, sh);
diff --git a/wave_tracer_amd/csrc/kernels_trace_heavy.h b/wave_tracer_amd/csrc/kernels_trace_heavy.h
--- /dev/null
+++ b/wave_tracer_amd/csrc/kernels_trace_heavy.h
@@ -0,0 +1,62 @@
+#pragma once
+#include "wtgpu_kernels.h"
+
+namespace wtk {
+
+template <bool PROF>
+WT_D void trace_heavy_body(const launch_args_t& a, coop_shared_t& sh) {
+    coop_set_dropped_counter(sh, a.st.counters + kDroppedSlot);
+    uint32_t* ctl = a.st.ctl;
+    const uint32_t n = ctl[CTL_HEAVY_COUNT];
+    const uint32_t* hq = a.st.heavy_queue;
+    uint32_t* head = ctl + CTL_HEAVY_HEAD;
+    unsigned long long n_segments = 0, n_ray_queries = 0, n_cone_queries = 0, n_overflow = 0;
+    const bool rt = a.sc.sensor.ray_trace_only || a.sc.opts.force_ray_tracing;
+    for (;;) {
+        const uint32_t item = wave_grab_item(head);
+        if (item >= n) break;
+        const uint32_t w = uniform(hq[item]);
+        const walk_trace_in_t wk = walk_load_trace_in(a.st.walks, a.st.walk_words, w);
+        const uint_list_t tris{a.st.tris + (size_t)w * kTriListWords, 1u, (a.collect_list & 1u) ? kMaxConeTris : 0u};
+        const cone_t env = uniform(walk_trace_envelope(a.sc, wk));
+        unsigned long long prof[12] = {0, 0, 0, 0, 0, 0, 0, 0, 0, 0, 0, 0};
+        const long long tt0 = PROF ? clock64() : 0;
+        const uint32_t* tv = a.st.trav + (size_t)w * kTravWords;
+        const float dist0 = uniform(__uint_as_float(tv[WT_TRAV_WORD(dist)]));
+        const uint32_t seg0 = uniform(tv[WT_TRAV_WORD(ntris)]);
+        const uint32_t nray0 = uniform(tv[WT_TRAV_WORD(n_ray_queries)]), ncone0 = uniform(tv[WT_TRAV_WORD(n_cone_queries)]);
+        ray_hit_t axis;
+        axis.tuid = uniform(tv[WT_TRAV_WORD(tuid)]);
+        axis.bx = uniform(__uint_as_float(tv[WT_TRAV_WORD(bx)]));
+        axis.by = uniform(__uint_as_float(tv[WT_TRAV_WORD(by)]));
+        axis.dist = uniform(__uint_as_float(tv[WT_TRAV_WORD(pdist)]));
+        axis.front_face = uniform(tv[WT_TRAV_WORD(front_face)]);
+        const uint32_t short0 = uniform(tv[WT_TRAV_WORD(overflow)]);
+        const uint32_t origin0 = uniform(wk.prev_offset_tuid);
+        const trav_result_t tr2 = coop_traverse(a.sc, env, uniform(wavenum_to_wavelen_m(wk.k)), WT_INF, rt, sh, tris, PROF ? prof : nullptr, true, seg0, dist0, nray0, ncone0,
+                                                &axis, !(a.collect_list & 1u) || (a.collect_list & 2u), a.heavy_probe != 0, a.heavy_cache ? short0 : kInvalid, a.heavy_cache ? origin0 : kInvalid, a.heavy_cache != 0);
+        if (PROF && threadIdx.x == 0) {
+            prof[3] = (unsigned long long)(clock64() - tt0);
+            for (int q = 0; q < 4; ++q) atomicAdd(a.st.counters + kNumCounters + q, prof[q]);
+            atomicAdd(a.st.counters + kNumCounters + 5, prof[5]);
+            atomicAdd(a.st.counters + kNumCounters + 6, prof[6]);
+            atomicAdd(a.st.counters + kNumCounters + 7, prof[7]);
+            for (int q = 8; q < 12; ++q) atomicAdd(a.st.counters + kNumCounters + q, prof[q]);
+            atomicAdd(a.st.counters + kNumCounters + 4, 1ull);
+        }
+        n_segments += 1;
+        n_ray_queries += tr2.n_ray_queries;
+        n_cone_queries += tr2.n_cone_queries;
+        if (a.collect_list & 1u) n_overflow += tr2.overflow;
+        if (threadIdx.x == 0) soa_store(a.st.trav, kTravWords, w, tr2);
+    }
+    if (a.count_stats && threadIdx.x == 0) {
+        unsigned long long* g = a.st.counters;
+        if (n_segments) atomicAdd(g + offsetof(bdpt_counters_t, segments) / 8, n_segments);
+        if (n_ray_queries) atomicAdd(g + offsetof(bdpt_counters_t, ray_queries) / 8, n_ray_queries);
+        if (n_cone_queries) atomicAdd(g + offsetof(bdpt_counters_t, cone_queries) / 8, n_cone_queries);
+        if (n_overflow) atomicAdd(g + offsetof(bdpt_counters_t, cone_tri_overflow) / 8, n_overflow);
+    }
+}
+
+}
diff --git a/wave_tracer_amd/csrc/kernels_trace_refill.h b/wave_tracer_amd/csrc/kernels_trace_refill.h
--- a/wave_tracer_amd/csrc/kernels_trace_refill.h
+++ b/wave_tracer_amd/csrc/kernels_trace_refill.h
@@ -41,6 +41,7 @@
     ctl[CTL_NEEQ_COUNT] = 0;
     ctl[CTL_NEEQ_HEAD] = 0;
     if (n > 0) ctl[CTL_ROUNDS] = round + 1;
+    if (ctl[CTL_HANDOVER_ROUND] == kInvalid && n <= ctl[CTL_LIGHT_LIMIT]) ctl[CTL_HANDOVER_ROUND] = round;
 }
 WT_D void trace_refill_body(const launch_args_t& a, int in, int first_round, uint32_t round) {
     __shared__ stack_entry_t lds[kLdsStack * kBlock];
diff --git a/wave_tracer_amd/csrc/kernels_walk.hip b/wave_tracer_amd/csrc/kernels_walk.hip
--- a/wave_tracer_amd/csrc/kernels_walk.hip
+++ b/wave_tracer_amd/csrc/kernels_walk.hip
@@ -1,5 +1,7 @@
 #include "wtgpu_kernels.h"
 #include "kernels_trace_refill.h"
+#include "kernels_trace_heavy.h"
+#include "kernels_fsd_bodies.h"
 
 namespace wtk {
 
@@ -15,6 +17,7 @@
         ctl[CTL_INTB_COUNT] = ctl[CTL_INTB_HEAD] = ctl[CTL_GATHER_COUNT] = ctl[CTL_GATHER_HEAD] = ctl[CTL_INTC_COUNT] = ctl[CTL_INTC_HEAD] = 0;
         ctl[CTL_FTASK_COUNT] = ctl[CTL_FTASK_HEAD] = ctl[CTL_FSPLIT_HEAD] = ctl[CTL_EPOOL_COUNT] = ctl[CTL_FSD_ECOUNTER] = 0;
         ctl[CTL_INTD_COUNT] = ctl[CTL_INTD_HEAD] = 0;
+        ctl[CTL_HANDOVER_ROUND] = kInvalid;
     }
     if (i >= a.nb) return;
     const uint64_t j = a.j0 + i;
@@ -238,9 +241,7 @@
 __global__ void __launch_bounds__(kBlock, WTGPU_LB_CLS_SPM) k_interact_spm(launch_args_t a, int in) { interact_cls_body<MAT_SURFACE_SPM>(a, in); }
 __global__ void __launch_bounds__(kBlock, WTGPU_LB_CLS_SPM) k_interact_any(launch_args_t a, int in) { interact_cls_body<-1>(a, in); }
 
-__global__ void __launch_bounds__(64, 3) k_edges(launch_args_t a) {
-    __shared__ coop_gather_shared_t sh;
-    __shared__ coop_edges_t eg;
+WT_D void edges_body(const launch_args_t& a, coop_gather_shared_t& sh, coop_edges_t& eg) {
     coop_set_dropped_counter(sh, a.st.counters + kDroppedSlot);
     uint32_t* ctl = a.st.ctl;
     const uint32_t n = ctl[CTL_GATHER_COUNT];
@@ -305,6 +306,11 @@
         __syncthreads();
     }
 }
+__global__ void __launch_bounds__(64, 3) k_edges(launch_args_t a) {
+    __shared__ coop_gather_shared_t sh;
+    __shared__ coop_edges_t eg;
+    edges_body(a, sh, eg);
+}
 
 __global__ void __launch_bounds__(kBlock, WTGPU_LB_INTERACT) k_interact(launch_args_t a, int in, int first_round) { interact_body<0>(a, in, first_round); }
 #ifndef WTGPU_LB_INTERACT_COOP
@@ -313,10 +319,6 @@
 __global__ void __launch_bounds__(kBlock, WTGPU_LB_INTERACT_COOP) k_interact_coop(launch_args_t a, int in, int first_round) { interact_body<0, true>(a, in, first_round); }
 __global__ void __launch_bounds__(kBlock, WTGPU_LB_INTERACT_B) k_interact_b(launch_args_t a, int in) { interact_body<1>(a, in, 0); }
 
-#ifndef WTGPU_LIGHT_MAX_WALKS
-#define WTGPU_LIGHT_MAX_WALKS 2048
-#endif
-constexpr uint32_t kLightMaxWalks = WTGPU_LIGHT_MAX_WALKS;
 #ifndef WTGPU_LIGHT_FENCE
 #define WTGPU_LIGHT_FENCE 0
 #endif
@@ -329,35 +331,57 @@
     __builtin_amdgcn_fence(__ATOMIC_ACQUIRE, "agent");
 #endif
 }
-__global__ void __launch_bounds__(kBlock, 2) k_light_rounds(launch_args_t a, int in, uint32_t round, uint32_t max_rounds) {
+__global__ void __launch_bounds__(64, 1) k_light_rounds(launch_args_t a, int in, uint32_t round, uint32_t max_rounds, uint32_t max_walks) {
+    __shared__ coop_shared_t sh_heavy;
+    __shared__ coop_gather_shared_t sh_region;
+    __shared__ coop_edges_t eg;
     uint32_t* ctl = a.st.ctl;
     uint32_t done = 0, stop = 0;
-    if (queue_count(ctl, in) > kLightMaxWalks) {
-        if (threadIdx.x == 0) {
-            ctl[CTL_LIGHT_DONE] = 0;
-            ctl[CTL_LIGHT_STOP] = 4;
-        }
-        return;
-    }
-    if (queue_count(ctl, in) == 0) max_rounds = 0;
+    uint32_t items[kTailStages] = {0, 0, 0, 0, 0, 0, 0};
+    const uint32_t n0 = queue_count(ctl, in);
+    if (n0 > max_walks) stop = 4;
+    if (n0 == 0 || stop) max_rounds = 0;
     for (; done < max_rounds; ++done) {
+        items[0] += queue_count(ctl, in);
+        items[2] += queue_count(ctl, in);
         trace_refill_body(a, in, 0, round + done);
         light_stage_barrier();
-        if (ctl[CTL_HEAVY_COUNT] != 0) {
-            stop = 1;
-            break;
+        const uint32_t n_heavy = ctl[CTL_HEAVY_COUNT];
+        if (n_heavy) {
+            items[1] += n_heavy;
+            trace_heavy_body<false>(a, sh_heavy);
+            light_stage_barrier();
         }
         interact_body<0>(a, in, 0);
         light_stage_barrier();
-        if (ctl[CTL_GATHER_COUNT] != 0) {
-            stop = 2;
-            break;
-        }
-        interact_body<1>(a, in, 0);
-        light_stage_barrier();
-        if (ctl[CTL_INTC_COUNT] != 0) {
-            stop = 3;
-            break;
+        const uint32_t n_gather = ctl[CTL_GATHER_COUNT], n_b = ctl[CTL_INTB_COUNT];
+        if (n_gather) {
+            items[3] += n_gather;
+            edges_body(a, sh_region, eg);
+            light_stage_barrier();
+        }
+        if (n_b) {
+            items[4] += n_b;
+            interact_body<1>(a, in, 0);
+            light_stage_barrier();
+        }
+        const uint32_t n_c = ctl[CTL_INTC_COUNT];
+        if (n_c) {
+            items[6] += n_c;
+            flux_split_body(a, sh_region);
+            light_stage_barrier();
+            const uint32_t n_tasks = min(ctl[CTL_FTASK_COUNT], a.st.ftask_cap);
+            if (n_tasks) {
+                items[5] += n_tasks;
+                flux_tasks_body(a, sh_region);
+                light_stage_barrier();
+            }
+            interact_c_body<64>(a, in);
+            light_stage_barrier();
+            if (ctl[CTL_INTD_COUNT] != 0) {
+                stop = 5;
+                break;
+            }
         }
         in = 1 - in;
         if (queue_count(ctl, in) == 0) {
@@ -365,10 +389,13 @@
             break;
         }
     }
-    if (threadIdx.x == 0) {
+    __builtin_amdgcn_wave_barrier();
+    if (wave_first_lane()) {
         ctl[CTL_LIGHT_DONE] = done;
         ctl[CTL_LIGHT_STOP] = stop;
-    }
-}
-
-}
+#pragma unroll
+        for (uint32_t q = 0; q < kTailStages; ++q) ctl[CTL_TAIL_ITEMS0 + q] = items[q];
+    }
+}
+
+}
diff --git a/wave_tracer_amd/csrc/wtgpu.hip b/wave_tracer_amd/csrc/wtgpu.hip
--- a/wave_tracer_amd/csrc/wtgpu.hip
+++ b/wave_tracer_amd/csrc/wtgpu.hip
@@ -3,6 +3,7 @@
 thread_local std::string g_err;
 
 static void note_rounds(wtgpu_scene* s, uint32_t n) { s->rounds_hist[s->rounds_hist_n++ % 8u] = n; }
+static void note_handover(wtgpu_scene* s, uint32_t round) { s->handover_hist[s->handover_hist_n++ % 8u] = round; }
 static int drain_rec(wtgpu_scene* s, chunk_rec_t& r) {
     if (!r.busy) return WTGPU_OK;
     HIP_CHECK(hipEventSynchronize(r.ev[r.ev_final]));
@@ -163,10 +164,12 @@
             if (sf <= 3) HP_LAUNCH(k_edges, dim3(gh), dim3(64), 0, st_, a);
             if (sf <= 4) HP_LAUNCH(k_interact_b, dim3(std::max<uint32_t>(1u, g0 / grid_div_b)), dim3(kBlock), 0, st_, a, in);
             rec(r, st_);
-            HP_LAUNCH(k_flux_split, dim3(std::max<uint32_t>(1u, gh / 4u)), dim3(64), 0, st_, a);
-            HP_LAUNCH(k_flux_tasks, dim3(std::max<uint32_t>(1u, gh * grid_mul_flux)), dim3(64), 0, st_, a);
-            rec(r, st_);
-            HP_LAUNCH(k_interact_c, dim3(std::max<uint32_t>(1u, gh / grid_div_c)), dim3(64), 0, st_, a, in);
+            if (sf <= 5) {
+                HP_LAUNCH(k_flux_split, dim3(std::max<uint32_t>(1u, gh / 4u)), dim3(64), 0, st_, a);
+                HP_LAUNCH(k_flux_tasks, dim3(std::max<uint32_t>(1u, gh * grid_mul_flux)), dim3(64), 0, st_, a);
+            }
+            rec(r, st_);
+            if (sf <= 6) HP_LAUNCH(k_interact_c, dim3(std::max<uint32_t>(1u, gh / grid_div_c)), dim3(64), 0, st_, a, in);
             HP_LAUNCH(k_interact_c_hard, dim3(std::max<uint32_t>(1u, gh / K.grid_div_hard)), dim3(WTGPU_HARD_BLOCK), 0, st_, a, in);
             rec(r, st_);
         }
@@ -175,7 +178,7 @@
     }
     void light(const launch_args_t& a, hipStream_t st_, uint32_t launched) {
         if (path_mode || !K.light_rounds || launched >= K.max_rounds) return;
-        HP_LAUNCH(k_light_rounds, dim3(1), dim3(kBlock), 0, st_, a, (int)(launched & 1u), launched, K.max_rounds - launched);
+        HP_LAUNCH(k_light_rounds, dim3(1), dim3(64), 0, st_, a, (int)(launched & 1u), launched, K.max_rounds - launched, K.light_max_walks);
     }
     int tail(const launch_args_t& a, chunk_rec_t& r, hipStream_t st_) {
         const uint32_t nb = a.nb, gf = g_full(nb);
@@ -225,8 +228,17 @@
 };
 static_assert(sizeof(launch_args_t) <= sizeof(wtgpu_scene::pending_t::args), "pending_t::args holds a launch block");
 
+static uint32_t expected_rounds_by_length(const wtgpu_scene* s);
 static uint32_t expected_rounds(const wtgpu_scene* s) {
     if (s->knobs.first_rounds) return s->knobs.first_rounds;
+    const uint32_t by_length = expected_rounds_by_length(s);
+    if (s->host.opts.integrator != INTEGRATOR_BDPT || !s->knobs.light_rounds || s->handover_hist_n == 0) return by_length;
+    const uint32_t n = std::min<uint32_t>(s->handover_hist_n, 8u);
+    uint32_t sum = 0;
+    for (uint32_t i = 0; i < n; ++i) sum += s->handover_hist[i];
+    return std::min<uint32_t>(by_length, (sum + n - 1) / n + s->knobs.rounds_margin);
+}
+static uint32_t expected_rounds_by_length(const wtgpu_scene* s) {
     if (s->rounds_hist_n == 0) return std::min<uint32_t>(kMaxWalkIters, 32u);
     const uint32_t n = std::min<uint32_t>(s->rounds_hist_n, 8u);
     uint32_t sum = 0;
@@ -246,19 +258,22 @@
     if (light && launched < s->knobs.max_rounds) {
         launched += r.h_mid[CTL_LIGHT_DONE];
         stop = r.h_mid[CTL_LIGHT_STOP];
-        s->light_rounds_run += r.h_mid[CTL_LIGHT_DONE];
+        s->tail_stats[0] += 1;
+        s->tail_stats[1] += r.h_mid[CTL_LIGHT_DONE];
+        for (uint32_t q = 0; q < kTailStages; ++q) s->tail_stats[2 + q] += r.h_mid[CTL_TAIL_ITEMS0 + q];
+        s->tail_stats[2 + kTailStages + std::min<uint32_t>(stop, 5u)] += 1;
     }
     bool done = false;
     if (s->knobs.tail_diag) {
-        static unsigned long long looks = 0, by_stop[8] = {0}, light_done = 0, left_sum = 0;
+        static unsigned long long looks = 0, by_stop[8] = {0}, light_done = 0, left_sum = 0, handover_sum = 0;
         static bool reg = false;
-        if (!reg) { reg = true; atexit([] { fprintf(stderr, "[tail diag] looks %llu (stop 0/1/2/3/4: %llu %llu %llu %llu %llu), light rounds %llu, walks left at looks (sum) %llu\n", looks, by_stop[0], by_stop[1], by_stop[2], by_stop[3], by_stop[4], light_done, left_sum); }); }
+        if (!reg) { reg = true; atexit([] { fprintf(stderr, "[tail diag] looks %llu (stop 0/1/2/3/4/5: %llu %llu %llu %llu %llu %llu), resident rounds %llu, walks left at looks (sum) %llu, hand-over rounds (sum) %llu\n", looks, by_stop[0], by_stop[1], by_stop[2], by_stop[3], by_stop[4], by_stop[5], light_done, left_sum, handover_sum); }); }
         looks++; by_stop[stop < 8 ? stop : 7]++; light_done += light ? r.h_mid[CTL_LIGHT_DONE] : 0;
         left_sum += r.h_mid[CTL_COUNT0 + (launched & 1u)] + r.h_mid[CTL_BACK0 + (launched & 1u)];
-    }
-    if (stop >= 1 && stop <= 3) {
-        static const int from[4] = {0, 1, 3, 5};
-        const int rc = L.rounds(a, s->d_path_slices[k], r, st_, launched, launched + 1, from[stop]);
+        if (stop == 0 && r.h_mid[CTL_COUNT0 + (launched & 1u)] + r.h_mid[CTL_BACK0 + (launched & 1u)] == 0 && r.h_mid[CTL_HANDOVER_ROUND] != kInvalid) handover_sum += r.h_mid[CTL_HANDOVER_ROUND];
+    }
+    if (stop == 5) {
+        const int rc = L.rounds(a, s->d_path_slices[k], r, st_, launched, launched + 1, 7);
         if (rc) return rc;
         launched += 1;
     } else {
@@ -266,6 +281,7 @@
         const uint32_t left = r.h_mid[CTL_COUNT0 + q] + r.h_mid[CTL_BACK0 + q];
         if (left == 0) {
             note_rounds(s, std::min<uint32_t>(r.h_mid[CTL_ROUNDS], kMaxWalkIters));
+            if (light && r.h_mid[CTL_HANDOVER_ROUND] != kInvalid) note_handover(s, std::min<uint32_t>(r.h_mid[CTL_HANDOVER_ROUND], kMaxWalkIters));
             done = true;
         } else if (launched >= s->knobs.max_rounds)
             done = true;
diff --git a/wave_tracer_amd/csrc/wtgpu_counters.hip b/wave_tracer_amd/csrc/wtgpu_counters.hip
--- a/wave_tracer_amd/csrc/wtgpu_counters.hip
+++ b/wave_tracer_amd/csrc/wtgpu_counters.hip
@@ -102,6 +102,18 @@
     s->cap_hits = 0;
     for (double& v : s->acc) v = 0;
     s->rounds_launched_total = 0;
+    for (uint64_t& v : s->tail_stats) v = 0;
+    return WTGPU_OK;
+}
+int wtgpu_tail_stats(wtgpu_scene* s, uint64_t out[16]) {
+    if (!s || !out || !s->uploaded) return fail(WTGPU_ERR_INVALID, "scene not uploaded");
+    const int rc = drain_all(s);
+    if (rc) return rc;
+    for (int i = 0; i < 16; ++i) out[i] = s->tail_stats[i];
+    if (s->knobs.tail_diag)
+        fprintf(stderr, "[tail stats] resident launches %llu, rounds %llu; items: trace %llu heavy %llu pass A %llu edge walk %llu pass B %llu flux tasks %llu pass C %llu; looks by stop code 0/4/5: %llu %llu %llu\n",
+                (unsigned long long)out[0], (unsigned long long)out[1], (unsigned long long)out[2], (unsigned long long)out[3], (unsigned long long)out[4], (unsigned long long)out[5], (unsigned long long)out[6],
+                (unsigned long long)out[7], (unsigned long long)out[8], (unsigned long long)out[9], (unsigned long long)out[13], (unsigned long long)out[14]);
     return WTGPU_OK;
 }
 
diff --git a/wave_tracer_amd/csrc/wtgpu_host.h b/wave_tracer_amd/csrc/wtgpu_host.h
--- a/wave_tracer_amd/csrc/wtgpu_host.h
+++ b/wave_tracer_amd/csrc/wtgpu_host.h
@@ -104,7 +104,9 @@
     film_scratch_t fs, fc;
     double ab_ms[2] = {0, 0};
     uint64_t ab_mismatch = 0, ab_walks = 0, ab_rounds = 0;
-    uint64_t light_rounds_run = 0;
+    uint32_t handover_hist[8] = {0};
+    uint32_t handover_hist_n = 0;
+    uint64_t tail_stats[16] = {0};
     using knobs_t = ::knobs_t;
     knobs_t knobs{};
 };
diff --git a/wave_tracer_amd/csrc/wtgpu_kernels.h b/wave_tracer_amd/csrc/wtgpu_kernels.h
--- a/wave_tracer_amd/csrc/wtgpu_kernels.h
+++ b/wave_tracer_amd/csrc/wtgpu_kernels.h
@@ -55,7 +55,12 @@
                   CTL_TPOL_COUNT0 = 41, CTL_TPOL_COUNT1 = 42, CTL_TPOL_HEAD = 43, CTL_TCONE_COUNT0 = 44, CTL_TCONE_COUNT1 = 45, CTL_TCONE_HEAD = 46,
                   CTL_CLS_COUNT0 = 33, CTL_CLS_HEAD0 = 37,
                   CTL_LIGHT_DONE = 47, CTL_LIGHT_STOP = 48,
-                  CTL_WORDS = 56 };
+                  CTL_LIGHT_LIMIT = 49,
+                  CTL_HANDOVER_ROUND = 50,
+                  CTL_TAIL_ITEMS0 = 51,
+                  CTL_WORDS = 64 };
+constexpr uint32_t kTailStages = 7;
+static_assert(CTL_TAIL_ITEMS0 + kTailStages <= CTL_WORDS, "control block");
 constexpr uint32_t kTriListWords = 128;
 constexpr uint32_t kGatherMarker = 0xFFFFFFFEu;
 constexpr uint32_t kApertureMarker = 0xFFFFFFFDu, kNullApertureMarker = 0xFFFFFFFCu;
@@ -314,7 +319,7 @@
 __global__ void k_interact_coop(launch_args_t a, int in, int first_round);
 __global__ void k_edges(launch_args_t a);
 __global__ void k_interact_b(launch_args_t a, int in);
-__global__ void k_light_rounds(launch_args_t a, int in, uint32_t round, uint32_t max_rounds);
+__global__ void k_light_rounds(launch_args_t a, int in, uint32_t round, uint32_t max_rounds, uint32_t max_walks);
 __global__ void k_flux_split(launch_args_t a);
 __global__ void k_flux_tasks(launch_args_t a);
 __global__ void k_interact_c(launch_args_t a, int in);
diff --git a/wave_tracer_amd/csrc/wtgpu_knobs.h b/wave_tracer_amd/csrc/wtgpu_knobs.h
--- a/wave_tracer_amd/csrc/wtgpu_knobs.h
+++ b/wave_tracer_amd/csrc/wtgpu_knobs.h
@@ -5,7 +5,7 @@
 struct knobs_t {
     uint32_t cone_budget, count_stats, split_queues, lane_cache, heavy_cache, heavy_probe, coop_aperture_min, flux_task_tris, profile, no_lists, primary_axis;
     uint32_t streams, state_gb, timing, conn_pool;
-    uint32_t first_rounds, rounds_margin, light_rounds, max_rounds, stagger_round;
+    uint32_t first_rounds, rounds_margin, light_rounds, light_max_walks, max_rounds, stagger_round;
     uint32_t shrink_r1, shrink_f1, shrink_r2, shrink_f2, shrink_h1, decay_q, decay_c;
     uint32_t heavy_waves_per_cu, round_blocks_per_cu, grid_div_b, grid_div_c, grid_div_hard, grid_mul_flux;
     uint32_t sorted_interact, coop_io, staged_connect, connect_class, tiled_splat;
diff --git a/wave_tracer_amd/csrc/wtgpu_knobs.hip b/wave_tracer_amd/csrc/wtgpu_knobs.hip
--- a/wave_tracer_amd/csrc/wtgpu_knobs.hip
+++ b/wave_tracer_amd/csrc/wtgpu_knobs.hip
@@ -30,7 +30,8 @@
     {"WTGPU_CONN_POOL", K(conn_pool), KNOB_U32, 16, 1, kU32, "staged connections: pending connections per sample of a chunk"},
     {"WTGPU_FIRST_ROUNDS", K(first_rounds), KNOB_U32, 0, 0, kMaxWalkIters, "rounds launched up front; 0: adaptive (the recent batches' mean + WTGPU_ROUNDS_MARGIN); tests use 2, 96 = as before round 4"},
     {"WTGPU_ROUNDS_MARGIN", K(rounds_margin), KNOB_U32, 2, 0, kU32, "rounds added to the recent batches' mean"},
-    {"WTGPU_LIGHT_ROUNDS", K(light_rounds), KNOB_U32, 1, 0, kU32, "0: the rounds beyond the expected ones as ordinary rounds only (k_light_rounds off)"},
+    {"WTGPU_LIGHT_ROUNDS", K(light_rounds), KNOB_U32, 1, 0, kU32, "1: the rounds of a thin queue run in the resident kernel k_light_rounds, every stage of a round in one one-wavefront launch, and the rounds launched up front end where the queue is expected to be thin; the resident launch lies outside the per-round HIP-event brackets of wtgpu_last_render_timings (its rounds count as launched rounds, as before); wtgpu_tail_stats says what it did.  0: ordinary rounds only (the A/B reference)"},
+    {"WTGPU_LIGHT_MAX_WALKS", K(light_max_walks), KNOB_U32, 16, 1, kU32, "queue length up to which k_light_rounds takes a batch over (a longer queue: declined, stop code 4, the host goes on with ordinary rounds); also the length at which the trace kernels note the hand-over round (wtgpu.hip: expected_rounds).  16: the final handful of walks, as before; the sweep 64 / 128 / 256 / 512 on the headline workload has NOT been measured yet (DESIGN.md §4)"},
     {"WTGPU_MAX_ROUNDS", K(max_rounds), KNOB_U32, kWalkIterLimit, 8, kWalkIterLimit, "rounds a batch may get before its surviving walks are dropped and counted (CHANGES RESULTS below the default, wt/bdpt.h kWalkIterLimit: nothing is dropped in any workload seen; 96 = rounds 1-5)"},
     {"WTGPU_STAGGER_ROUND", K(stagger_round), KNOB_U32, 0, 0, kMaxWalkIters - 1, "r > 0 (diagnostic): a batch starts when the previous one has finished its round r; 0: all streams start at once.  4 streams, r = 0 / 3 / 6 / 10 / 16: 151 / 150 / 161 / 200 / 263 ms per pass"},
     {"WTGPU_SHRINK_R1", K(shrink_r1), KNOB_U32, 8, 0, kU32, "from this round on the round kernels' grids are divided by WTGPU_SHRINK_F1 (heavy: WTGPU_SHRINK_H1)"},
diff --git a/wave_tracer_amd/csrc/wtgpu_upload.hip b/wave_tracer_amd/csrc/wtgpu_upload.hip
--- a/wave_tracer_amd/csrc/wtgpu_upload.hip
+++ b/wave_tracer_amd/csrc/wtgpu_upload.hip
@@ -178,6 +178,7 @@
     if ((rc = dmalloc(s, &st.epool, (size_t)st.epool_cap))) return rc;
     if ((rc = dmalloc(s, &st.ctl, (size_t)CTL_WORDS))) return rc;
     HIP_CHECK(hipMemset(st.ctl, 0, CTL_WORDS * sizeof(uint32_t)));
+    HIP_CHECK(hipMemcpy(st.ctl + CTL_LIGHT_LIMIT, &s->knobs.light_max_walks, sizeof(uint32_t), hipMemcpyHostToDevice));
     st.fsd_cap = (h.opts.FSD && !h.opts.force_ray_tracing && !path_mode) ? (uint32_t)std::min<uint64_t>(W2, 1u << 22) : 1u;
     if ((rc = dmalloc(s, &st.fsd_hdr, st.fsd_cap))) return rc;
     st.fsd_ecap = st.fsd_cap > 1 ? (uint32_t)std::min<uint64_t>(64ull * st.cap + kFsdMaxEdges, 1ull << 28) : 1u;
```
